# ctu-mrs/space_filling_forest_star

Measured on AMD Instinct MI355X. Metric: accepted node expansions/sec + collision checks/sec, dense_3D 6-DoF, higher is better.
Workload: dtype f64

## Files before the change

### space_filling_forest_star_amd/csrc/engine.cpp

```cpp
#include "engine.h"
#include <dlfcn.h>

#include <algorithm>
#include <chrono>
#include <cmath>
#include <cstdlib>
#include <cstring>
#include <limits>
#include <stdexcept>

#include "sff_geom.h"

namespace sff {

void hip_check(hipError_t e, const char* what) {
  if (e != hipSuccess) throw HipError{std::string(what) + ": " + hipGetErrorString(e)};
}
#define HIPCHK(x) hip_check((x), #x)

void DevBuf::ensure(size_t bytes) {
  if (bytes <= cap) return;
  size_t want = std::max(bytes, cap * 2);
  want = (want + 255) & ~(size_t)255;
  void* np = nullptr;
  HIPCHK(hipMalloc(&np, want));
  if (p) {
    HIPCHK(hipMemcpy(np, p, cap, hipMemcpyDeviceToDevice));
    (void)hipFree(p);
  }
  p = np;
  cap = want;
}
void DevBuf::release() {
  if (p) (void)hipFree(p);
  p = nullptr;
  cap = 0;
}
void PinBuf::ensure(size_t bytes) {
  if (bytes <= cap) return;
  size_t want = std::max(bytes, cap * 2);
  void* np = nullptr;
  HIPCHK(hipHostMalloc(&np, want, hipHostMallocDefault));
  if (p) {
    memcpy(np, p, cap);
    (void)hipHostFree(p);
  }
  p = np;
  cap = want;
}
void PinBuf::release() {
  if (p) (void)hipHostFree(p);
  p = nullptr;
  cap = 0;
}
void WordRing::init(uint64_t words) {
  HIPCHK(hipEventCreateWithFlags(&ev_ring, hipEventDisableTiming));
  ring_words = words;
  ring.ensure((size_t)words * 8);
  h_ring.ensure((size_t)words * 8);
}
void WordRing::release() {
  ring.release();
  h_ring.release();
  if (ev_ring) (void)hipEventDestroy(ev_ring);
  ev_ring = nullptr;
}
void WordRing::wait_on(hipStream_t s) {
  if (!ring_pending) return;
  HIPCHK(hipStreamWaitEvent(s, ev_ring, 0));
  ring_pending = false;
}

void Mt64::reseed(uint64_t seed) {
  mt[0] = seed;
  for (int i = 1; i < 312; ++i) mt[i] = 6364136223846793005ULL * (mt[i - 1] ^ (mt[i - 1] >> 62)) + (uint64_t)i;
  idx = 312;
  draws = 0;
  q = nullptr;
  qh = qn = 0;
}
static inline uint64_t mt_step(uint64_t a, uint64_t b, uint64_t far) {
  const uint64_t x = (a & 0xFFFFFFFF80000000ULL) | (b & 0x7FFFFFFFULL);
  return far ^ (x >> 1) ^ ((0ULL - (x & 1ULL)) & 0xB5026F5AA96619E9ULL);
}
static inline uint64_t mt_temper(uint64_t y) {
  y ^= (y >> 29) & 0x5555555555555555ULL;
  y ^= (y << 17) & 0x71D67FFFEDA60000ULL;
  y ^= (y << 37) & 0xFFF7EEE000000000ULL;
  y ^= (y >> 43);
  return y;
}
void Mt64::twist() {
  for (int i = 0; i < 156; ++i) mt[i] = mt_step(mt[i], mt[i + 1], mt[i + 156]);
  for (int i = 156; i < 311; ++i) mt[i] = mt_step(mt[i], mt[i + 1], mt[i - 156]);
  mt[311] = mt_step(mt[311], mt[0], mt[155]);
  idx = 0;
}
uint64_t Mt64::next() {
  ++draws;
  if (qh < qn) return q[qh++];
  if (idx >= 312) twist();
  return mt_temper(mt[idx++]);
}
void Mt64::fill(uint64_t* out, size_t n) {
  draws += n;
  size_t k = 0;
  if (qh < qn) {
    k = std::min(n, qn - qh);
    memcpy(out, q + qh, k * sizeof(uint64_t));
    qh += k;
  }
  while (k < n) {
    if (idx >= 312) twist();
    const size_t take = std::min<size_t>(312 - idx, n - k);
    for (size_t j = 0; j < take; ++j) out[k + j] = mt_temper(mt[idx + j]);
    idx += (int)take;
    k += take;
  }
}
void Mt64::prefetch(uint64_t* buf, size_t want) {
  if (q != buf || qh > 0) {
    const size_t left = qn - qh;
    if (left) memmove(buf, q + qh, left * sizeof(uint64_t));
    q = buf;
    qh = 0;
    qn = left;
  }
  while (qn < want) {
    if (idx >= 312) twist();
    size_t take = std::min<size_t>(312 - idx, want - qn);
    for (size_t k = 0; k < take; ++k) buf[qn + k] = mt_temper(mt[idx + k]);
    idx += (int)take;
    qn += take;
  }
}
int Mt64::uniform_int(int lo, int hi) {
  uint64_t range = (uint64_t)((int64_t)hi - (int64_t)lo) + 1ULL;
  unsigned __int128 prod = (unsigned __int128)next() * range;
  uint64_t low = (uint64_t)prod;
  if (low < range) {
    uint64_t thr = (0ULL - range) % range;
    while (low < thr) {
      prod = (unsigned __int128)next() * range;
      low = (uint64_t)prod;
    }
  }
  return lo + (int)(uint64_t)(prod >> 64);
}

Ctx::Ctx(int dev, const Ctx* owner) : device(dev) {
  kn = Knobs::from_env();
  int n = 0;
  HIPCHK(hipGetDeviceCount(&n));
  if (n <= 0) throw HipError{"no HIP device visible: libsffgpu has no CPU fallback"};
  if (dev < 0 || dev >= n) throw HipError{"device index out of range"};
  HIPCHK(hipSetDevice(dev));
  hipDeviceProp_t prop;
  HIPCHK(hipGetDeviceProperties(&prop, dev));
  if (std::string(prop.gcnArchName).find("gfx950") == std::string::npos)
    throw HipError{std::string("device is ") + prop.gcnArchName + ", kernels are built for gfx950 only"};
  if (owner) {
    env = owner->env;
    envv = owner->envv;
    robv = owner->robv;
    env_built_here = false;
    round_lazy = true;
    grid_compact = kn.compact_grid;
  } else {
    env = std::make_shared<EnvBlock>(dev);
  }
  {
    int khz = 0;
    if (hipDeviceGetAttribute(&khz, hipDeviceAttributeWallClockRate, dev) == hipSuccess && khz > 0) wall_clock_khz = khz;
  }
  HIPCHK(hipStreamCreateWithFlags(&stream, hipStreamNonBlocking));
  own_stream = stream;
  HIPCHK(hipStreamCreateWithFlags(&copy_stream, hipStreamNonBlocking));
  HIPCHK(hipEventCreateWithFlags(&ev_mid, hipEventDisableTiming));
  HIPCHK(hipEventCreateWithFlags(&ev_early, hipEventDisableTiming));
}

namespace {
struct RcclApi {
  struct Id128 { char b[128]; };
  int (*GetUniqueId)(void*) = nullptr;
  int (*CommInitRank)(void**, int, Id128, int) = nullptr;
  int (*AllGather)(const void*, void*, size_t, int, void*, hipStream_t) = nullptr;
  int (*CommDestroy)(void*) = nullptr;
  const char* (*GetErrorString)(int) = nullptr;
  bool ok = false;
};
RcclApi& rccl() {
  static RcclApi api;
  static bool tried = false;
  if (tried) return api;
  tried = true;
  void* h = nullptr;
  for (const char* name : {"librccl.so.1", "librccl.so"}) {
    h = dlopen(name, RTLD_NOW | RTLD_NOLOAD);
    if (h) break;
  }
  for (const char* name : {"librccl.so.1", "librccl.so", "/opt/rocm/lib/librccl.so.1"}) {
    if (h) break;
    h = dlopen(name, RTLD_NOW | RTLD_GLOBAL);
  }
  if (!h) return api;
  api.GetUniqueId = reinterpret_cast<decltype(api.GetUniqueId)>(dlsym(h, "ncclGetUniqueId"));
  api.CommInitRank = reinterpret_cast<decltype(api.CommInitRank)>(dlsym(h, "ncclCommInitRank"));
  api.AllGather = reinterpret_cast<decltype(api.AllGather)>(dlsym(h, "ncclAllGather"));
  api.CommDestroy = reinterpret_cast<decltype(api.CommDestroy)>(dlsym(h, "ncclCommDestroy"));
  api.GetErrorString = reinterpret_cast<decltype(api.GetErrorString)>(dlsym(h, "ncclGetErrorString"));
  api.ok = api.GetUniqueId && api.CommInitRank && api.AllGather && api.CommDestroy;
  return api;
}
void rccl_check(int rc, const char* what) {
  if (rc == 0) return;
  const char* msg = rccl().GetErrorString ? rccl().GetErrorString(rc) : "?";
  throw HipError{std::string("rccl: ") + what + " failed: " + msg};
}
}

void Ctx::rccl_unique_id(uint8_t* id128) {
  if (!rccl().ok) throw HipError{"rccl: librccl could not be bound"};
  rccl_check(rccl().GetUniqueId(id128), "ncclGetUniqueId");
}
void Ctx::rccl_init(const uint8_t* id128, int rank, int world) {
  if (!rccl().ok) throw HipError{"rccl: librccl could not be bound"};
  if (world < 1 || rank < 0 || rank >= world) throw HipError{"rccl: bad rank / world"};
  HIPCHK(hipSetDevice(device));
  if (rccl_comm) { (void)rccl().CommDestroy(rccl_comm); rccl_comm = nullptr; }
  RcclApi::Id128 id;
  memcpy(id.b, id128, 128);
  rccl_check(rccl().CommInitRank(&rccl_comm, world, id, rank), "ncclCommInitRank");
  rccl_rank = rank;
  rccl_world = world;
}
void Ctx::rccl_all_gather_i32(const void* send, void* recv, size_t words) {
  if (xchg_fn) {
    if (xchg_fn(xchg_user, send, recv, words, stream) != 0) throw HipError{"exchange: the caller's all-gather failed"};
    return;
  }
  rccl_check(rccl().AllGather(send, recv, words,  2, rccl_comm, stream), "ncclAllGather");
}

Ctx::~Ctx() {
  (void)hipSetDevice(device);
  if (stream) (void)hipStreamSynchronize(stream);
  if (own_stream && own_stream != stream) (void)hipStreamSynchronize(own_stream);
  if (copy_stream) (void)hipStreamSynchronize(copy_stream);
  if (rccl_comm && rccl().CommDestroy) { (void)rccl().CommDestroy(rccl_comm); rccl_comm = nullptr; }
  for (hipEvent_t e : rr_ev) if (e) (void)hipEventDestroy(e);
  for (SegJob& J : seg_job) if (J.ev) (void)hipEventDestroy(J.ev);
  if (ev_mid) (void)hipEventDestroy(ev_mid);
  if (ev_early) (void)hipEventDestroy(ev_early);
  for (auto& t : pending) { (void)hipEventDestroy(t.a); (void)hipEventDestroy(t.b); }
  for (auto e : pool) (void)hipEventDestroy(e);
  DevBuf* bufs[] = {&sx, &sy, &sz, &syaw, &spitch, &sroll, &stree, &spos,
                    &d_a, &d_b, &d_c, &d_d, &d_e, &d_f, &d_g, &d_h, &r_in, &r_out, &r_out2, &r_q, &r_cnt,
                    &r_sega, &r_segb, &r_items, &r_items2, &r_center, &r_qrec, &g_cnt, &g_items, &g_ovfcnt, &g_ovf, &g_bucket, &t_cnt, &t_items, &t_ovfcnt, &t_ovf, &t_occ, &g_lite, &g_ovf_lite, &t_lite, &t_ovf_lite, &r_sub, &rr_q1, &rr_q2, &rr_a, &rr_out, &rr_sq, &rr_np, &rr_alt, &rr_q2b, &rr_sqb, &seg_job[0].ids, &seg_job[0].a, &seg_job[0].b, &seg_job[0].c, &seg_job[1].ids, &seg_job[1].a,
                    &seg_job[1].b, &seg_job[1].c, &seg_job[2].ids, &seg_job[2].a, &seg_job[2].b, &seg_job[2].c, &seg_job[3].ids, &seg_job[3].a,
                    &seg_job[3].b, &seg_job[3].c, &sm_dev};
  for (DevBuf* b : bufs) b->release();
  env.reset();
  PinBuf* pins[] = {&h_a, &h_b, &h_c, &h_d, &h_e, &h_f, &h_g, &h_h, &p_in, &p_out, &rr_hq, &rr_hout, &seg_job[0].hids, &seg_job[0].hc, &seg_job[1].hids, &seg_job[1].hc, &seg_job[2].hids, &seg_job[2].hc,
                    &seg_job[3].hids, &seg_job[3].hc, &sm_pin};
  for (PinBuf* b : pins) b->release();
  if (copy_stream) (void)hipStreamDestroy(copy_stream);
  if (own_stream) (void)hipStreamDestroy(own_stream);
}

void Ctx::set_stream(hipStream_t s) {
  HIPCHK(hipSetDevice(device));
  sync();
  stream = s ? s : own_stream;
}

hipEvent_t Ctx::get_event() {
  if (!pool.empty()) {
    hipEvent_t e = pool.back();
    pool.pop_back();
    return e;
  }
  hipEvent_t e;
  HIPCHK(hipEventCreate(&e));
  return e;
}
void Ctx::time_begin(int kind) {
  kernel_calls[kind] += 1;
  if (round_scope) round_calls[kind] += 1;
  timed_now = timing_on;
  if (!timed_now) return;
  Timed t{get_event(), get_event(), kind, round_scope};
  HIPCHK(hipEventRecord(t.a, stream));
  pending.push_back(t);
}
void Ctx::time_end() { if (timed_now) HIPCHK(hipEventRecord(pending.back().b, stream)); }
double Ctx::kernel_ms_total(int kind) const {
  double ms = kernel_ms[kind];
  if (round_timed[kind]) ms += round_ms[kind] * ((double)round_calls[kind] / (double)round_timed[kind]);
  return ms;
}
void Ctx::sync() {
  HIPCHK(hipStreamSynchronize(stream));
  for (auto& t : pending) {
    float ms = 0;
    HIPCHK(hipEventElapsedTime(&ms, t.a, t.b));
    if (t.round) { round_ms[t.kind] += ms; round_timed[t.kind] += 1; }
    else kernel_ms[t.kind] += ms;
    kernel_launches[t.kind] += 1;
    pool.push_back(t.a);
    pool.push_back(t.b);
  }
  pending.clear();
}

static inline uint64_t spread21(uint64_t v) {
  v &= 0x1FFFFF;
  v = (v | v << 32) & 0x1F00000000FFFFULL;
  v = (v | v << 16) & 0x1F0000FF0000FFULL;
  v = (v | v << 8) & 0x100F00F00F00F00FULL;
  v = (v | v << 4) & 0x10C30C30C30C30C3ULL;
  v = (v | v << 2) & 0x1249249249249249ULL;
  return v;
}

void Ctx::upload_mesh(int role, const double* tri9, int n) {
  if (env.use_count() > 1)
    throw std::runtime_error("mesh_upload: the models of this context are shared with " + std::to_string(env.use_count() - 1) +
                             " other live context(s) (sffgpu_create_member); destroy them first");
  kn = Knobs::from_env();
  HIPCHK(hipSetDevice(device));
  struct Views {
    Ctx& c;
    ~Views() { c.envv = c.env->envv; c.robv = c.env->robv; }
  } views{*this};
  env->upload(kn, stream, role, tri9, n);
}

EnvBlock::~EnvBlock() {
  (void)hipSetDevice(device);
  DevBuf* bufs[] = {&env_tri, &env_box, &env_plane, &rob_tri, &env_clear, &env_clear_edge, &env_ext, &env_cand, &env_tg_start, &env_tg_list};
  for (DevBuf* b : bufs) b->release();
  for (auto& b : level_box) b.release();
}
size_t EnvBlock::device_bytes() const {
  size_t sum = env_tri.cap + env_box.cap + env_plane.cap + rob_tri.cap + env_clear.cap + env_clear_edge.cap + env_ext.cap + env_cand.cap +
               env_tg_start.cap + env_tg_list.cap;
  for (const DevBuf& b : level_box) sum += b.cap;
  return sum;
}

void EnvBlock::upload(const Knobs& kn, hipStream_t stream, int role, const double* tri9, int n) {
  if (role == SFFGPU_MESH_ROBOT) {
    if (n <= 0) throw HipError{"robot mesh must have at least one triangle"};
    rob_tri.ensure((size_t)n * 9 * sizeof(double));
    HIPCHK(hipMemcpy(rob_tri.p, tri9, (size_t)n * 9 * sizeof(double), hipMemcpyHostToDevice));
    robv.tri = rob_tri.as<double>();
    robv.n_tri = n;
    double lo[3] = {1e300, 1e300, 1e300}, hi[3] = {-1e300, -1e300, -1e300};
    for (int v = 0; v < n * 3; ++v)
      for (int i = 0; i < 3; ++i) {
        lo[i] = std::min(lo[i], tri9[3 * v + i]);
        hi[i] = std::max(hi[i], tri9[3 * v + i]);
      }
    double rad = 0;
    for (int i = 0; i < 3; ++i) { robv.lo[i] = lo[i]; robv.hi[i] = hi[i]; robv.center[i] = 0.5 * (lo[i] + hi[i]); }
    for (int v = 0; v < n * 3; ++v) {
      double d2 = 0;
      for (int i = 0; i < 3; ++i) d2 += (tri9[3 * v + i] - robv.center[i]) * (tri9[3 * v + i] - robv.center[i]);
      rad = std::max(rad, std::sqrt(d2));
    }
    robv.radius = rad;
    have_robot = true;
    h_rob.assign(tri9, tri9 + (size_t)n * 9);
    build_robot_extents(kn);
    build_clearance(kn, stream);
    build_tri_grid(kn, stream);
    return;
  }
  if (role != SFFGPU_MESH_ENV) throw HipError{"unknown mesh role"};
  envv = sffk::EnvView{};
  have_env = true;
  clear_cells = 0;
  if (n <= 0) return;
  std::vector<double> box((size_t)n * 6);
  double glo[3] = {1e300, 1e300, 1e300}, ghi[3] = {-1e300, -1e300, -1e300};
  for (int t = 0; t < n; ++t)
    for (int a = 0; a < 3; ++a) {
      const double* P = tri9 + 9 * (size_t)t;
      double lo = std::min(P[a], std::min(P[3 + a], P[6 + a])), hi = std::max(P[a], std::max(P[3 + a], P[6 + a]));
      box[6 * (size_t)t + a] = lo;
      box[6 * (size_t)t + 3 + a] = hi;
      glo[a] = std::min(glo[a], lo);
      ghi[a] = std::max(ghi[a], hi);
    }
  for (int a = 0; a < 3; ++a) { env_lo[a] = glo[a]; env_hi[a] = ghi[a]; }
  env_maxabs = 1.0;
  for (int a = 0; a < 3; ++a) env_maxabs = std::max(env_maxabs, std::max(std::fabs(glo[a]), std::fabs(ghi[a])));
  std::vector<std::pair<uint64_t, int>> order(n);
  for (int t = 0; t < n; ++t) {
    uint64_t code = 0;
    for (int a = 0; a < 3; ++a) {
      double ext = ghi[a] - glo[a];
      double c = 0.5 * (box[6 * (size_t)t + a] + box[6 * (size_t)t + 3 + a]);
      double u = ext > 0 ? (c - glo[a]) / ext : 0.0;
      uint64_t q = (uint64_t)std::min(2097151.0, std::max(0.0, u * 2097151.0));
      code |= spread21(q) << a;
    }
    order[t] = {code, t};
  }
  std::sort(order.begin(), order.end());
  std::vector<double> tri_s((size_t)n * 9), box_s((size_t)n * 6);
  for (int k = 0; k < n; ++k) {
    memcpy(&tri_s[9 * (size_t)k], tri9 + 9 * (size_t)order[k].second, 9 * sizeof(double));
    memcpy(&box_s[6 * (size_t)k], &box[6 * (size_t)order[k].second], 6 * sizeof(double));
// ... 232 lines not shown
  if (n <= 0) return;
  HIPCHK(hipSetDevice(device));
  store_reserve(store_n + n);
  const size_t pb = (size_t)n * 6 * sizeof(double), tb = (size_t)n * sizeof(int32_t);
  h_a.ensure(pb + tb);
  memcpy(h_a.p, pos6, pb);
  memcpy(h_a.as<char>() + pb, tree, tb);
  for (int i = 0; i < n * 6; ++i)
    if (i % 6 < 3) store_maxabs = std::max(store_maxabs, std::fabs(pos6[i]));
  d_a.ensure(pb + tb);
  HIPCHK(hipMemcpyAsync(d_a.p, h_a.p, pb + tb, hipMemcpyHostToDevice, stream));
  const bool fuse_grid = grid_on && grid_inserted == store_n;
  sffk::launch_store_write(stream, store_mut(*this), d_a.as<double>(), reinterpret_cast<const int32_t*>(d_a.as<char>() + pb),
                           nullptr, nullptr, n, store_n,
                           fuse_grid ? &gridv : nullptr);
  if (wait) sync();
  store_n += n;
  if (fuse_grid) grid_inserted = store_n;
}

void Ctx::store_set_tree(const int32_t* ids, int n, int32_t tree) {
  if (n <= 0) return;
  HIPCHK(hipSetDevice(device));
  h_a.ensure((size_t)n * 4);
  d_a.ensure((size_t)n * 4);
  memcpy(h_a.p, ids, (size_t)n * 4);
  HIPCHK(hipMemcpyAsync(d_a.p, h_a.p, (size_t)n * 4, hipMemcpyHostToDevice, stream));
  sffk::launch_set_tree(stream, stree.as<int32_t>(), d_a.as<int32_t>(), n, tree);
  sync();
  if (grid_on) {
    double lim[6];
    memcpy(lim, grid_limits, sizeof lim);
    grid_setup(lim, grid_cell);
    grid_insert_new();
    if (grid_compact) ++grid_rebuilds;
    grid_check(true);
  }
}

void Ctx::grid_setup(const double limits[6], double cell) {
  HIPCHK(hipSetDevice(device));
  memcpy(grid_limits, limits, sizeof grid_limits);
  double ext[3] = {limits[1] - limits[0], limits[3] - limits[2], limits[5] - limits[4]};
  for (int tries = 0; tries < 64; ++tries) {
    double cells = 1;
    for (int a = 0; a < 3; ++a) cells *= std::floor(ext[a] / cell) + 1;
    if (cells <= 16777216.0) break;
    cell *= 1.26;
  }
  gridv = sffk::GridView{};
  gridv.ox = (float)limits[0];
  gridv.oy = (float)limits[2];
  gridv.oz = (float)limits[4];
  grid_cell = cell;
  gridv.inv_cell = (float)(1.0 / cell);
  gridv.nx = (int)std::floor(ext[0] / cell) + 1;
  gridv.ny = (int)std::floor(ext[1] / cell) + 1;
  gridv.nz = (int)std::floor(ext[2] / cell) + 1;
  gridv.bk = grid_bk;
  const size_t ncells = (size_t)gridv.nx * gridv.ny * gridv.nz;
  if (gridv_ovf_cap_next < 65536) gridv_ovf_cap_next = 65536;
  gridv.ovf_cap = gridv_ovf_cap_next;
  if (kn.test_grid_ovf >= 0) gridv.ovf_cap = std::max(gridv.ovf_cap / 65536 * kn.test_grid_ovf, kn.test_grid_ovf);
  g_cnt.ensure(ncells * sizeof(int32_t));
  g_ovfcnt.ensure(16);
  g_ovf.ensure((size_t)gridv.ovf_cap * sizeof(sffk::GridItem));
  if (grid_compact) {
    int pool = grid_pool_next > 0 ? grid_pool_next : (kn.test_grid_pool > 0 ? kn.test_grid_pool : store_cap);
    if (kn.test_grid_pool <= 0) pool = std::max(pool, store_cap);
    grid_pool = grid_pool_next = std::max(pool, 1);
    g_bucket.ensure(ncells * sizeof(int32_t));
    g_items.ensure((size_t)grid_pool * gridv.bk * sizeof(sffk::GridItem));
    HIPCHK(hipMemsetAsync(g_bucket.p, 0xff, ncells * sizeof(int32_t), stream));
    gridv.bucket = g_bucket.as<int32_t>();
    gridv.pool_cnt = g_ovfcnt.as<int32_t>() + 1;
    gridv.pool_cap = grid_pool;
  } else {
    g_items.ensure(ncells * gridv.bk * sizeof(sffk::GridItem));
    g_lite.ensure(ncells * gridv.bk * sizeof(sffk::GridItem32));
    g_ovf_lite.ensure((size_t)gridv.ovf_cap * sizeof(sffk::GridItem32));
    gridv.lite = g_lite.as<sffk::GridItem32>();
    gridv.ovf_lite = g_ovf_lite.as<sffk::GridItem32>();
  }
  HIPCHK(hipMemsetAsync(g_cnt.p, 0, ncells * sizeof(int32_t), stream));
  HIPCHK(hipMemsetAsync(g_ovfcnt.p, 0, 16, stream));
  gridv.cnt = g_cnt.as<int32_t>();
  gridv.items = g_items.as<sffk::GridItem>();
  gridv.ovf_cnt = g_ovfcnt.as<int32_t>();
  gridv.ovf = g_ovf.as<sffk::GridItem>();
  tgridv = gridv;
  tgridv.bucket = nullptr;
  tgridv.pool_cnt = nullptr;
  tgridv.pool_cap = 0;
  tgridv.bk = 8;
  tgridv.ovf_cap = std::max(1 << 20, tgrid_ovf_min);
  tgridv.cnt = nullptr;
  tgridv.items = nullptr;
  tgridv.ovf = nullptr;
  tgridv.lite = nullptr;
  tgridv.ovf_lite = nullptr;
  tgridv.occ = nullptr;
  t_ovfcnt.ensure(16);
  HIPCHK(hipMemsetAsync(t_ovfcnt.p, 0, 16, stream));
  tgridv.ovf_cnt = t_ovfcnt.as<int32_t>();
  grid_on = true;
  grid_inserted = 0;
  const bool had_round = round_ready;
  round_ready = false;
  if (!round_lazy || had_round) round_grid();
}
void Ctx::grid_dense() {
  if (!grid_compact) return;
  grid_compact = false;
  if (!grid_on) return;
  sync();
  double lim[6];
  memcpy(lim, grid_limits, sizeof lim);
  grid_setup(lim, grid_cell);
  grid_insert_new();
  grid_check(true);
}
void Ctx::round_grid() {
  if (round_ready || !grid_on) return;
  if (grid_compact) throw HipError{"round grid asked for on a compact node grid (grid_dense() comes first)"};
  HIPCHK(hipSetDevice(device));
  const size_t ncells = (size_t)tgridv.nx * tgridv.ny * tgridv.nz;
  t_cnt.ensure(ncells * sizeof(int32_t));
  t_items.ensure(ncells * tgridv.bk * sizeof(sffk::GridItem));
  t_ovf.ensure((size_t)tgridv.ovf_cap * sizeof(sffk::GridItem));
  t_lite.ensure(ncells * tgridv.bk * sizeof(sffk::GridItem32));
  t_ovf_lite.ensure((size_t)tgridv.ovf_cap * sizeof(sffk::GridItem32));
  HIPCHK(hipMemsetAsync(t_cnt.p, 0, ncells * sizeof(int32_t), stream));
  tgridv.cnt = t_cnt.as<int32_t>();
  tgridv.items = t_items.as<sffk::GridItem>();
  tgridv.ovf = t_ovf.as<sffk::GridItem>();
  tgridv.lite = t_lite.as<sffk::GridItem32>();
  tgridv.ovf_lite = t_ovf_lite.as<sffk::GridItem32>();
  t_occ.ensure((ncells / 32 + 2) * 4);
  HIPCHK(hipMemsetAsync(t_occ.p, 0, (ncells / 32 + 2) * 4, stream));
  tgridv.occ = t_occ.as<uint32_t>();
  round_ready = true;
}
void Ctx::memory(sffgpu_ctx_memory* out) const {
  auto sum = [](std::initializer_list<const DevBuf*> l) { size_t s = 0; for (const DevBuf* b : l) s += b->cap; return (uint64_t)s; };
  *out = sffgpu_ctx_memory{};
  out->env_bytes = env_built_here ? (uint64_t)env->device_bytes() : 0;
  out->env_holders = (uint64_t)env.use_count();
  out->store_bytes = sum({&sx, &sy, &sz, &syaw, &spitch, &sroll, &stree, &spos});
  out->grid_bytes = sum({&g_cnt, &g_items, &g_ovfcnt, &g_ovf, &g_lite, &g_ovf_lite, &t_ovfcnt, &g_bucket});
  out->round_grid_bytes = sum({&t_cnt, &t_items, &t_ovf, &t_occ, &t_lite, &t_ovf_lite});
  out->other_bytes = sum({&d_a, &d_b, &d_c, &d_d, &d_e, &d_f, &d_g, &d_h, &sm_dev, &r_in, &r_out, &r_q, &r_cnt, &r_sega, &r_segb,
                          &r_items, &r_items2, &r_sub, &r_center, &r_qrec, &r_out2, &rr_q1, &rr_q2, &rr_a, &rr_out, &rr_sq, &rr_np, &rr_alt, &rr_q2b, &rr_sqb});
  for (const SegJob& J : seg_job) out->other_bytes += sum({&J.ids, &J.a, &J.b, &J.c});
  out->total_bytes = out->env_bytes + out->store_bytes + out->grid_bytes + out->round_grid_bytes + out->other_bytes;
}
void Ctx::grid_insert_new() {
  if (!grid_on || grid_inserted >= store_n) return;
  sffk::launch_grid_insert(stream, gridv, store_view(), grid_inserted, store_n - grid_inserted);
  grid_inserted = store_n;
}
void Ctx::grid_check(bool bulk) {
  if (!grid_on) return;
  int32_t v = 0;
  if (grid_compact) {
    int32_t w[2] = {0, 0};
    HIPCHK(hipMemcpyAsync(w, g_ovfcnt.p, 8, hipMemcpyDeviceToHost, stream));
    HIPCHK(hipStreamSynchronize(stream));
    for (int tries = 0; tries < 32 && w[1] > grid_pool; ++tries) {
      if (!bulk && w[0] > gridv.ovf_cap) throw HipError{"neighbour grid overflow list exhausted during a wave (nodes were dropped)"};
      grid_pool_next = std::max(2 * grid_pool, kn.test_grid_pool > 0 ? 0 : store_cap);
      double lim[6];
      memcpy(lim, grid_limits, sizeof lim);
      grid_setup(lim, grid_cell);
      grid_insert_new();
      ++grid_rebuilds;
      bulk = true;
      HIPCHK(hipMemcpyAsync(w, g_ovfcnt.p, 8, hipMemcpyDeviceToHost, stream));
      HIPCHK(hipStreamSynchronize(stream));
    }
  }
  HIPCHK(hipMemcpyAsync(&v, g_ovfcnt.p, 4, hipMemcpyDeviceToHost, stream));
  HIPCHK(hipStreamSynchronize(stream));
  if (bulk) {
    for (int tries = 0; tries < 40 && v > grid_rebuild_at(); ++tries) {
      const size_t cells_now = (size_t)gridv.nx * gridv.ny * gridv.nz;
      double cell = grid_cell;
      if (cells_now * 4 <= 16777216 && grid_cell * 0.63 >= 0.5 * grid_cell0) cell = grid_cell * 0.63;
      else if (grid_bk < kn.test_grid_bkmax && cells_now * (size_t)grid_bk * 2 * sizeof(sffk::GridItem) <= ((size_t)24 << 30)) grid_bk *= 2;
      else if (cells_now * 4 <= 16777216) cell = grid_cell * 0.63;
      else grid_grow_list();
      double lim[6];
      memcpy(lim, grid_limits, sizeof lim);
      grid_setup(lim, cell);
      grid_insert_new();
      ++grid_rebuilds;
      HIPCHK(hipMemcpyAsync(&v, g_ovfcnt.p, 4, hipMemcpyDeviceToHost, stream));
      HIPCHK(hipStreamSynchronize(stream));
    }
    if (v > gridv.ovf_cap) throw HipError{"grid overflow list exhausted"};
    return;
  }
  if (v > gridv.ovf_cap) throw HipError{"neighbour grid overflow list exhausted during a wave (nodes were dropped)"};
  if (v <= grid_rebuild_at()) return;
  const size_t cells_now = (size_t)gridv.nx * gridv.ny * gridv.nz;
  double cell = grid_cell;
  if (cells_now * 4 <= 16777216 && grid_cell * 0.63 >= 0.5 * grid_cell0) cell = grid_cell * 0.63;
  else if (grid_bk < kn.test_grid_bkmax && cells_now * (size_t)grid_bk * 2 * sizeof(sffk::GridItem) <= ((size_t)24 << 30))
    grid_bk *= 2;
  else grid_grow_list();
  double lim[6];
  memcpy(lim, grid_limits, sizeof lim);
  grid_setup(lim, cell);
  grid_insert_new();
  ++grid_rebuilds;
  HIPCHK(hipMemcpyAsync(&v, g_ovfcnt.p, 4, hipMemcpyDeviceToHost, stream));
  HIPCHK(hipStreamSynchronize(stream));
  if (v > gridv.ovf_cap) throw HipError{"grid overflow list exhausted"};
}

void Ctx::grid_grow_list() {
  grid_exhausted = true;
  if (gridv.ovf_cap > (1 << 24)) throw HipError{"neighbour grid: more than 2^24 nodes do not fit their cells' buckets (too many nodes per xyz cell)"};
  gridv_ovf_cap_next = gridv.ovf_cap * 4;
}

double Ctx::sweep_eps() const { return std::max(store_maxabs, env_maxabs()) * std::ldexp(1.0, -20); }

void Ctx::collide_poses(const double* pos6, int n, uint8_t* hit, bool explicit_rt) {
  if (n <= 0) return;
  if (!have_env() || !have_robot()) throw HipError{"collide_poses: upload ENV and ROBOT meshes first"};
  HIPCHK(hipSetDevice(device));
  const size_t per = (explicit_rt ? 12 : 6) * sizeof(double);
  h_a.ensure((size_t)n * per);
  h_b.ensure((size_t)n);
  memcpy(h_a.p, pos6, (size_t)n * per);
  d_a.ensure((size_t)n * per);
  d_b.ensure((size_t)n);
  HIPCHK(hipMemcpyAsync(d_a.p, h_a.p, (size_t)n * per, hipMemcpyHostToDevice, stream));
  time_begin(T_COLLIDE);
  sffk::launch_collide_poses(stream, envv, robv, d_a.as<double>(), n, nullptr, d_b.as<uint8_t>(), explicit_rt);
  time_end();
  HIPCHK(hipMemcpyAsync(h_b.p, d_b.p, (size_t)n, hipMemcpyDeviceToHost, stream));
  sync();
  memcpy(hit, h_b.p, (size_t)n);
}

void Ctx::collide_segments(const double* a6, const double* b6, int n, uint8_t* is_free, int32_t* first_hit,
                           int32_t* n_samples) {
  collide_segments_core(a6, b6, nullptr, nullptr, n, is_free, first_hit, n_samples);
}
void Ctx::collide_segments_ids(const int32_t* ida, const int32_t* idb, int n, uint8_t* is_free, int32_t* first_hit,
                               int32_t* n_samples) {
  collide_segments_core(nullptr, nullptr, ida, idb, n, is_free, first_hit, n_samples);
}
void Ctx::collide_segments_refs(const int32_t* ida, const int32_t* idb, int n, uint8_t* is_free, int32_t* first_hit, int32_t* n_samples) {
  if (!rr_np_dev) throw HipError{"collide_segments_refs: no rrt_chain has run"};
  collide_segments_core(nullptr, nullptr, ida, idb, n, is_free, first_hit, n_samples, rr_np_dev);
}
void Ctx::collide_segments_core(const double* a6, const double* b6, const int32_t* ida, const int32_t* idb, int n,
                                uint8_t* is_free, int32_t* first_hit, int32_t* n_samples, const double* extra_dev) {
  if (n <= 0) return;
  if (!have_env() || !have_robot()) throw HipError{"collide_segments: upload ENV and ROBOT meshes first"};
  HIPCHK(hipSetDevice(device));
  const size_t pb = (size_t)n * 6 * sizeof(double);
  h_a.ensure(pb); h_b.ensure(pb); h_c.ensure((size_t)n * 12 + 64);
  if (a6) {
    memcpy(h_a.p, a6, pb);
    memcpy(h_b.p, b6, pb);
  } else {
    memcpy(h_a.p, ida, (size_t)n * 4);
    memcpy(h_b.p, idb, (size_t)n * 4);
  }
  d_a.ensure(pb); d_b.ensure(pb); d_c.ensure((size_t)n * 12 + 64);
  int32_t* d_ns = d_c.as<int32_t>();
  int32_t* d_fh = d_ns + n;
  int32_t* d_ov = d_fh + n;
  int32_t* d_ctrl = d_ov + n;
  if (a6) {
    HIPCHK(hipMemcpyAsync(d_a.p, h_a.p, pb, hipMemcpyHostToDevice, stream));
    HIPCHK(hipMemcpyAsync(d_b.p, h_b.p, pb, hipMemcpyHostToDevice, stream));
  } else {
    d_d.ensure((size_t)n * 8);
    HIPCHK(hipMemcpyAsync(d_d.p, h_a.p, (size_t)n * 4, hipMemcpyHostToDevice, stream));
    HIPCHK(hipMemcpyAsync(d_d.as<int32_t>() + n, h_b.p, (size_t)n * 4, hipMemcpyHostToDevice, stream));
    sffk::launch_seg_gather(stream, spos.as<double>(), d_d.as<int32_t>(), d_d.as<int32_t>() + n, n, d_a.as<double>(),
                            d_b.as<double>(), extra_dev);
  }
  HIPCHK(hipMemsetAsync(d_ctrl, 0, 64, stream));
  const int list_cap = 8 * n + 65536;
  r_items.ensure((size_t)list_cap * SFFK_ITEM_BYTES);
  r_items2.ensure(((size_t)list_cap + (1u << 20)) * 8);
  time_begin(T_COLLIDE);
  sffk::launch_seg_prepare(stream, d_a.as<double>(), d_b.as<double>(), n, d_ns, d_fh, d_ov);
  sffk::launch_collide_segments_dyn(stream, kn, envv, robv, d_a.as<double>(), d_b.as<double>(), d_ns, n, d_ctrl,
                                    r_items.p, list_cap, r_items2.p, d_fh, d_ov);
  time_end();
  HIPCHK(hipMemcpyAsync(h_c.p, d_c.p, (size_t)n * 12, hipMemcpyDeviceToHost, stream));
  sync();
  seg_finish(h_c.as<int32_t>(), n, a6, b6, d_a.p, d_b.p, is_free, first_hit, n_samples);
}

void Ctx::seg_finish(const int32_t* hn_in, int n, const double* a6, const double* b6, const void* dev_a, const void* dev_b, uint8_t* is_free,
                     int32_t* first_hit, int32_t* n_samples) {
  const size_t pb = (size_t)n * 6 * sizeof(double);
  bool any_ovf = false;
  {
// ... 535 lines not shown
```

### space_filling_forest_star_amd/csrc/engine.h

```cpp
#pragma once
#include <hip/hip_runtime.h>
#include <stdint.h>
#include <string.h>

#include <algorithm>
#include <functional>
#include <map>
#include <memory>
#include <unordered_set>
#include <string>
#include <utility>
#include <vector>

#include "../../include/sffgpu.h"
#include "kernels.h"
#include "knobs.h"

namespace sff {

struct HipError {
  std::string msg;
};
void hip_check(hipError_t e, const char* what);

struct DevBuf {
  void* p = nullptr;
  size_t cap = 0;
  void ensure(size_t bytes);
  void release();
  template <class T> T* as() const { return reinterpret_cast<T*>(p); }
};
struct PinBuf {
  void* p = nullptr;
  size_t cap = 0;
  void ensure(size_t bytes);
  void release();
  template <class T> T* as() const { return reinterpret_cast<T*>(p); }
};

struct Mt64 {
  uint64_t mt[312];
  int idx;
  uint64_t draws = 0;
  uint64_t* q = nullptr;
  size_t qh = 0, qn = 0;
  explicit Mt64(uint64_t seed = 5489ULL) { reseed(seed); }
  void reseed(uint64_t seed);
  void twist();
  void prefetch(uint64_t* buf, size_t want);
  uint64_t next();
  void fill(uint64_t* out, size_t n);
  int uniform_int(int lo, int hi);
};

struct WordRing {
  DevBuf ring;
  PinBuf h_ring;
  hipEvent_t ev_ring = nullptr;
  uint64_t ring_words = 0;
  uint64_t produced = 0;
  bool ring_pending = false;
  void init(uint64_t words);
  void release();
  template <class PerRun = void (*)(uint64_t, size_t)>
  void append(hipStream_t copy_stream, const uint64_t* words, Mt64* gen, size_t n, PerRun per_run = [](uint64_t, size_t) {}) {
    uint64_t* hr = h_ring.as<uint64_t>();
    for (size_t done = 0; done < n;) {
      const uint64_t at = (produced + done) & (ring_words - 1);
      const size_t run = std::min<size_t>(n - done, (size_t)(ring_words - at));
      if (words) memcpy(hr + at, words + done, run * 8);
      else gen->fill(hr + at, run);
      hip_check(hipMemcpyAsync(ring.as<uint64_t>() + at, hr + at, run * 8, hipMemcpyHostToDevice, copy_stream), "ring copy");
      per_run(at, run);
      done += run;
    }
    produced += n;
    hip_check(hipEventRecord(ev_ring, copy_stream), "ring event");
    ring_pending = true;
  }
  void wait_on(hipStream_t s);
};

struct HitRec {
  double d;
  int id;
  bool operator<(const HitRec& o) const { return d < o.d || (d == o.d && id < o.id); }
};

enum TimerKind { T_SWEEP = 0, T_COLLIDE = 1, T_SAMPLE = 2, T_COMMIT = 3, T_EXCHANGE = 4, T_KINDS = 5 };

struct EnvBlock {
  int device = 0;
  DevBuf env_tri, env_box, env_plane, level_box[SFFK_MAX_LEVELS], rob_tri, env_clear, env_clear_edge, env_ext, env_cand;
  DevBuf env_tg_start, env_tg_list;
  std::vector<double> h_plane, h_rob;
  sffk::EnvView envv{};
  sffk::RobotView robv{};
  bool have_env = false, have_robot = false;
  double env_maxabs = 1.0;
  double env_lo[3] = {0, 0, 0}, env_hi[3] = {0, 0, 0};
  long long clear_cells = 0;
  void upload(const Knobs& kn, hipStream_t stream, int role, const double* tri9, int n);
  void build_robot_extents(const Knobs& kn);
  void build_clearance(const Knobs& kn, hipStream_t stream);
  void build_tri_grid(const Knobs& kn, hipStream_t stream);
  size_t device_bytes() const;
  explicit EnvBlock(int dev) : device(dev) {}
  EnvBlock(const EnvBlock&) = delete;
  EnvBlock& operator=(const EnvBlock&) = delete;
  ~EnvBlock();
};

struct Ctx {
  int device = 0;
  Knobs kn;
  int wall_clock_khz = 100000;
  hipStream_t stream = nullptr;
  hipStream_t own_stream = nullptr;
  void set_stream(hipStream_t s);
  hipStream_t copy_stream = nullptr;
  hipEvent_t ev_mid = nullptr, ev_early = nullptr;
  std::string err;

  std::shared_ptr<EnvBlock> env;
  bool env_built_here = true;
  sffk::EnvView envv{};
  sffk::RobotView robv{};
  bool have_env() const { return env->have_env; }
  bool have_robot() const { return env->have_robot; }
  double env_maxabs() const { return env->env_maxabs; }
  void* rccl_comm = nullptr;
  int rccl_rank = 0, rccl_world = 1;
  void rccl_init(const uint8_t* id128, int rank, int world);
  void rccl_all_gather_i32(const void* send, void* recv, size_t words);
  int (*xchg_fn)(void* user, const void* send_dev, void* recv_dev, size_t words_i32, void* hip_stream) = nullptr;
  void* xchg_user = nullptr;
  int xchg_rank = 0, xchg_world = 1;
  bool can_exchange(int rank, int world) const {
    return (xchg_fn && xchg_world == world && xchg_rank == rank) || (rccl_comm && rccl_world == world && rccl_rank == rank);
  }
  static void rccl_unique_id(uint8_t* id128);

  int store_cap = 0, store_n = 0;
  DevBuf sx, sy, sz, syaw, spitch, sroll, stree, spos;
  double store_maxabs = 1.0;

  bool grid_on = false;
  sffk::GridView gridv{};
  DevBuf g_cnt, g_items, g_ovfcnt, g_ovf, g_lite, g_ovf_lite;
  DevBuf g_bucket;
  DevBuf t_cnt, t_items, t_ovfcnt, t_ovf, t_occ, t_lite, t_ovf_lite;
  sffk::GridView tgridv{};
  bool round_lazy = false;
  bool grid_compact = false;
  int grid_pool = 0;
  int grid_pool_next = 0;
  void grid_dense();
  bool round_ready = false;
  void round_grid();
  int grid_inserted = 0;
  void grid_setup(const double limits[6], double cell);
  void grid_insert_new();
  void grid_check(bool bulk = false);
  double grid_cell = 0, grid_limits[6] = {0, 0, 0, 0, 0, 0};
  int grid_rebuilds = 0;
  int gridv_ovf_cap_next = 65536;
  int grid_bk = 8;
  bool grid_exhausted = false;
  int grid_rebuild_at() const { return grid_exhausted ? std::max(128, gridv.ovf_cap / 4) : std::min(gridv.ovf_cap / 4, 128); }
  void grid_grow_list();
  double grid_cell0 = 0;
  int tgrid_ovf_min = 0;

  DevBuf d_a, d_b, d_c, d_d, d_e, d_f, d_g, d_h;
  PinBuf h_a, h_b, h_c, h_d, h_e, h_f, h_g, h_h;
  DevBuf sm_dev;
  PinBuf sm_pin;
  DevBuf r_in, r_out, r_q, r_cnt, r_sega, r_segb, r_items, r_items2, r_sub, r_center;
  DevBuf r_qrec;
  DevBuf r_out2;
  PinBuf p_in, p_out;

  struct Timed { hipEvent_t a, b; int kind; bool round; };
  std::vector<Timed> pending;
  std::vector<hipEvent_t> pool;
  double kernel_ms[T_KINDS] = {0, 0, 0, 0, 0};
  uint64_t kernel_launches[T_KINDS] = {0, 0, 0, 0, 0};
  uint64_t kernel_calls[T_KINDS] = {0, 0, 0, 0, 0};
  double round_ms[T_KINDS] = {0, 0, 0, 0, 0};
  uint64_t round_calls[T_KINDS] = {0, 0, 0, 0, 0}, round_timed[T_KINDS] = {0, 0, 0, 0, 0};
  bool round_scope = false;
  bool timing_on = true, timed_now = true;
  double kernel_ms_total(int kind) const;

  explicit Ctx(int dev, const Ctx* owner = nullptr);
  ~Ctx();
  void memory(sffgpu_ctx_memory* out) const;
  void sync();
  hipEvent_t get_event();
  void time_begin(int kind);
  void time_end();

  void upload_mesh(int role, const double* tri9, int n);
  sffk::NodeStoreView store_view() const;
  void store_reset(int capacity);
  void store_reserve(int capacity);
  void store_append(const double* pos6, const int32_t* tree, int n, bool wait = true);
  void store_set_tree(const int32_t* ids, int n, int32_t tree);

  void collide_poses(const double* pos6, int n, uint8_t* hit, bool explicit_rt = false);
  void collide_segments(const double* a6, const double* b6, int n, uint8_t* is_free, int32_t* first_hit,
                        int32_t* n_samples);
  void collide_segments_ids(const int32_t* ida, const int32_t* idb, int n, uint8_t* is_free, int32_t* first_hit,
                            int32_t* n_samples);
  void collide_segments_refs(const int32_t* ida, const int32_t* idb, int n, uint8_t* is_free, int32_t* first_hit, int32_t* n_samples);
  const double* rr_np_dev = nullptr;
  void collide_segments_core(const double* a6, const double* b6, const int32_t* ida, const int32_t* idb, int n,
                             uint8_t* is_free, int32_t* first_hit, int32_t* n_samples, const double* extra_dev = nullptr);
  void sample_steer(const uint64_t* words, const double* center6, int n, double dist, int dim, const double* limits,
                    double* out6, uint8_t* in_limits);
  void radius(const double* q6, int nq, const double* r, const int32_t* tree, const int32_t* max_id, int32_t* idx,
              double* dist, int32_t* cnt, int cap);
  void knn(const double* q6, int nq, int k, const int32_t* tree, const int32_t* max_id, int32_t* idx, double* dist,
           int32_t* cnt, bool tree_by_grid = false);
  struct RrtRows {
    double* np6; uint8_t* hit; int32_t* seg; int32_t* mem_idx; double* mem_d; int32_t* mem_cnt;
    int32_t* conn_idx; double* conn_d; int32_t* conn_cnt;
  };
  void rrt_chain(const double* rnd6, const int32_t* tree, int n, double dist, bool by_grid1, int kmax, bool by_gridk,
                 int32_t* near_idx, double* near_d, int32_t* near_cnt, int32_t* mate, RrtRows& R, double conn_r = 0, int conn_cap = 0,
                 int alt_cap = 0, int32_t* alt_slot = nullptr, int32_t* alt_mate = nullptr, int32_t* n_alt = nullptr, RrtRows* R2 = nullptr);
  void rrt_chain_alt(const int32_t* slot, const int32_t* mate, int n_alt, double dist, int kmax, bool by_gridk, RrtRows& R,
                     double conn_r = 0, int conn_cap = 0);
  int rr_rows0 = 0;
  DevBuf rr_q1, rr_q2, rr_a, rr_out, rr_sq, rr_np, rr_alt, rr_q2b, rr_sqb;
  struct SegJob { DevBuf ids, a, b, c; PinBuf hids, hc; hipEvent_t ev = nullptr; int n = 0; };
  SegJob seg_job[4];
  void seg_refs_begin(int which, const int32_t* ida, const int32_t* idb, int n, int n_hint);
  void seg_refs_end(int which, uint8_t* is_free, int32_t* first_hit, int32_t* n_samples);
  void seg_finish(const int32_t* hn_in, int n, const double* a6, const double* b6, const void* dev_a, const void* dev_b, uint8_t* is_free,
                  int32_t* first_hit, int32_t* n_samples);
  hipEvent_t rr_ev[3] = {nullptr, nullptr, nullptr};
  PinBuf rr_hq, rr_hout;
  double sweep_eps() const;
  void sweep_lists(const double* q6, int nq, const std::vector<double>& r, const int32_t* tree, const int32_t* max_id,
                   const std::vector<uint8_t>& active, int cap, int n_store, std::vector<int32_t>& cnt,
                   std::vector<std::vector<HitRec>>& out, bool sort_lists = true);
};

struct FNode {
  double pos[6];
  int tree, parent, idx_in_tree;
  double d_closest, d_root;
  unsigned iter;
};
struct Border {
  int n1, n2;
  double dist;
};

struct PHeap {
  std::vector<int> v;
  const std::vector<FNode>* nodes = nullptr;
  double ref[6];
  double cost(int i) const;
  void bubble_down(int index);
  void bubble_up(int index);
  void push(int n);
  int pop();
  int pop_at(int id);
};

struct FlatSet64 {
  std::vector<uint64_t> tab;
  size_t used = 0;
  bool insert(uint64_t key) {
    if (tab.empty()) tab.assign(1024, 0);
    if ((used + 1) * 10 > tab.size() * 7) grow();
    size_t m = tab.size() - 1, h = (size_t)((key * 0x9E3779B97F4A7C15ULL) >> 20) & m;
    while (tab[h] != 0) {
      if (tab[h] == key) return false;
      h = (h + 1) & m;
    }
    tab[h] = key;
    ++used;
    return true;
  }
  void grow() {
    std::vector<uint64_t> old;
    old.swap(tab);
    tab.assign(old.size() * 2, 0);
    used = 0;
    for (uint64_t k : old) if (k) insert(k);
  }
};

struct DevEngine {
  bool on = false;
  bool inited = false;
  bool active = false;
  bool host_stale = false;
  bool table_dirty = false;
  DevBuf frontier2, rm_words, rm_pref, slot_pos, act_slot2, w_acc, acc_pref, ustate32, wg_pub, commit_seq, kc_trace;
  DevBuf ord_hist, ord_start, ord_key, ord_rank, ord_pos, ord_lst, ord_cnt;
  DevBuf w_ev, ev_h, ev_nb, ev_raw;
  DevBuf ctrl, parent, d_root, d_closest, iter, nflag, frontier, closed, claim, slot_node, slot_fail, act_slot, b_n1,
      b_n2, b_ta, b_tb, b_dist, bt_key, bt_val, pair, ulist, d_parent, d_parent2, d_force, fault_pending;
  DevBuf hp_base, hp_size, hp_v, hp_key, hp_pos, hp_ref, hp_gen, hp_cnt, slot_tree, slot_heap, slot_idx, slot_word, hp_plan;
  int prio_heaps = 0, prio_cap = 0;
  DevBuf s_ktab, s_tree_cnt, s_head, s_mcnt, s_mid, s_md, s_next, s_prop, s_best, s_psel, s_dcl, s_cnt, s_accs, s_hdr, s_changed,
      s_ew, s_ida, s_idb, s_sub, s_segns, s_fh, s_sovf, s_evs, s_evn, s_eve, s_evd, s_acc, s_backup, s_items, s_dbg, s_hist;
  int hist_cap = 0;
  int s_items_cap = 0;
  bool star_inited = false;
  hipGraphExec_t wave_graph = nullptr;
  uint64_t wave_graph_sig = 0;
  bool graph_enabled = true;
  int round_parity = 0;
  int force_timing = -1;
  bool round_timing = false;
  uint64_t graph_calls[T_KINDS] = {0, 0, 0, 0, 0};
  uint64_t waves_enqueued = 0, graph_launches = 0, graph_captures = 0;
  PinBuf h_ctrl, h_trig;
  WordRing wr;
  DevBuf trig;
  bool dev_trig = false;
  hipEvent_t ev_wave = nullptr, ev_wave2 = nullptr;
  int node_cap = 0, border_cap = 0, temp_base = 0;
  uint64_t bt_size = 0, max_wave_words = 0;
  uint64_t rounds_enqueued = 0;
  int host_nodes = 0, host_borders = 0;
  sffk::DevCtrl last{};
  uint32_t status_next = 0;
  uint32_t status_of[2] = {0, 0};
  bool status_copied[2] = {true, true};
  DevBuf spec_tab, spec_area;
  DevBuf qclk_sh;
  int spec_n_sc = 0, spec_sets = 0, spec_tm = 0;
  bool spec_off = false;
  PinBuf h_seq;
  DevBuf seq_args;
  uint64_t seq_pick_slack = 0;
};

struct Forest {
  Ctx* ctx;
  sffgpu_forest_cfg cfg;
  Knobs kn;
  DevEngine dev;
  bool device_eligible() const;
  sffk::DevForestView dev_view() const;
  sffk::StarView star_view() const;
  void dev_star_setup();
  void dev_size_node_arrays();
  void dev_size_border_arrays(int want_cap);
  void dev_ring_append(const uint64_t* words, size_t n);
  void dev_ring_top_up(uint64_t cursor, uint64_t ahead);
  void dev_upload_state();
  void dev_to_host();
  void dev_enqueue_begin();
  void dev_enqueue_round_eval(void* send_dev, bool sample = true);
  void dev_enqueue_round_commit(const void* recv_dev, bool sample_next = false);
  void dev_enqueue_end(int slot = 0);
  int dev_finish_wave(double* wait_ms, int slot = 0, bool stream_idle = true);
  void dev_enqueue_wave(int slot);
  void dev_enqueue_wave_kernels(bool sharded, size_t words);
  uint64_t dev_launch_signature();
  DevBuf x_send, x_recv;
  bool need_host_exchange = false;
  bool exchange_open = false;
  Ctx::Timed exchange_t{};
  void exchange_timer_drop();
  bool dev_wave_begin();
  size_t dev_exchange_bytes() const;
  void run_device(int max_waves);
  bool batch_eligible() const;
  bool seq_eligible() const;
  void run_device_seq(int max_waves);
  int seq_kind() const { return (cfg.optimize ? 1 : 0) | (use_priority() ? 2 : 0) | (cfg.has_goal ? 4 : 0); }
  int seq_launch_waves(int waves_left) const;
  uint64_t seq_words_end(int batch) const;
  uint64_t seq_words_per_wave() const;
  void seq_note_launch(uint64_t waves_before);
  sffk::SeqArgs seq_prepare(int batch);
  void grid_dense();
  void seq_lists_fault();
  bool spec_setup();
  bool seq_suspended = false;
  void sync_host();
  void fill_stats(sffgpu_forest_stats* out);
  ~Forest();
  Mt64 rng;
  std::vector<uint64_t> rng_ahead;
  struct HistRec { int32_t node, parent; uint32_t iter; };
  std::vector<HistRec> hist;
  size_t hist_sorted = 0;
  bool hist_overflow = false;
  std::vector<FNode> nodes;
  std::vector<uint8_t> nflag;
  std::vector<std::vector<int>> trees;
  std::vector<int> frontier, closed;
  std::map<std::pair<int, int>, std::vector<Border>> borders;
  FlatSet64 border_keys;
  std::vector<int> connected;
  int num_roots = 0;
  int goal_node = -1;
  int iter = 0;
  bool solved = false, empty_frontier = false;
  sffgpu_forest_stats st{};

  struct Slot { int node; bool from_closed; bool failing; int tree = -1, heap = -1; };
  std::vector<Slot> slots;
  std::vector<std::vector<PHeap>> heaps;
  bool use_priority() const { return cfg.priority_bias != 0; }
  void dev_prio_upload(int gen = -2);
  void dev_prio_download();
  void dev_prio_regrow();
  bool tree_frontiers_empty(int t) const;
  bool all_frontiers_empty() const;
  int round = 0;
  bool in_wave = false;

  struct Nb {
    int tree;
    double d;
    int order;
    int id;
    bool same_tree;
    int seg;
    bool free = false;
    int fh = -1, ns = 0;
  };
  struct Member {
    int id;
    bool fwd_free = false, bwd_free = false;
    int fwd_fh = -1, fwd_ns = 0, bwd_fh = -1, bwd_ns = 0;
    int seg_f = -1, seg_b = -1;
  };
  struct Cand {
    int slot, expanded;
    int accepted_id = -1;
    bool in_lim = false;
    bool answered = false, pose_hit = false, par_free = false;
    bool has_members = false;
    int par_fh = -1, par_ns = 0;
    double pdist = 0;
    double pos[6];
    int pose_task = -1, seg_parent = -1;
    std::vector<Nb> nbs;
    std::vector<Member> members;
    void reset(int s, int e) {
      slot = s; expanded = e; accepted_id = -1; in_lim = false;
      answered = pose_hit = par_free = false; par_fh = -1; par_ns = 0; pdist = 0;
      if (has_members) { members.clear(); has_members = false; }
    }
  };
  std::vector<Cand> cands;
  std::vector<int> round_todo;
  const double* round_hpos = nullptr;
  const double* round_hpd = nullptr;
  const uint8_t* round_hlim = nullptr;
  std::vector<uint8_t> round_skip;
  int n_cands = 0;
  std::vector<int32_t> records;
  uint64_t bulk_counts[4] = {0, 0, 0, 0};
  bool pending_round = false;
  int iter0 = 0, N0 = 0, Tb = 0;
  double knn_r = 0;
  std::vector<std::vector<HitRec>> knn_out;
  std::vector<int32_t> edge_ia, edge_ib;
  bool query_wide = false;
  void on_list_fault();

  struct Holder {
    int n1 = -1, n2 = -1;
    double dist = 1.7976931348623157e308;
    std::vector<int> plan;
    bool exists() const { return n1 >= 0; }
  };
  std::vector<Holder> nm;
  Holder& NM(int i, int j) { return nm[(size_t)(i < j ? i : j) * num_roots + (i < j ? j : i)]; }
  void get_paths();
  void get_all_paths();
  void smooth_paths();
  sffgpu_smooth_stats sm{};

  Forest(Ctx* c, const sffgpu_forest_cfg& cf, const double* roots6, int n_roots);
  int add_node(const double* pos, int tree, int parent, double dclosest, double droot, unsigned it);
  std::vector<Border>& border(int i, int j);
  int max_connected();
  template <class HasBorder> int max_connected_over(HasBorder has_border, std::vector<int>& out_connected) const;
  bool budget_hit() const { return cfg.node_budget > 0 && (int)nodes.size() >= cfg.node_budget; }
  bool terminated() const { return solved || iter >= cfg.max_iterations || budget_hit(); }
  void begin_wave();
  void end_wave();
  void round_begin();
  void round_commit(const int32_t* all, int total_words, const int32_t* counts, int world);
  void run(int max_waves);
  uint64_t fingerprint() const;
};

void run_forest_batch(Forest* const* members, int n, int max_waves, int* failed);

struct RNode {
  double pos[6];
  int root_tree;
  int tree;
  int parent, idx_in_tree;
  double d_closest, d_root;
  unsigned iter;
};
// ... 84 lines not shown
```

### space_filling_forest_star_amd/csrc/forest.cpp

```cpp
#include <algorithm>
#include <chrono>
#include <cmath>
#include <cstdio>
#include <cstdlib>
#include <cstring>
#include <limits>

#include "engine.h"
#include "sff_geom.h"

namespace sff {

#define HIPCHK(x) hip_check((x), #x)
using Clock = std::chrono::steady_clock;
static double g_sec[8] = {0, 0, 0, 0, 0, 0, 0, 0};
extern double g_sweep_dbg[4];
static double g_star[4] = {0, 0, 0, 0};
static double g_wait[3] = {0, 0, 0};
static uint64_t g_items[4] = {0, 0, 0, 0};
static uint64_t g_cnt[4] = {0, 0, 0, 0};
struct Sec {
  int k;
  Clock::time_point t0;
  explicit Sec(int kk) : k(kk), t0(Clock::now()) {}
// ... 103 lines not shown
  if (cfg.has_goal) {
    goal_node = add_node(cfg.goal, n_roots, -1, 0, 0, 0);
    if (cfg.record_parents) hist.push_back({goal_node, -1, 0u});
    int32_t gt = n_roots;
    ctx->store_append(cfg.goal, &gt, 1);
  }
  ctx->grid_insert_new();
  if (use_priority()) {
    heaps.resize(num_roots);
    auto add_heap = [&](int tree, int ref_node) {
      PHeap hp;
      hp.nodes = &nodes;
      memcpy(hp.ref, nodes[ref_node].pos, sizeof hp.ref);
      for (int id : trees[tree]) hp.v.push_back(id);
      for (int k = (int)hp.v.size() - 1; k >= 0; --k) hp.bubble_down(k);
      heaps[tree].push_back(hp);
    };
    if (!cfg.has_goal) {
      for (int i = 0; i < n_roots; ++i)
        for (int j = 0; j < n_roots; ++j)
          if (i != j) add_heap(i, trees[j][0]);
    } else {
      for (int i = 0; i < n_roots; ++i) add_heap(i, goal_node);
    }
  }
  memset(&st, 0, sizeof st);
  knn_r = 2.5 * cfg.sampling_dist;
  if (kn.test_hitcap < 24) query_wide = true;
  dev.spec_off = !kn.spec;
  if (kn.no_graph >= 0) dev.graph_enabled = kn.no_graph == 0;
  else if (cfg.optimize && kn.profiler_preloaded) {
    dev.graph_enabled = false;
    fprintf(stderr, "[sffgpu] profiler library in LD_PRELOAD: SFF* waves are launched kernel by kernel (SFFGPU_NO_GRAPH=0 / 1 overrides)\n");
  }
}

int Forest::add_node(const double* pos, int tree, int parent, double dclosest, double droot, unsigned it) {
  FNode n;
  memcpy(n.pos, pos, sizeof n.pos);
  n.tree = tree;
  n.parent = parent;
  n.d_closest = dclosest;
  n.d_root = droot;
  n.iter = it;
  n.idx_in_tree = (int)trees[tree].size();
  int id = (int)nodes.size();
  nodes.push_back(n);
  nflag.push_back(0);
  trees[tree].push_back(id);
  return id;
}

std::vector<Border>& Forest::border(int i, int j) {
  if (i > j) std::swap(i, j);
  return borders[{i, j}];
}

template <class HasBorder>
int Forest::max_connected_over(HasBorder has_border, std::vector<int>& out_connected) const {
  int max_conn = 0, remaining = num_roots;
  std::vector<char> conn(num_roots, 0);
  int unconnected = 0;
  while (max_conn < remaining) {
    out_connected.clear();
    std::vector<int> stack{unconnected};
    conn[unconnected] = 1;
    while (!stack.empty()) {
      int root = stack.front();
      stack.erase(stack.begin());
      out_connected.push_back(root);
      for (int i = 0; i < num_roots; ++i) {
        if (root == i) continue;
        if (!conn[i] && has_border(std::min(root, i), std::max(root, i))) {
          conn[i] = 1;
          stack.insert(stack.begin(), i);
        }
      }
    }
    max_conn = (int)out_connected.size();
    for (int i = 0; i < num_roots; ++i)
      if (!conn[i]) { unconnected = i; break; }
    remaining -= max_conn;
  }
  return max_conn;
}
int Forest::max_connected() {
  return max_connected_over([&](int a, int b) {
    auto it = borders.find({a, b});
    return it != borders.end() && !it->second.empty();
  }, connected);
}

void Forest::fill_stats(sffgpu_forest_stats* out) {
  sffgpu_forest_stats s = st;
  if (dev.active && dev.host_stale) {
    const sffk::DevCtrl& k = dev.last;
    std::vector<uint8_t> pair((size_t)num_roots * num_roots);
    HIPCHK(hipMemcpy(pair.data(), dev.pair.p, pair.size(), hipMemcpyDeviceToHost));
    std::vector<int> conn;
    const int mc = max_connected_over([&](int a, int b) { return pair[(size_t)a * num_roots + b] != 0; }, conn);
    s.iterations = k.iter;
    s.solved = (k.solved || (!cfg.has_goal && mc == num_roots)) ? 1 : 0;
    s.n_nodes = k.n_nodes;
    s.frontier_size = k.frontier_n;
    s.closed_size = k.closed_n;
    s.n_connected = (int)conn.size();
    s.n_borders = k.n_borders;
    s.collide_calls = k.collide_calls;
    s.path_free_calls = k.path_free_calls;
    s.nn_queries = k.nn_queries;
    s.poses_executed = k.poses_executed;
    s.segments_executed = k.segments_executed;
    s.samples_executed = k.samples_executed;
    if (use_priority() && kn.prio_seq) s.prio_seq_waves += k.waves - st.waves;
    s.waves = k.waves;
    s.sweeps = k.rounds;
    s.sweep_nodes = k.round_nodes;
    s.sweep_queries = k.round_queries;
    s.star_rounds = k.star_rounds;
    s.star_passes = k.star_passes;
    s.star_members = k.star_members;
    s.star_rewires = k.star_rewires;
    s.spec_steps = k.spec_steps;
    s.spec_evaluated = k.spec_evaluated;
    s.spec_committed = k.spec_committed;
  } else {
    s.iterations = iter;
    bool sv = solved;
    if (!sv && !cfg.has_goal) sv = max_connected() == num_roots;
    s.solved = sv;
    s.n_nodes = (int)nodes.size();
    s.frontier_size = (int)frontier.size();
    s.closed_size = (int)closed.size();
    s.n_connected = (int)connected.size();
    int nb = 0;
    for (auto& kv : borders) nb += (int)kv.second.size();
    s.n_borders = nb;
  }
  s.n_trees = (int)trees.size();
  if (dev.active || dev.inited) {
    s.query_clock_ms = (double)dev.last.q_ticks / (double)ctx->wall_clock_khz;
    s.query_clock_launches = dev.last.q_launches;
  }
  s.grid_rebuilds = (uint64_t)ctx->grid_rebuilds;
  s.sweep_ms = ctx->kernel_ms_total(T_SWEEP);
  s.collide_ms = ctx->kernel_ms_total(T_COLLIDE);
  s.sample_ms = ctx->kernel_ms_total(T_SAMPLE);
  s.commit_ms = ctx->kernel_ms_total(T_COMMIT);
  s.exchange_ms = ctx->kernel_ms_total(T_EXCHANGE);
  s.graph_launches = dev.graph_launches;
  *out = s;
}

Forest::~Forest() {
  DevBuf* bufs[] = {&dev.ctrl, &dev.parent, &dev.d_root, &dev.d_closest, &dev.iter, &dev.nflag, &dev.frontier, &dev.closed,
                    &dev.claim, &dev.slot_node, &dev.slot_fail, &dev.act_slot, &dev.b_n1, &dev.b_n2, &dev.b_ta, &dev.b_tb,
                    &dev.b_dist, &dev.bt_key, &dev.bt_val, &dev.pair, &dev.ulist,
                    &dev.d_parent, &dev.d_parent2, &dev.d_force, &dev.fault_pending, &dev.frontier2, &dev.rm_words, &dev.rm_pref,
                    &dev.slot_pos, &dev.act_slot2, &dev.trig, &dev.s_ktab, &dev.s_tree_cnt, &dev.s_head, &dev.s_mcnt, &dev.s_mid, &dev.s_md,
                    &dev.s_next, &dev.s_prop, &dev.s_best, &dev.s_psel, &dev.s_dcl, &dev.s_cnt, &dev.s_accs, &dev.s_hdr, &dev.s_changed,
                    &dev.s_ew, &dev.s_ida, &dev.s_idb, &dev.s_sub, &dev.s_segns, &dev.s_fh, &dev.s_sovf, &dev.s_evs, &dev.s_evn, &dev.s_eve,
                    &dev.s_evd, &dev.s_acc, &dev.s_backup, &dev.s_items, &dev.s_dbg, &dev.s_hist, &dev.w_acc, &dev.acc_pref, &dev.ustate32, &dev.wg_pub, &dev.commit_seq, &dev.kc_trace, &x_send, &x_recv,
                    &dev.hp_base, &dev.hp_size, &dev.hp_v, &dev.hp_key, &dev.hp_pos, &dev.hp_ref, &dev.hp_gen, &dev.hp_cnt, &dev.slot_tree, &dev.slot_heap, &dev.slot_idx, &dev.slot_word, &dev.hp_plan,
                    &dev.ord_hist, &dev.ord_start, &dev.ord_key, &dev.ord_rank, &dev.ord_pos, &dev.ord_lst, &dev.ord_cnt,
                    &dev.w_ev, &dev.ev_h, &dev.ev_nb, &dev.ev_raw, &dev.spec_tab, &dev.spec_area, &dev.qclk_sh, &dev.seq_args};
  if (dev.inited) {
    (void)hipSetDevice(ctx->device);
    (void)hipStreamSynchronize(ctx->stream);
    (void)hipStreamSynchronize(ctx->copy_stream);
  }
  for (DevBuf* b : bufs) b->release();
  dev.h_ctrl.release();
  dev.h_seq.release();
  dev.wr.release();
  dev.h_trig.release();
  if (dev.wave_graph) (void)hipGraphExecDestroy(dev.wave_graph);
  if (dev.ev_wave) (void)hipEventDestroy(dev.ev_wave);
  if (dev.ev_wave2) (void)hipEventDestroy(dev.ev_wave2);
}

void Forest::begin_wave() {
  slots.clear();
  if (use_priority() && !empty_frontier) {
    int pool = 0;
    for (auto& hs : heaps) if (!hs.empty()) pool += (int)hs[0].v.size();
    const int n_slots = std::max(1, std::min(cfg.wave, pool));
    for (int s = 0; s < n_slots; ++s) {
      if (all_frontiers_empty()) break;
      int t = -1;
      while (t < 0 || tree_frontiers_empty(t)) t = rng.uniform_int(0, (int)trees.size() - 1);
      int hp = -1;
      while (hp < 0 || heaps[t][hp].v.empty()) hp = rng.uniform_int(0, (int)heaps[t].size() - 1);
      PHeap& prior = heaps[t][hp];
      Slot sl;
      if (sffg::uniform_real(rng.next(), 0.0, 1.0) <= cfg.priority_bias) sl.node = prior.pop();
      else sl.node = prior.pop_at(rng.uniform_int(0, (int)prior.v.size() - 1));
      sl.from_closed = false;
      sl.failing = true;
      sl.tree = t;
      sl.heap = hp;
      slots.push_back(sl);
    }
  } else {
    const bool use_closed = !closed.empty() && empty_frontier;
    const int pool = use_closed ? (int)closed.size() : (int)frontier.size();
    const int n_slots = std::max(1, std::min(cfg.wave, pool));
    for (int s = 0; s < n_slots; ++s) {
      Slot sl;
      if (use_closed) {
        sl.node = closed[rng.uniform_int(0, (int)closed.size() - 1)];
        sl.from_closed = true;
      } else {
        sl.node = frontier[rng.uniform_int(0, (int)frontier.size() - 1)];
        sl.from_closed = false;
      }
      sl.failing = true;
      slots.push_back(sl);
    }
  }
  round = 0;
  in_wave = true;
  ++st.waves;
}

void Forest::end_wave() {
  bool removed = false;
  for (Slot& sl : slots) {
    if (use_priority() && sl.tree >= 0) {
      if (sl.failing) {
        for (int i = (int)heaps[sl.tree].size() - 1; i > -1; --i) {
          if (i == sl.heap) continue;
          PHeap& p = heaps[sl.tree][i];
          for (int j = (int)p.v.size() - 1; j > -1; --j)
            if (j < (int)p.v.size() && p.v[j] == sl.node) p.pop_at(j);
        }
        if (!(nflag[sl.node] & 1)) {
          nflag[sl.node] |= 1;
          closed.push_back(sl.node);
        }
      } else {
        heaps[sl.tree][sl.heap].push(sl.node);
      }
      continue;
    }
    if (sl.failing && !sl.from_closed && (nflag[sl.node] & 2)) {
      nflag[sl.node] = (uint8_t)((nflag[sl.node] & ~2) | 1);
      closed.push_back(sl.node);
      removed = true;
    }
  }
  if (removed) {
    size_t w = 0;
    for (size_t r = 0; r < frontier.size(); ++r)
      if (nflag[frontier[r]] & 2) frontier[w++] = frontier[r];
    frontier.resize(w);
  }
  ctx->grid_check();
  if (!solved && use_priority()) empty_frontier = all_frontiers_empty();
  else empty_frontier = frontier.empty();
  if (!solved) {
    bool conn = max_connected() == num_roots;
    solved = (!cfg.has_goal && empty_frontier && conn);
  } else {
    max_connected();
  }
  in_wave = false;
}

static const int32_t REC_MAGIC = 0x53464652;

static void sample_point_libm(const uint64_t* w, const double* center, double dist, int dim, double* out) {
  sffg::SampleTrig t{};
  const double phi = sffg::sample_angle(w[0]);
  t.c_phi = std::cos(phi);
  t.s_phi = std::sin(phi);
  if (dim != 2) {
    const double theta = sffg::sample_angle(w[1]);
    t.c_theta = std::cos(theta);
    t.s_theta = std::sin(theta);
    t.acos_u = std::acos(sffg::sample_acos_arg(w[3]));
  }
  const double nolim[6] = {-1e300, 1e300, -1e300, 1e300, -1e300, 1e300};
  sffg::sample_point_with(w, center, dist, dim, nolim, out, t);
}

void Forest::round_begin() {
  Ctx& c = *ctx;
  HIPCHK(hipSetDevice(c.device));
  if (pending_round) throw HipError{"forest: round_begin called twice without round_commit"};
  if (dev.active) dev_to_host();
  grid_dense();
  c.round_grid();
  if (!in_wave) {
    if (terminated()) return;
    begin_wave();
  }
  auto t_host = Clock::now();
  double wait_ms = 0;
  auto timed_sync = [&]() {
    auto t0 = Clock::now();
    c.sync();
    wait_ms += ms_since(t0);
  };
  auto _t0 = Clock::now();
  if (cands.size() < slots.size()) cands.resize(slots.size());
  n_cands = 0;
  for (int s = 0; s < (int)slots.size(); ++s) {
    if (!slots[s].failing) continue;
    if (iter + n_cands >= cfg.max_iterations) break;
    cands[n_cands++].reset(s, slots[s].node);
  }
  const int n = n_cands;
  ++round;
  pending_round = true;
  records.clear();
  records.push_back(REC_MAGIC);
  records.push_back(n);
  for (int k = 0; k < 8; ++k) records.push_back(0);
  bulk_counts[0] = bulk_counts[1] = bulk_counts[2] = bulk_counts[3] = 0;
  if (n == 0) return;
  iter0 = iter;
  iter += n;
  N0 = (int)nodes.size();
  Tb = (N0 + 3) & ~3;
  c.store_reserve(Tb + n + 4);

  g_sec[0] += ms_since(_t0);
  auto _t1 = Clock::now();
  const int words_per = cfg.dim == 2 ? 1 : 6;
  const int CAP = kn.test_hitcap, NBCAP = kn.test_nbcap, STRIDE = 1 + NBCAP;
  const size_t in_words = 0, in_parent = (size_t)n * 48, in_force = in_parent + (size_t)n * 4;
// ... 842 lines not shown
```

### space_filling_forest_star_amd/csrc/forest_batch.cpp

```cpp
#include "batch_lockstep.h"

namespace sff {

namespace {
struct ForestFamily {
  using Args = sffk::SeqArgs;
  static constexpr int n_kinds = 8;
  Forest* const* m;
  int n, max_waves;
  std::vector<uint64_t> w0, w_launch;
  std::vector<double> alone_ms;

  int device() { return m[0]->ctx->device; }
  void begin(int i) {
    Forest& f = *m[i];
    if (!f.dev.active) f.dev_upload_state();
    f.ctx->sync();
    w0[i] = f.dev.last.waves;
  }
  int plan(int i) {
    Forest& f = *m[i];
    const sffk::DevCtrl& k = f.dev.last;
    while (k.in_wave) {
      const double before = f.st.total_ms;
      f.seq_suspended = true;
      f.run_device(1);
      f.seq_suspended = false;
      alone_ms[i] += f.st.total_ms - before;
      f.ctx->sync();
    }
    if (k.terminated) return 0;
    if (max_waves > 0 && (int)(k.waves - w0[i]) >= max_waves) return 0;
    return f.seq_launch_waves(max_waves > 0 ? max_waves - (int)(k.waves - w0[i]) : 0);
  }
  uint64_t words_needed(int i, int waves) {
    const uint64_t end = m[i]->seq_words_end(waves);
    return end > m[i]->dev.wr.produced ? end - m[i]->dev.wr.produced : 0;
  }
  Mt64& gen(int i) { return m[i]->rng; }
  void ring_append(int i, const uint64_t* w, size_t nw) { m[i]->dev_ring_append(w, nw); }
  WordRing& ring(int i) { return m[i]->dev.wr; }
  Args prepare(int i, int waves) {
    w_launch[i] = m[i]->dev.last.waves;
    return m[i]->seq_prepare(waves);
  }
  int kind(int i) { return m[i]->seq_kind(); }
  hipStream_t stream(int i) { return m[i]->ctx->stream; }
  StatusBlock status(int i) { return {m[i]->dev.h_ctrl.p, m[i]->dev.ctrl.p, sizeof(sffk::DevCtrl)}; }
  hipError_t launch(hipStream_t s, const Args* a, int count, int kind, size_t lds) {
    return sffk::launch_seq_waves_batch(s, a, count, (kind & 1) != 0, (kind & 2) != 0, (kind & 4) != 0, lds);
  }
  void take_in(int i, double* wait_ms) {
    Forest& f = *m[i];
    f.dev.status_copied[0] = true;
    f.dev.host_stale = true;
    ++f.st.batch_launches;
    const int fault = f.dev_finish_wave(wait_ms, 0, true);
    f.seq_note_launch(w_launch[i]);
    if (fault == SFFK_FAULT_LISTS) f.seq_lists_fault();
    f.ctx->sync();
  }
  void finish(double wall, double wait_ms) {
    for (int i = 0; i < n; ++i) {
      m[i]->seq_suspended = false;
      m[i]->st.total_ms += std::max(0.0, wall - alone_ms[i]);
      m[i]->st.host_ms += std::max(0.0, wall - alone_ms[i] - wait_ms);
    }
  }
};
}

void run_forest_batch(Forest* const* members, int n, int max_waves, int* failed) {
  ForestFamily fam{members, n, max_waves, std::vector<uint64_t>((size_t)n), std::vector<uint64_t>((size_t)n, 0), std::vector<double>((size_t)n, 0.0)};
  run_lockstep(fam, n, failed);
}

}
```

### space_filling_forest_star_amd/csrc/forest_dev.cpp

```cpp
#include <algorithm>
#include <chrono>
#include <cmath>
#include <cstdio>
#include <cstdlib>
#include <cstring>
#include <thread>
#include <vector>

#include "engine.h"
#include "sff_geom.h"

namespace sff {

#define HIPCHK(x) hip_check((x), #x)
using Clock = std::chrono::steady_clock;
static double ms_since(Clock::time_point t0) { return std::chrono::duration<double, std::milli>(Clock::now() - t0).count(); }

static uint64_t next_pow2(uint64_t v) {
  uint64_t p = 1;
  while (p < v) p <<= 1;
  return p;
}

bool Forest::device_eligible() const {
  if (!use_priority()) return true;
  if (cfg.has_goal) {
    if (!kn.prio_goal_loop || !kn.prio_device || kn.no_seq || num_roots > 64 || cfg.wave != 1 || cfg.world > 1) return false;
    const long long heaps_n = num_roots - 1;
    const long long cap = (long long)std::max(cfg.node_budget, 4096) + 2LL * cfg.wave + 128;
    return heaps_n >= 1 && heaps_n <= SFFK_PRIO_MAX_HEAPS && heaps_n * cap * 16 <= (32LL << 30);
  }
  const int min_wave = !kn.prio_device ? 0x7fffffff : (kn.prio_loop && !kn.no_seq && num_roots <= 64) ? 1 : 2;
  if (cfg.wave < min_wave || cfg.world > 1) return false;
  const long long heaps_n = (long long)num_roots * (num_roots - 1);
  const long long cap = (long long)std::max(cfg.node_budget, 4096) + 2LL * cfg.wave + 128;
  return heaps_n >= 1 && heaps_n <= SFFK_PRIO_MAX_HEAPS && heaps_n * cap * 16 <= (32LL << 30);
}

void Forest::dev_prio_upload(int gen) {
  DevEngine& d = dev;
  Ctx& c = *ctx;
  int H = 0;
  std::vector<int32_t> base(heaps.size() + 1, 0);
  for (size_t t = 0; t < heaps.size(); ++t) { base[t] = H; H += (int)heaps[t].size(); }
  base[heaps.size()] = H;
  const int cap = cfg.node_budget > 0 ? std::min(d.node_cap, cfg.node_budget + 2 * cfg.wave + 256) : d.node_cap;
  d.prio_heaps = H;
  d.prio_cap = cap;
  d.hp_base.ensure(base.size() * 4);
  d.hp_size.ensure((size_t)H * 4);
  d.hp_gen.ensure((size_t)H * 4);
  d.hp_cnt.ensure(16);
  d.hp_ref.ensure((size_t)H * 48);
  d.hp_v.ensure((size_t)H * cap * 4);
  d.hp_key.ensure((size_t)H * cap * 8);
  d.hp_pos.ensure((size_t)H * cap * 4);
  d.slot_tree.ensure((size_t)cfg.wave * 4);
  d.slot_heap.ensure((size_t)cfg.wave * 4);
  d.slot_idx.ensure((size_t)cfg.wave * 4);
  d.slot_word.ensure((size_t)cfg.wave * 8);
  d.hp_plan.ensure(64);
  std::vector<int32_t> sizes(H);
  std::vector<double> refs((size_t)H * 6);
  HIPCHK(hipMemsetAsync(d.hp_pos.p, 0xFF, (size_t)H * cap * 4, c.stream));
  HIPCHK(hipMemsetD32Async(reinterpret_cast<hipDeviceptr_t>(d.hp_gen.p), gen, (size_t)H, c.stream));
  HIPCHK(hipMemsetAsync(d.hp_cnt.p, 0, 16, c.stream));
  std::vector<double> keys;
  int h = 0;
  for (size_t t = 0; t < heaps.size(); ++t)
    for (PHeap& hp : heaps[t]) {
      sizes[h] = (int32_t)hp.v.size();
      memcpy(&refs[6 * (size_t)h], hp.ref, 48);
      if (!hp.v.empty()) {
        keys.resize(hp.v.size());
        for (size_t i = 0; i < hp.v.size(); ++i) keys[i] = hp.cost((int)i);
        HIPCHK(hipMemcpy(d.hp_v.as<int32_t>() + (size_t)h * cap, hp.v.data(), hp.v.size() * 4, hipMemcpyHostToDevice));
        HIPCHK(hipMemcpy(d.hp_key.as<double>() + (size_t)h * cap, keys.data(), keys.size() * 8, hipMemcpyHostToDevice));
      }
      ++h;
    }
  HIPCHK(hipMemcpy(d.hp_base.p, base.data(), base.size() * 4, hipMemcpyHostToDevice));
  HIPCHK(hipMemcpy(d.hp_size.p, sizes.data(), (size_t)H * 4, hipMemcpyHostToDevice));
  HIPCHK(hipMemcpy(d.hp_ref.p, refs.data(), refs.size() * 8, hipMemcpyHostToDevice));
  sffk::launch_prio_index(c.stream, dev_view().prio);
  HIPCHK(hipStreamSynchronize(c.stream));
}
void Forest::dev_prio_regrow() {
  DevEngine& d = dev;
  Ctx& c = *ctx;
  const int H = d.prio_heaps, old_cap = d.prio_cap;
  const int cap = cfg.node_budget > 0 ? std::min(d.node_cap, cfg.node_budget + 2 * cfg.wave + 256) : d.node_cap;
  if (!H || cap <= old_cap) return;
  DevBuf nv, nk;
  nv.ensure((size_t)H * cap * 4);
  nk.ensure((size_t)H * cap * 8);
  HIPCHK(hipMemcpy2DAsync(nv.p, (size_t)cap * 4, d.hp_v.p, (size_t)old_cap * 4, (size_t)old_cap * 4, H, hipMemcpyDeviceToDevice, c.stream));
  HIPCHK(hipMemcpy2DAsync(nk.p, (size_t)cap * 8, d.hp_key.p, (size_t)old_cap * 8, (size_t)old_cap * 8, H, hipMemcpyDeviceToDevice, c.stream));
  HIPCHK(hipStreamSynchronize(c.stream));
  d.hp_v.release(); d.hp_key.release(); d.hp_pos.release();
  d.hp_v = nv; d.hp_key = nk;
  nv.p = nullptr; nv.cap = 0; nk.p = nullptr; nk.cap = 0;
  d.hp_pos.ensure((size_t)H * cap * 4);
  d.prio_cap = cap;
  HIPCHK(hipMemsetAsync(d.hp_pos.p, 0xFF, (size_t)H * cap * 4, c.stream));
  sffk::launch_prio_index(c.stream, dev_view().prio);
  HIPCHK(hipStreamSynchronize(c.stream));
}
void Forest::dev_prio_download() {
  DevEngine& d = dev;
  if (!d.prio_heaps) return;
  const int H = d.prio_heaps, cap = d.prio_cap;
  std::vector<int32_t> sizes(H);
  HIPCHK(hipMemcpy(sizes.data(), d.hp_size.p, (size_t)H * 4, hipMemcpyDeviceToHost));
  int h = 0;
  for (size_t t = 0; t < heaps.size(); ++t)
    for (PHeap& hp : heaps[t]) {
      hp.v.resize((size_t)sizes[h]);
      if (sizes[h]) HIPCHK(hipMemcpy(hp.v.data(), d.hp_v.as<int32_t>() + (size_t)h * cap, (size_t)sizes[h] * 4, hipMemcpyDeviceToHost));
      ++h;
    }
}

sffk::StarView Forest::star_view() const {
  const DevEngine& d = dev;
  sffk::StarView v{};
  v.ktab = d.s_ktab.as<int32_t>();
  v.tree_cnt = d.s_tree_cnt.as<int32_t>();
  v.head = d.s_head.as<unsigned long long>();
  v.m_cnt = d.s_mcnt.as<int32_t>();
  v.m_id = d.s_mid.as<int32_t>();
  v.m_d = d.s_md.as<double>();
  v.next = d.s_next.as<int32_t>();
  v.prop = d.s_prop.as<double>();
  v.best = d.s_best.as<double>();
  v.psel = d.s_psel.as<int32_t>();
  v.dcl = d.s_dcl.as<double>();
  v.cnt = d.s_cnt.as<unsigned long long>();
  v.acc_sample = d.s_accs.as<int32_t>();
  v.hdr = d.s_hdr.as<int32_t>();
  v.changed = d.s_changed.as<int32_t>();
  v.ew = d.s_ew.as<int32_t>();
  v.ens = d.s_segns.as<int32_t>();
  v.first_hit = d.s_fh.as<int32_t>();
  v.seg_ovf = d.s_sovf.as<int32_t>();
  v.ida = d.s_ida.as<int32_t>();
  v.idb = d.s_idb.as<int32_t>();
  v.sub = d.s_sub.as<int32_t>();
  v.items = d.s_items.p;
  v.items_cap = d.s_items_cap;
  v.ev_sample = d.s_evs.as<int32_t>();
  v.ev_nb = d.s_evn.as<int32_t>();
  v.ev_ex = d.s_eve.as<int32_t>();
  v.ev_dist = d.s_evd.as<double>();
  v.acc = d.s_acc.as<unsigned long long>();
  v.backup = d.s_backup.as<sffk::DevCtrl>();
  v.dbg = d.s_dbg.as<unsigned long long>();
  if (cfg.record_parents) {
    v.hist = d.s_hist.as<int32_t>() + 4;
    v.hist_ctl = d.s_hist.as<int32_t>();
    v.hist_cap = d.hist_cap;
  }
  return v;
}
// ... 8 lines not shown
    for (int m = 1; m < 64; ++m) {
      long long lo = 1, hi = 0x7fffffffLL;
      if (k_of(hi) < m) { ktab[m] = 0x7fffffff; continue; }
      while (lo < hi) {
        const long long mid = (lo + hi) / 2;
        if (k_of(mid) >= m) hi = mid; else lo = mid + 1;
      }
      ktab[m] = (int32_t)lo;
    }
    d.s_ktab.ensure(64 * 4);
    HIPCHK(hipMemcpy(d.s_ktab.p, ktab.data(), 64 * 4, hipMemcpyHostToDevice));
    d.s_tree_cnt.ensure((size_t)num_roots * 16 * 4);
    d.s_mcnt.ensure(W * 4);
    d.s_mid.ensure(W * KC * 4);
    d.s_md.ensure(W * KC * 8);
    d.s_next.ensure(W * KC * 4);
    d.s_prop.ensure(W * KC * 8);
    d.s_best.ensure(W * 8);
    d.s_psel.ensure(W * 4);
    d.s_dcl.ensure(W * 8);
    d.s_cnt.ensure(W * 16);
    d.s_accs.ensure(W * 4);
    d.s_hdr.ensure(64);
    d.s_changed.ensure(256);
    d.s_ew.ensure(W * KC * 2 * 4);
    d.s_ida.ensure(W * KC * 2 * 4);
    d.s_idb.ensure(W * KC * 2 * 4);
    d.s_sub.ensure((size_t)SFFK_STAR_PASSES * SFFK_SUBLISTS * SFFK_STAR_SUB * 4);
    d.s_segns.ensure(W * KC * 2 * 4);
    d.s_fh.ensure(W * KC * 2 * 4);
    d.s_sovf.ensure(W * KC * 2 * 4);
    d.s_evs.ensure(W * 4);
    d.s_evn.ensure(W * 4);
    d.s_eve.ensure(W * 4);
    d.s_evd.ensure(W * 8);
    d.s_acc.ensure(64 * SFFK_STAR_ACC * 8);
    d.s_backup.ensure(sizeof(sffk::DevCtrl));
    d.s_items_cap = (int)std::min<size_t>(16 * W + 65536, (size_t)1 << 26) / SFFK_SUBLISTS * SFFK_SUBLISTS;
    if (kn.test_star_items >= 0) d.s_items_cap = std::max(SFFK_SUBLISTS, kn.test_star_items) / SFFK_SUBLISTS * SFFK_SUBLISTS;
    d.s_items.ensure((size_t)d.s_items_cap * sizeof(sffk::SurvivorItem));
    HIPCHK(hipMemset(d.s_sub.p, 0, d.s_sub.cap));
    if (kn.profile) {
      d.s_dbg.ensure(32 * 8);
      HIPCHK(hipMemset(d.s_dbg.p, 0, 32 * 8));
    }
    HIPCHK(hipMemset(d.s_hdr.p, 0, 64));
    HIPCHK(hipMemset(d.s_changed.p, 0, 256));
    HIPCHK(hipMemset(d.s_acc.p, 0, 64 * SFFK_STAR_ACC * 8));
    d.star_inited = true;
  }
  if (cfg.record_parents) {
    d.hist_cap = std::max(d.hist_cap, 4 * ctx->store_cap + 4 * cfg.wave);
    d.s_hist.ensure(((size_t)3 * d.hist_cap + 4) * 4);
    HIPCHK(hipMemset(d.s_hist.p, 0, 16));
  }
  if (d.s_head.p) HIPCHK(hipMemset(d.s_head.p, 0, d.s_head.cap));
  std::vector<int32_t> tc((size_t)num_roots * 16, 0);
  for (int t = 0; t < num_roots; ++t) tc[(size_t)t * 16] = (int32_t)trees[t].size();
  HIPCHK(hipMemcpy(d.s_tree_cnt.p, tc.data(), tc.size() * 4, hipMemcpyHostToDevice));
}

sffk::DevForestView Forest::dev_view() const {
  const DevEngine& d = dev;
  sffk::DevForestView v{};
  v.ctrl = d.ctrl.as<sffk::DevCtrl>();
  v.parent = d.parent.as<int32_t>();
  v.d_root = d.d_root.as<double>();
  v.d_closest = d.d_closest.as<double>();
  v.iter = d.iter.as<uint32_t>();
  v.nflag = d.nflag.as<uint8_t>();
  v.frontier = d.frontier.as<int32_t>();
  v.frontier2 = d.frontier2.as<int32_t>();
  v.rm_words = d.rm_words.as<unsigned long long>();
  v.rm_pref = d.rm_pref.as<int32_t>();
  v.slot_pos = d.slot_pos.as<int32_t>();
  v.closed = d.closed.as<int32_t>();
  v.claim = d.claim.as<int32_t>();
  v.slot_node = d.slot_node.as<int32_t>();
  v.act_slot = d.act_slot.as<int32_t>();
  v.act_slot2 = d.act_slot2.as<int32_t>();
  v.w_acc = d.w_acc.as<unsigned long long>();
  v.acc_pref = d.acc_pref.as<int32_t>();
  v.w_ev = d.w_ev.as<unsigned long long>();
  v.ev_h = d.ev_h.as<unsigned long long>();
  v.ev_nb = d.ev_nb.as<int32_t>();
  v.ev_raw = d.ev_raw.as<int32_t>();
  v.ustate32 = d.ustate32.as<int32_t>();
  v.wg_pub = d.wg_pub.as<unsigned long long>();
  v.commit_seq = d.commit_seq.as<int32_t>();
  v.goal_id = cfg.has_goal ? goal_node : -1;
  {
    const sffk::GridView& g = ctx->gridv;
    if (!kn.no_order && !use_priority() && d.ord_hist.p && g.cnt && g.nx > 0 && cfg.wave >= kn.order_min_wave) {
      sffk::OrderView& o = v.ord;
      o.hist = d.ord_hist.as<int32_t>(); o.start = d.ord_start.as<int32_t>();
      o.slot_key = d.ord_key.as<int32_t>(); o.slot_rank = d.ord_rank.as<int32_t>();
      o.slot_pos = d.ord_pos.as<int32_t>();
      o.n_sub = (cfg.wave + 63) / 64;
      o.lst[0] = d.ord_lst.as<int32_t>(); o.lst[1] = o.lst[0] + (size_t)o.n_sub * 64;
      o.cnt[0] = d.ord_cnt.as<int32_t>(); o.cnt[1] = o.cnt[0] + (size_t)o.n_sub * SFFK_ORD_CNT_STRIDE;
      o.pos = ctx->spos.as<double>();
      o.ox = g.ox; o.oy = g.oy; o.oz = g.oz; o.inv_cell = g.inv_cell;
      o.nx = g.nx; o.ny = g.ny; o.nz = g.nz;
      int sh = 0;
      auto coarse = [&](int n) { return ((n - 1) >> sh) + 1; };
      while ((long long)coarse(g.nx) * coarse(g.ny) * coarse(g.nz) > SFFK_ORD_BUCKETS) ++sh;
      o.shift = sh; o.cnx = coarse(g.nx); o.cny = coarse(g.ny);
      o.n_buckets = coarse(g.nx) * coarse(g.ny) * coarse(g.nz);
    }
  }
  if (use_priority() && d.prio_heaps) {
    v.prio.n_heaps = d.prio_heaps; v.prio.cap = d.prio_cap;
    v.prio.base = d.hp_base.as<int32_t>(); v.prio.size = d.hp_size.as<int32_t>(); v.prio.v = d.hp_v.as<int32_t>();
    v.prio.key = d.hp_key.as<double>(); v.prio.pos = d.hp_pos.as<int32_t>(); v.prio.ref = d.hp_ref.as<double>();
    v.prio.slot_tree = d.slot_tree.as<int32_t>(); v.prio.slot_heap = d.slot_heap.as<int32_t>(); v.prio.slot_idx = d.slot_idx.as<int32_t>();
    v.prio.counters = d.hp_cnt.as<int32_t>(); v.prio.gen = d.hp_gen.as<int32_t>();
    v.prio.slot_word = d.slot_word.as<unsigned long long>();
    v.prio.plan = kn.prio_seq ? nullptr : d.hp_plan.as<int32_t>();
    v.prio.bias = cfg.priority_bias;
  }
  v.profile = kn.profile ? 1 : 0;
  v.qclk_sh = d.qclk_sh.as<unsigned long long>();
  v.host_status = (!kn.no_zc_status && d.h_ctrl.p) ? d.h_ctrl.as<sffk::DevCtrl>() : nullptr;
  v.kc_trace = d.kc_trace.as<unsigned long long>();
  v.kc_trace_round = kn.kc_trace;
  v.b_n1 = d.b_n1.as<int32_t>();
  v.b_n2 = d.b_n2.as<int32_t>();
  v.b_ta = d.b_ta.as<int32_t>();
  v.b_tb = d.b_tb.as<int32_t>();
  v.b_dist = d.b_dist.as<double>();
  v.bt_key = d.bt_key.as<unsigned long long>();
  v.bt_val = d.bt_val.as<unsigned long long>();
  v.bt_mask = d.bt_size - 1;
  v.pair = d.pair.as<uint8_t>();
  v.ring = d.wr.ring.as<uint64_t>();
  v.ring_mask = d.wr.ring_words - 1;
  v.node_cap = d.node_cap;
  v.border_cap = d.border_cap;
  v.wave = cfg.wave;
  v.n_trees = num_roots;
  v.words_per = cfg.dim == 2 ? 1 : 6;
  v.threshold_misses = cfg.threshold_misses;
  v.max_iterations = cfg.max_iterations;
  v.node_budget = cfg.node_budget;
  v.temp_base = d.temp_base;
  v.ulist = d.ulist.as<int32_t>();
  return v;
}

void Forest::dev_size_node_arrays() {
  Ctx& c = *ctx;
  DevEngine& d = dev;
  const int cap = c.store_cap;
  d.node_cap = cap - cfg.wave - 16;
  d.temp_base = (cap - cfg.wave - 8) & ~3;
  if (d.node_cap < 64) throw HipError{"forest: node store too small for the device engine"};
  d.parent.ensure((size_t)cap * 4);
  d.d_root.ensure((size_t)cap * 8);
  d.d_closest.ensure((size_t)cap * 8);
  d.iter.ensure((size_t)cap * 4);
  d.nflag.ensure((size_t)cap);
  d.frontier.ensure((size_t)cap * 4);
  d.frontier2.ensure((size_t)cap * 4);
  const size_t old_rm = d.rm_words.cap;
  d.rm_words.ensure(((size_t)cap / 64 + 2) * 8);
  if (d.rm_words.cap != old_rm)
    HIPCHK(hipMemsetAsync(d.rm_words.p, 0, d.rm_words.cap, c.stream));
  d.rm_pref.ensure(((size_t)cap / 64 + 2) * 4);
  d.closed.ensure((size_t)cap * 4);
  if (cfg.optimize) {
    const size_t old_head = d.s_head.cap;
    d.s_head.ensure((size_t)cap * 8);
    if (d.s_head.cap != old_head) HIPCHK(hipMemsetAsync(d.s_head.p, 0, d.s_head.cap, c.stream));
  }
  if (cfg.record_parents && d.s_hist.p && 4 * cap + 4 * cfg.wave > d.hist_cap) {
    d.hist_cap = 4 * cap + 4 * cfg.wave;
    d.s_hist.ensure(((size_t)3 * d.hist_cap + 4) * 4);
  }
  const size_t old_claim = d.claim.cap;
  d.claim.ensure((size_t)cap * 4);
  if (d.claim.cap != old_claim)
    HIPCHK(hipMemsetD32Async(reinterpret_cast<hipDeviceptr_t>(d.claim.p), 0x7fffffff, d.claim.cap / 4, c.stream));
}

void Forest::dev_size_border_arrays(int want_cap) {
  Ctx& c = *ctx;
  DevEngine& d = dev;
  if (want_cap > d.border_cap) {
    d.border_cap = want_cap;
    d.b_n1.ensure((size_t)want_cap * 4);
    d.b_n2.ensure((size_t)want_cap * 4);
    d.b_ta.ensure((size_t)want_cap * 4);
    d.b_tb.ensure((size_t)want_cap * 4);
    d.b_dist.ensure((size_t)want_cap * 8);
  }
  const uint64_t want_tab = next_pow2((uint64_t)std::max(kn.test_border_cap >= 0 ? 64 : 1 << 16, 4 * d.border_cap));
  if (want_tab > d.bt_size) {
    d.bt_size = want_tab;
    d.bt_key.release();
    d.bt_val.release();
    d.bt_key.ensure((size_t)want_tab * 8);
    d.bt_val.ensure((size_t)want_tab * 8);
    HIPCHK(hipMemsetAsync(d.bt_key.p, 0, (size_t)want_tab * 8, c.stream));
    HIPCHK(hipMemsetAsync(d.bt_val.p, 0xFF, (size_t)want_tab * 8, c.stream));
    d.table_dirty = true;
  }
}

void Forest::dev_ring_append(const uint64_t* words, size_t n) {
  DevEngine& d = dev;
  Ctx& c = *ctx;
  d.wr.append(c.copy_stream, words, &rng, n, [&](uint64_t at, size_t run) {
    if (cfg.libm_sampling) {
      double* ht = d.h_trig.as<double>() + 3 * at;
      const uint64_t* hw = d.wr.h_ring.as<uint64_t>() + at;
      const unsigned hw_threads = std::max(1u, std::min(16u, std::thread::hardware_concurrency()));
      const size_t per = (run + hw_threads - 1) / hw_threads;
      auto work = [&](size_t b, size_t e) {
        for (size_t j = b; j < e; ++j) {
          const double ang = sffg::sample_angle(hw[j]);
          ht[3 * j] = std::cos(ang);
          ht[3 * j + 1] = std::sin(ang);
          ht[3 * j + 2] = std::acos(sffg::sample_acos_arg(hw[j]));
        }
      };
      if (run < 4096 || hw_threads == 1) work(0, run);
      else {
        std::vector<std::thread> th;
        for (unsigned t = 0; t < hw_threads; ++t) {
          const size_t b = std::min(run, t * per), e = std::min(run, b + per);
          if (b < e) th.emplace_back(work, b, e);
        }
        for (auto& x : th) x.join();
      }
      HIPCHK(hipMemcpyAsync(d.trig.as<double>() + 3 * at, ht, run * 24, hipMemcpyHostToDevice, c.copy_stream));
    } else if (d.dev_trig) {
      sffk::launch_ring_trig(c.copy_stream, d.wr.ring.as<uint64_t>() + at, d.trig.as<double>() + 3 * at, (int)run);
    }
  });
}

void Forest::dev_ring_top_up(uint64_t cursor, uint64_t ahead) {
  DevEngine& d = dev;
  if (d.wr.produced >= cursor + ahead) return;
  const uint64_t need = cursor + ahead - d.wr.produced;
  if (d.wr.produced + need - cursor > d.wr.ring_words) throw HipError{"forest: engine-word ring too small (internal error)"};
  dev_ring_append(nullptr, (size_t)need);
}

void Forest::dev_upload_state() {
  Ctx& c = *ctx;
  DevEngine& d = dev;
  HIPCHK(hipSetDevice(c.device));
  const int wave = cfg.wave;
  const int words_per = cfg.dim == 2 ? 1 : 6;
  if (!d.inited) {
    HIPCHK(hipEventCreateWithFlags(&d.ev_wave, hipEventDisableTiming));
    HIPCHK(hipEventCreateWithFlags(&d.ev_wave2, hipEventDisableTiming));
    d.max_wave_words = (uint64_t)wave * ((use_priority() ? 5 : 1) + (uint64_t)std::max(1, cfg.threshold_misses) * words_per) + 64;
    uint64_t ring_words = next_pow2(std::max<uint64_t>(4 * d.max_wave_words, (uint64_t)rng_ahead.size() + 2 * d.max_wave_words + 64));
    if (cfg.wave == 1) ring_words = std::max<uint64_t>(ring_words, 1 << 18);
    d.wr.init(ring_words);
    if (cfg.libm_sampling) {
      d.trig.ensure((size_t)d.wr.ring_words * 24);
      d.h_trig.ensure((size_t)d.wr.ring_words * 24);
    } else if (cfg.wave == 1 && !kn.no_dev_trig) {
      d.trig.ensure((size_t)d.wr.ring_words * 24);
      d.dev_trig = true;
    }
    d.ctrl.ensure(sizeof(sffk::DevCtrl));
    d.h_ctrl.ensure((size_t)SFFK_STATUS_RING * sizeof(sffk::DevCtrl));
    d.slot_node.ensure((size_t)wave * 4);
    d.slot_pos.ensure((size_t)wave * 4);
    d.act_slot.ensure((size_t)wave * 4);
    d.act_slot2.ensure((size_t)wave * 4);
    d.w_acc.ensure(((size_t)wave / 64 + 2) * 8);
    d.acc_pref.ensure(((size_t)wave / 64 + 2) * 4);
    d.w_ev.ensure(((size_t)wave / 64 + 2) * 8);
    d.ev_h.ensure(((size_t)wave + 64) * 8);
    d.ev_nb.ensure(((size_t)wave + 64) * 4);
    d.ev_raw.ensure(((size_t)wave + 64) * 4);
    d.ustate32.ensure(((size_t)wave + 64) * 4);
    d.wg_pub.ensure(((size_t)wave / 64 + 2) * SFFK_PUB_WORDS * 8);
    d.commit_seq.ensure(64);
    d.qclk_sh.ensure(64 * 16 * 8);
    HIPCHK(hipMemsetAsync(d.qclk_sh.p, 0, 64 * 16 * 8, c.stream));
    d.ord_hist.ensure((size_t)SFFK_ORD_BUCKETS * 4);
    d.ord_start.ensure((size_t)SFFK_ORD_BUCKETS * 4);
    d.ord_key.ensure((size_t)wave * 4);
    d.ord_rank.ensure((size_t)wave * 4);
    d.ord_pos.ensure((size_t)wave * 4);
    {
      const size_t n_sub = ((size_t)wave + 63) / 64;
      d.ord_lst.ensure(2 * n_sub * 64 * 4);
      d.ord_cnt.ensure(2 * n_sub * SFFK_ORD_CNT_STRIDE * 4);
      HIPCHK(hipMemsetAsync(d.ord_cnt.p, 0, 2 * n_sub * SFFK_ORD_CNT_STRIDE * 4, c.stream));
    }
    HIPCHK(hipMemsetAsync(d.ord_hist.p, 0, (size_t)SFFK_ORD_BUCKETS * 4, c.stream));
    if (kn.kc_trace >= 0) {
      d.kc_trace.ensure(((size_t)wave / 64 + 2) * 64);
      HIPCHK(hipMemsetAsync(d.kc_trace.p, 0, ((size_t)wave / 64 + 2) * 64, c.stream));
    }
    HIPCHK(hipMemsetAsync(d.ustate32.p, 0, ((size_t)wave + 64) * 4, c.stream));
    HIPCHK(hipMemsetAsync(d.wg_pub.p, 0, ((size_t)wave / 64 + 2) * SFFK_PUB_WORDS * 8, c.stream));
    HIPCHK(hipMemsetAsync(d.commit_seq.p, 0, 64, c.stream));
    d.ulist.ensure((size_t)wave * 4);
    d.d_parent.ensure((size_t)wave * 4);
    d.d_parent2.ensure((size_t)wave * 4);
    d.d_force.ensure((size_t)wave);
    d.fault_pending.ensure(16);
    HIPCHK(hipMemsetAsync(d.fault_pending.p, 0, 16, c.stream));
    d.pair.ensure((size_t)num_roots * num_roots);
    d.inited = true;
  }
  c.store_reserve((int)nodes.size() + 2 * wave + 64);
  dev_size_node_arrays();
  int nb = 0;
  for (auto& kv : borders) nb += (int)kv.second.size();
  {
    int first_cap = std::max(std::max(1 << 16, 2 * (nb + wave)), cfg.node_budget > 0 ? cfg.node_budget / 10 + 2 * wave : 0);
    if (kn.test_border_cap >= 0) first_cap = std::max(nb + 1, kn.test_border_cap);
    dev_size_border_arrays(first_cap);
  }
  if (cfg.optimize) dev_star_setup();
  if (use_priority()) dev_prio_upload();
  for (int a = 0; a < 6; ++a) c.store_maxabs = std::max(c.store_maxabs, std::fabs(cfg.limits[a]));

  const int n = (int)nodes.size();
  {
    std::vector<int32_t> par(n);
    std::vector<double> dr(n), dc(n);
    std::vector<uint32_t> it(n);
    for (int i = 0; i < n; ++i) { par[i] = nodes[i].parent; dr[i] = nodes[i].d_root; dc[i] = nodes[i].d_closest; it[i] = nodes[i].iter; }
    HIPCHK(hipMemcpyAsync(d.parent.p, par.data(), (size_t)n * 4, hipMemcpyHostToDevice, c.stream));
    HIPCHK(hipMemcpyAsync(d.d_root.p, dr.data(), (size_t)n * 8, hipMemcpyHostToDevice, c.stream));
    HIPCHK(hipMemcpyAsync(d.d_closest.p, dc.data(), (size_t)n * 8, hipMemcpyHostToDevice, c.stream));
    HIPCHK(hipMemcpyAsync(d.iter.p, it.data(), (size_t)n * 4, hipMemcpyHostToDevice, c.stream));
    HIPCHK(hipMemcpyAsync(d.nflag.p, nflag.data(), (size_t)n, hipMemcpyHostToDevice, c.stream));
    if (!frontier.empty()) HIPCHK(hipMemcpyAsync(d.frontier.p, frontier.data(), frontier.size() * 4, hipMemcpyHostToDevice, c.stream));
    if (!closed.empty()) HIPCHK(hipMemcpyAsync(d.closed.p, closed.data(), closed.size() * 4, hipMemcpyHostToDevice, c.stream));
    HIPCHK(hipStreamSynchronize(c.stream));
  }
  {
    std::vector<int32_t> n1, n2, ta, tb;
    std::vector<double> ds;
    std::vector<uint8_t> pair((size_t)num_roots * num_roots, 0);
    for (auto& kv : borders)
      for (const Border& b : kv.second) {
        n1.push_back(b.n1); n2.push_back(b.n2); ta.push_back(kv.first.first); tb.push_back(kv.first.second); ds.push_back(b.dist);
        pair[(size_t)kv.first.first * num_roots + kv.first.second] = 1;
        pair[(size_t)kv.first.second * num_roots + kv.first.first] = 1;
      }
    const size_t m = n1.size();
    if (m) {
      HIPCHK(hipMemcpyAsync(d.b_n1.p, n1.data(), m * 4, hipMemcpyHostToDevice, c.stream));
      HIPCHK(hipMemcpyAsync(d.b_n2.p, n2.data(), m * 4, hipMemcpyHostToDevice, c.stream));
      HIPCHK(hipMemcpyAsync(d.b_ta.p, ta.data(), m * 4, hipMemcpyHostToDevice, c.stream));
      HIPCHK(hipMemcpyAsync(d.b_tb.p, tb.data(), m * 4, hipMemcpyHostToDevice, c.stream));
      HIPCHK(hipMemcpyAsync(d.b_dist.p, ds.data(), m * 8, hipMemcpyHostToDevice, c.stream));
    }
    HIPCHK(hipMemcpyAsync(d.pair.p, pair.data(), pair.size(), hipMemcpyHostToDevice, c.stream));
    HIPCHK(hipMemsetAsync(d.bt_key.p, 0, (size_t)d.bt_size * 8, c.stream));
    HIPCHK(hipMemsetAsync(d.bt_val.p, 0xFF, (size_t)d.bt_size * 8, c.stream));
    d.table_dirty = false;
    sffk::launch_border_rehash(c.stream, dev_view(), (int)m);
    HIPCHK(hipStreamSynchronize(c.stream));
    d.host_borders = (int)m;
  }
  {
    const uint64_t cursor = rng.draws;
    d.wr.produced = cursor;
    const size_t left = rng.qn - rng.qh;
    std::vector<uint64_t> ahead(rng.q ? rng.q + rng.qh : nullptr, rng.q ? rng.q + rng.qn : nullptr);
    rng.q = nullptr;
    rng.qh = rng.qn = 0;
    if (left) dev_ring_append(ahead.data(), std::min<size_t>(left, (size_t)d.wr.ring_words));
    if (left > d.wr.ring_words) throw HipError{"forest: look-ahead queue larger than the engine-word ring"};
    rng.draws = d.wr.produced;
    sffk::DevCtrl k{};
    k.status_seq = (int32_t)d.status_next;
    k.n_nodes = n;
    k.iter = iter;
    k.round = round;
    k.in_wave = in_wave ? 1 : 0;
    k.frontier_n = (int)frontier.size();
    k.closed_n = (int)closed.size();
    k.solved = solved ? 1 : 0;
    k.empty_frontier = empty_frontier ? 1 : 0;
    k.terminated = (!in_wave && terminated()) ? 1 : 0;
    k.halt = k.terminated;
    k.n_borders = d.host_borders;
    k.cursor = cursor;
    k.collide_calls = st.collide_calls;
    k.path_free_calls = st.path_free_calls;
    k.nn_queries = st.nn_queries;
    k.poses_executed = st.poses_executed;
    k.segments_executed = st.segments_executed;
    k.samples_executed = st.samples_executed;
    k.waves = st.waves;
    k.rounds = st.sweeps;
    k.round_nodes = st.sweep_nodes;
    k.round_queries = st.sweep_queries;
    k.star_rounds = st.star_rounds;
    k.star_passes = st.star_passes;
    k.star_members = st.star_members;
    k.star_rewires = st.star_rewires;
    k.spec_steps = st.spec_steps;
    k.spec_evaluated = st.spec_evaluated;
    k.spec_committed = st.spec_committed;
    k.epoch = 1;
    k.prio_n0 = n;
    k.prio_all_empty = (use_priority() && all_frontiers_empty()) ? 1 : 0;
    k.prio_gen = -2;
    if (in_wave && use_priority() && !slots.empty() && slots[0].tree >= 0) {
      k.prio_wave = 1;
      std::vector<int32_t> stt(slots.size()), sh(slots.size());
      for (size_t s = 0; s < slots.size(); ++s) { stt[s] = slots[s].tree; sh[s] = slots[s].heap; }
      HIPCHK(hipMemcpy(d.slot_tree.p, stt.data(), stt.size() * 4, hipMemcpyHostToDevice));
      HIPCHK(hipMemcpy(d.slot_heap.p, sh.data(), sh.size() * 4, hipMemcpyHostToDevice));
    }
    if (in_wave) {
      k.n_slots = (int)slots.size();
      k.use_closed = (!slots.empty() && slots[0].from_closed) ? 1 : 0;
      std::vector<int32_t> sn(slots.size()), sp(slots.size(), 0), act;
      std::vector<int32_t> where(nodes.size(), 0);
      for (size_t r = 0; r < frontier.size(); ++r) where[frontier[r]] = (int32_t)r;
      for (size_t s = 0; s < slots.size(); ++s) {
        sn[s] = slots[s].node;
        sp[s] = where[slots[s].node];
        if (slots[s].failing) act.push_back((int32_t)s);
      }
      k.act_cnt = (int)act.size();
      k.act_sel = 0;
      HIPCHK(hipMemcpy(d.slot_pos.p, sp.data(), sp.size() * 4, hipMemcpyHostToDevice));
      HIPCHK(hipMemcpy(d.slot_node.p, sn.data(), sn.size() * 4, hipMemcpyHostToDevice));
      if (!act.empty()) HIPCHK(hipMemcpy(d.act_slot.p, act.data(), act.size() * 4, hipMemcpyHostToDevice));
    }
    HIPCHK(hipMemcpy(d.ctrl.p, &k, sizeof k, hipMemcpyHostToDevice));
    d.last = k;
  }
  d.host_nodes = n;
  d.host_stale = false;
  d.active = true;
}

void Forest::sync_host() {
  DevEngine& d = dev;
  if (!d.active || !d.host_stale) return;
  Ctx& c = *ctx;
  HIPCHK(hipSetDevice(c.device));
  HIPCHK(hipStreamSynchronize(c.stream));
  sffk::DevCtrl k;
  HIPCHK(hipMemcpy(&k, d.ctrl.p, sizeof k, hipMemcpyDeviceToHost));
  if (cfg.optimize && d.star_inited) {
    unsigned long long acc[64 * SFFK_STAR_ACC], sum[SFFK_STAR_ACC] = {0, 0, 0, 0, 0, 0, 0, 0};
    HIPCHK(hipMemcpy(acc, d.s_acc.p, sizeof acc, hipMemcpyDeviceToHost));
    bool any = false;
    for (int j = 0; j < 64 * SFFK_STAR_ACC; ++j) { sum[j % SFFK_STAR_ACC] += acc[j]; any |= acc[j] != 0; }
    if (any) {
      k.collide_calls += sum[0]; k.path_free_calls += sum[1];
      k.star_rounds += sum[2]; k.star_passes += sum[3]; k.star_members += sum[4]; k.star_rewires += sum[5];
      HIPCHK(hipMemset(d.s_acc.p, 0, sizeof acc));
      HIPCHK(hipMemcpy(d.ctrl.p, &k, sizeof k, hipMemcpyHostToDevice));
    }
  }
  d.last = k;
  const int n = k.n_nodes, n0 = d.host_nodes;
  if (n > n0) {
    const int m = n - n0;
    std::vector<double> pos((size_t)m * 6), dr(m), dc(m);
    std::vector<int32_t> par(m), tr(m);
    std::vector<uint32_t> it(m);
    HIPCHK(hipMemcpy(pos.data(), c.spos.as<double>() + 6 * (size_t)n0, (size_t)m * 48, hipMemcpyDeviceToHost));
    HIPCHK(hipMemcpy(tr.data(), c.stree.as<int32_t>() + n0, (size_t)m * 4, hipMemcpyDeviceToHost));
    HIPCHK(hipMemcpy(par.data(), d.parent.as<int32_t>() + n0, (size_t)m * 4, hipMemcpyDeviceToHost));
    HIPCHK(hipMemcpy(dr.data(), d.d_root.as<double>() + n0, (size_t)m * 8, hipMemcpyDeviceToHost));
    HIPCHK(hipMemcpy(dc.data(), d.d_closest.as<double>() + n0, (size_t)m * 8, hipMemcpyDeviceToHost));
    HIPCHK(hipMemcpy(it.data(), d.iter.as<uint32_t>() + n0, (size_t)m * 4, hipMemcpyDeviceToHost));
    for (int j = 0; j < m; ++j) add_node(&pos[6 * (size_t)j], tr[j], par[j], dc[j], dr[j], it[j]);
  }
  if (cfg.optimize && cfg.record_parents && d.s_hist.p) {
    int32_t ctl[4];
    HIPCHK(hipMemcpy(ctl, d.s_hist.p, 16, hipMemcpyDeviceToHost));
    if (ctl[1]) hist_overflow = true;
    const int m = std::min(ctl[0], d.hist_cap);
    if (m > 0) {
      std::vector<int32_t> raw((size_t)3 * m);
      HIPCHK(hipMemcpy(raw.data(), d.s_hist.as<int32_t>() + 4, raw.size() * 4, hipMemcpyDeviceToHost));
      for (int j = 0; j < m; ++j) hist.push_back({raw[3 * (size_t)j], raw[3 * (size_t)j + 1], (uint32_t)raw[3 * (size_t)j + 2]});
      HIPCHK(hipMemset(d.s_hist.p, 0, 16));
    }
  }
  if (cfg.optimize && n0 > 0) {
    std::vector<double> dr(n0), dc(n0);
    std::vector<int32_t> par(n0);
    HIPCHK(hipMemcpy(par.data(), d.parent.p, (size_t)n0 * 4, hipMemcpyDeviceToHost));
    HIPCHK(hipMemcpy(dr.data(), d.d_root.p, (size_t)n0 * 8, hipMemcpyDeviceToHost));
    HIPCHK(hipMemcpy(dc.data(), d.d_closest.p, (size_t)n0 * 8, hipMemcpyDeviceToHost));
    for (int j = 0; j < n0; ++j) { nodes[j].parent = par[j]; nodes[j].d_root = dr[j]; nodes[j].d_closest = dc[j]; }
  }
  if (n > 0) HIPCHK(hipMemcpy(nflag.data(), d.nflag.p, (size_t)n, hipMemcpyDeviceToHost));
  frontier.resize((size_t)k.frontier_n);
  closed.resize((size_t)k.closed_n);
  if (k.frontier_n) HIPCHK(hipMemcpy(frontier.data(), k.front_sel ? d.frontier2.p : d.frontier.p, (size_t)k.frontier_n * 4, hipMemcpyDeviceToHost));
  if (k.closed_n) HIPCHK(hipMemcpy(closed.data(), d.closed.p, (size_t)k.closed_n * 4, hipMemcpyDeviceToHost));
  if (k.n_borders > d.host_borders) {
    const int b0 = d.host_borders, m = k.n_borders - b0;
    std::vector<int32_t> n1(m), n2(m), ta(m), tb(m);
    std::vector<double> ds(m);
    HIPCHK(hipMemcpy(n1.data(), d.b_n1.as<int32_t>() + b0, (size_t)m * 4, hipMemcpyDeviceToHost));
    HIPCHK(hipMemcpy(n2.data(), d.b_n2.as<int32_t>() + b0, (size_t)m * 4, hipMemcpyDeviceToHost));
    HIPCHK(hipMemcpy(ta.data(), d.b_ta.as<int32_t>() + b0, (size_t)m * 4, hipMemcpyDeviceToHost));
    HIPCHK(hipMemcpy(tb.data(), d.b_tb.as<int32_t>() + b0, (size_t)m * 4, hipMemcpyDeviceToHost));
    HIPCHK(hipMemcpy(ds.data(), d.b_dist.as<double>() + b0, (size_t)m * 8, hipMemcpyDeviceToHost));
    for (int j = 0; j < m; ++j) {
      border(ta[j], tb[j]).push_back({n1[j], n2[j], ds[j]});
      border_keys.insert(((uint64_t)(uint32_t)n1[j] << 32) | ((uint64_t)(uint32_t)n2[j] + 1));
    }
    d.host_borders = k.n_borders;
  }
  iter = k.iter;
  solved = k.solved != 0;
  empty_frontier = k.empty_frontier != 0;
  in_wave = k.in_wave != 0;
  round = k.round;
  st.collide_calls = k.collide_calls;
  st.path_free_calls = k.path_free_calls;
  st.nn_queries = k.nn_queries;
  st.poses_executed = k.poses_executed;
  st.segments_executed = k.segments_executed;
  st.samples_executed = k.samples_executed;
  if (use_priority() && kn.prio_seq) st.prio_seq_waves += k.waves - st.waves;
  st.waves = k.waves;
  st.sweeps = k.rounds;
  st.sweep_nodes = k.round_nodes;
  st.sweep_queries = k.round_queries;
  st.star_rounds = k.star_rounds;
  st.star_passes = k.star_passes;
  st.star_members = k.star_members;
  st.star_rewires = k.star_rewires;
  st.spec_steps = k.spec_steps;
  st.spec_evaluated = k.spec_evaluated;
  st.spec_committed = k.spec_committed;
  if (use_priority()) {
    dev_prio_download();
    if (in_wave)
      for (int id = std::max(k.prio_n0, 0); id < n; ++id)
        for (PHeap& hp : heaps[nodes[id].tree]) hp.push(id);
  }
  if (in_wave) {
    std::vector<int32_t> sn(k.n_slots), act((size_t)k.act_cnt);
    std::vector<uint8_t> sf(k.n_slots, 0);
    HIPCHK(hipMemcpy(sn.data(), d.slot_node.p, (size_t)k.n_slots * 4, hipMemcpyDeviceToHost));
    if (k.act_cnt) HIPCHK(hipMemcpy(act.data(), k.act_sel ? d.act_slot2.p : d.act_slot.p, (size_t)k.act_cnt * 4, hipMemcpyDeviceToHost));
    for (int32_t s : act) sf[s] = 1;
    slots.resize((size_t)k.n_slots);
    for (int s = 0; s < k.n_slots; ++s) { slots[s].node = sn[s]; slots[s].failing = sf[s] != 0; slots[s].from_closed = k.use_closed != 0; slots[s].tree = -1; slots[s].heap = -1; }
    if (use_priority() && k.prio_wave) {
      std::vector<int32_t> stt(k.n_slots), sh(k.n_slots);
      HIPCHK(hipMemcpy(stt.data(), d.slot_tree.p, (size_t)k.n_slots * 4, hipMemcpyDeviceToHost));
      HIPCHK(hipMemcpy(sh.data(), d.slot_heap.p, (size_t)k.n_slots * 4, hipMemcpyDeviceToHost));
      for (int s = 0; s < k.n_slots; ++s) { slots[s].tree = stt[s]; slots[s].heap = sh[s]; slots[s].from_closed = false; }
    }
  }
  if (cfg.has_goal && batch_eligible() && !in_wave) max_connected();
  c.store_n = n;
  c.grid_inserted = n;
  d.host_nodes = n;
  d.host_stale = false;
}

void Forest::dev_to_host() {
  DevEngine& d = dev;
  exchange_timer_drop();
  if (!d.active) return;
  d.host_stale = true;
  sync_host();
  Ctx& c = *ctx;
  HIPCHK(hipStreamSynchronize(c.copy_stream));
  const uint64_t cursor = d.last.cursor;
  const size_t left = (size_t)(d.wr.produced - cursor);
  const size_t keep = std::max(rng_ahead.size(), left + 16);
  std::vector<uint64_t> buf(keep, 0);
  const uint64_t* hr = d.wr.h_ring.as<uint64_t>();
  for (size_t j = 0; j < left; ++j) buf[j] = hr[(cursor + j) & (d.wr.ring_words - 1)];
  rng_ahead.swap(buf);
  rng.q = rng_ahead.data();
  rng.qh = 0;
  rng.qn = left;
  rng.draws = cursor;
  d.active = false;
}

struct DevRoundBufs {
  int n, CAP, NBCAP, STRIDE, list_cap;
  double *d_pos, *d_pd;
// ... 120 lines not shown
  P.dv.force_out = d.d_force.as<uint8_t>();
  P.dv.qclk = reinterpret_cast<unsigned long long*>(reinterpret_cast<char*>(d.ctrl.p) + offsetof(sffk::DevCtrl, q_t0));
  P.dv.qclk_sh = d.qclk_sh.as<unsigned long long>();
  P.dv.ord = V.ord;
  P.node_pos = c.spos.as<double>();
  P.n = B.n;
  P.dist = F.cfg.sampling_dist;
  P.dim = F.cfg.dim;
  P.out6 = B.d_pos;
  P.in_lim = B.d_lim;
  P.parent_dist = B.d_pd;
  P.queries = c.r_q.as<sffk::SweepQuery>();
  P.q_max_base = d.temp_base;
  return P;
}

void Forest::dev_enqueue_round_eval(void* send_dev, bool sample) {
  Ctx& c = *ctx;
  DevEngine& d = dev;
  const sffk::DevForestView V = dev_view();
  const DevRoundBufs B = dev_round_bufs(*this);
  const int n = B.n;
  const int32_t* dev_n = reinterpret_cast<const int32_t*>(d.ctrl.p);
  c.timing_on = d.force_timing >= 0 ? d.force_timing != 0
                                   : (kn.timer_stride <= 1 || d.rounds_enqueued % (uint64_t)kn.timer_stride == 0);
  d.round_timing = c.timing_on;
  c.round_scope = true;
  ++d.rounds_enqueued;
  if (sample) {
    const sffk::SampleLaunch P = dev_sample_launch(*this, B);
    c.time_begin(T_SAMPLE);
    sffk::launch_sample_steer(c.stream, P);
    c.time_end();
  }
  int32_t* const round_parent = (d.round_parity ? d.d_parent2 : d.d_parent).as<int32_t>();
  unsigned long long* const qclk = reinterpret_cast<unsigned long long*>(reinterpret_cast<char*>(d.ctrl.p) + offsetof(sffk::DevCtrl, q_t0));
  sffk::ClassifyArgs ca{};
  ca.n = n; ca.N0 = d.temp_base; ca.cap = B.CAP; ca.nbcap = B.NBCAP; ca.rank = cfg.rank; ca.world = cfg.world;
  ca.goal_id = cfg.has_goal ? goal_node : -1;
  ca.wide = query_wide ? 1 : 0;
  ca.lazy_nb = (cfg.world <= 1 && !cfg.optimize) ? 1 : 0;
  ca.qrec = c.r_qrec.as<sffk::QRec>();
  ca.dist_tree = cfg.dist_tree;
  ca.newpos = B.d_pos;
  ca.in_lim = B.d_lim;
  ca.pdist = B.d_pd;
  ca.parent = round_parent;
  ca.center = c.r_center.as<double>();
  ca.force = d.d_force.as<uint8_t>();
  ca.cnt = c.r_cnt.as<int32_t>();
  ca.hit_idx = nullptr;
  ca.hit_dist = nullptr;
  ca.tree = c.stree.as<int32_t>();
  ca.pos = c.spos.as<double>();
  ca.rec_flags = B.d_rec;
  ca.rec_nnb = ca.rec_flags + n;
  ca.rec_nb = ca.rec_nnb + n;
  ca.rec_meta = ca.rec_nb + (size_t)n * B.NBCAP;
  ca.seg_a = c.r_sega.as<double>();
  ca.seg_b = c.r_segb.as<double>();
  ca.seg_ns = B.seg_ns;
  ca.first_hit = B.first_hit;
  ca.seg_ovf = B.seg_ovf;
  ca.ctrl = B.d_rctrl;
  ca.dev_n = dev_n;
  ca.qclk = qclk;
  ca.qclk_sh = d.qclk_sh.as<unsigned long long>();
  if (V.ord.hist) {
    ca.ord_valid = reinterpret_cast<const int32_t*>(reinterpret_cast<char*>(d.ctrl.p) + offsetof(sffk::DevCtrl, ord_valid));
    ca.ord_nslots = reinterpret_cast<const int32_t*>(reinterpret_cast<char*>(d.ctrl.p) + offsetof(sffk::DevCtrl, n_slots));
    ca.ord_sel = reinterpret_cast<const int32_t*>(reinterpret_cast<char*>(d.ctrl.p) + offsetof(sffk::DevCtrl, act_sel));
    for (int q = 0; q < 2; ++q) { ca.ord_lst[q] = V.ord.lst[q]; ca.ord_cnt[q] = V.ord.cnt[q]; }
  }
  c.time_begin(T_SWEEP);
  ca.items = c.r_items.p;
  ca.items_cap = B.list_cap;
  ca.sub = c.r_sub.as<int32_t>();
  ca.pose_hit = B.d_pose;
  const bool blocked = sffk::launch_query_classify(c.stream, kn, c.gridv, &c.tgridv, c.store_view(), c.r_q.as<sffk::SweepQuery>(), ca, &c.envv);
  c.time_end();
  c.time_begin(T_COLLIDE);
  sffk::TempGridRef tref{c.tgridv, c.sx.as<float>() + d.temp_base, c.sy.as<float>() + d.temp_base,
                         c.sz.as<float>() + d.temp_base, n};
  sffk::TempGridRef tref_keep = tref;
  tref_keep.tg = sffk::GridView{};
  tref_keep.n = 0;
  sffk::launch_collide_items(c.stream, kn, c.envv, c.robv, B.d_pos, n, ca.rec_flags, B.d_pose, ca.seg_a, ca.seg_b, ca.seg_ns,
                             B.STRIDE, ca.ctrl, c.r_items.p, ca.items_cap, ca.sub, ca.first_hit, ca.seg_ovf,
                             cfg.optimize ? &tref_keep : &tref, dev_n, blocked ? &ca : nullptr);
  c.time_end();
  if (send_dev) {
    c.time_begin(T_EXCHANGE);
    sffk::launch_pack_records(c.stream, dev_resolve_args(*this, B), cfg.rank, cfg.world, n, static_cast<int32_t*>(send_dev));
    exchange_timer_drop();
    exchange_open = c.timed_now;
    if (exchange_open) { exchange_t = c.pending.back(); c.pending.pop_back(); }
  }
  c.timing_on = true;
  c.round_scope = false;
}

void Forest::dev_enqueue_round_commit(const void* recv_dev, bool sample_next) {
  Ctx& c = *ctx;
  const DevRoundBufs B = dev_round_bufs(*this);
  const sffk::ResolveArgs ra = dev_resolve_args(*this, B);
  if (recv_dev) {
    sffk::launch_unpack_records(c.stream, ra, cfg.rank, cfg.world, B.n, static_cast<const int32_t*>(recv_dev));
    if (exchange_open) {
      HIPCHK(hipEventRecord(exchange_t.b, c.stream));
      c.pending.push_back(exchange_t);
      exchange_open = false;
    }
  }
  sffk::SampleLaunch next{};
  if (sample_next) {
    dev.round_parity ^= 1;
    next = dev_sample_launch(*this, dev_round_bufs(*this));
    dev.round_parity ^= 1;
  }
  c.round_scope = true;
  c.timing_on = dev.round_timing;
  c.time_begin(T_COMMIT);
  if (cfg.optimize) {
    sffk::StarLaunch sl{};
    sl.g = c.gridv;
    sl.tg = c.tgridv;
    sl.st = c.store_view();
    sl.env = c.envv;
    sl.rob = c.robv;
    sl.cell_edge = c.grid_cell;
    sl.slack = 8 * c.sweep_eps();
    sl.cube_reach = 2.0 * cfg.sampling_dist;
    sl.passes = kn.test_star_passes;
    sl.tail = kn.star_tail ? 1 : 0;
    sl.tail_wgs = kn.star_tail_wgs;
    sl.tail_stall = kn.test_star_stall;
    sl.knn_lone = kn.star_knn == Knobs::STAR_KNN_LONE;
    sl.seg_blocks = kn.seg_blocks;
    sffk::launch_commit(c.stream, ra, B.n, &sl, sample_next ? &next : nullptr);
  } else {
    sffk::launch_commit(c.stream, ra, B.n, nullptr, sample_next ? &next : nullptr);
  }
  c.time_end();
  c.timing_on = true;
  c.round_scope = false;
}

void Forest::dev_enqueue_end(int slot) {
  Ctx& c = *ctx;
  DevEngine& d = dev;
  if (use_priority()) sffk::launch_prio_end(c.stream, dev_view(), c.store_view());
  sffk::launch_wave_end(c.stream, dev_view(), c.gridv.ovf_cnt, c.tgridv.ovf_cnt,
                        cfg.optimize ? d.s_acc.as<unsigned long long>() : nullptr);
  d.status_copied[slot] = kn.no_zc_status;
  if (!kn.no_zc_status) d.status_of[slot] = d.status_next++;
  else HIPCHK(hipMemcpyAsync(d.h_ctrl.as<sffk::DevCtrl>() + slot, d.ctrl.p, sizeof(sffk::DevCtrl), hipMemcpyDeviceToHost, c.stream));
  HIPCHK(hipEventRecord(slot ? d.ev_wave2 : d.ev_wave, c.stream));
}

uint64_t Forest::dev_launch_signature() {
  Ctx& c = *ctx;
  uint64_t x = 1469598103934665603ULL;
  auto mix = [&](const void* p, size_t n) {
    const unsigned char* q = static_cast<const unsigned char*>(p);
    for (size_t i = 0; i < n; ++i) { x ^= q[i]; x *= 1099511628211ULL; }
  };
  for (int parity = 0; parity < 2; ++parity) {
    dev.round_parity = parity;
    const DevRoundBufs B = dev_round_bufs(*this);
    const sffk::ResolveArgs ra = dev_resolve_args(*this, B);
    mix(&B, sizeof B);
    mix(&ra, sizeof ra);
  }
  dev.round_parity = 0;
  mix(&c.gridv, sizeof c.gridv);
  mix(&c.tgridv, sizeof c.tgridv);
  mix(&c.envv, sizeof c.envv);
  mix(&c.robv, sizeof c.robv);
  const void* ptrs[] = {c.r_q.p, c.r_cnt.p, c.r_sega.p, c.r_segb.p, c.r_items.p, c.r_sub.p, c.r_out.p, c.r_center.p, c.r_qrec.p, dev.d_parent.p, dev.d_force.p,
                        dev.ctrl.p, dev.wr.ring.p, dev.trig.p, c.sx.p, c.spos.p, c.stree.p};
  mix(ptrs, sizeof ptrs);
  const double scal[] = {c.sweep_eps(), c.grid_cell, cfg.sampling_dist, cfg.dist_tree};
  mix(scal, sizeof scal);
  const int ints[] = {cfg.threshold_misses, kn.test_star_passes, cfg.wave, c.store_cap, dev.temp_base, kn.test_hitcap, kn.test_nbcap, query_wide ? 1 : 0};
  mix(ints, sizeof ints);
  return x ? x : 1;
}

void Forest::dev_enqueue_wave_kernels(bool sharded, size_t words) {
  sffk::launch_wave_begin(ctx->stream, dev_view());
  const int R = std::max(1, cfg.threshold_misses);
  const bool fuse = !kn.no_fused_sample;
  for (int r = 0; r < R; ++r) {
    dev.round_parity = fuse ? (r & 1) : 0;
    dev_enqueue_round_eval(sharded ? x_send.p : nullptr, !fuse || r == 0);
    if (sharded) ctx->rccl_all_gather_i32(x_send.p, x_recv.p, words);
    dev_enqueue_round_commit(sharded ? x_recv.p : nullptr, fuse && r + 1 < R);
  }
  dev.round_parity = 0;
  if (use_priority()) sffk::launch_prio_end(ctx->stream, dev_view(), ctx->store_view());
  sffk::launch_wave_end(ctx->stream, dev_view(), ctx->gridv.ovf_cnt, ctx->tgridv.ovf_cnt,
                        cfg.optimize ? dev.s_acc.as<unsigned long long>() : nullptr);
}

void Forest::dev_enqueue_wave(int slot) {
  Ctx& c = *ctx;
  DevEngine& d = dev;
  grid_dense();
  c.round_grid();
  d.wr.wait_on(c.stream);
  const bool self_exchange = kn.test_exchange_self;
  const bool sharded = cfg.world > 1 || (self_exchange && (ctx->rccl_comm != nullptr || ctx->xchg_fn != nullptr));
  size_t words = 0;
  if (sharded) {
    words = dev_exchange_bytes() / 4;
    x_send.ensure(words * 4);
    x_recv.ensure(words * 4 * (size_t)cfg.world);
  }
  const bool timed_wave = kn.timer_stride <= 1 || d.waves_enqueued % (uint64_t)kn.timer_stride == 0;
  ++d.waves_enqueued;
  const bool use_graph = d.graph_enabled && !sharded && !timed_wave;
  if (use_graph) {
    const uint64_t sig = dev_launch_signature();
    if (!d.wave_graph || sig != d.wave_graph_sig) {
      if (d.wave_graph) { (void)hipGraphExecDestroy(d.wave_graph); d.wave_graph = nullptr; }
      uint64_t before[T_KINDS];
      for (int k = 0; k < T_KINDS; ++k) before[k] = c.round_calls[k];
      d.force_timing = 0;
      HIPCHK(hipStreamBeginCapture(c.stream, hipStreamCaptureModeRelaxed));
      hipGraph_t g = nullptr;
      try {
        dev_enqueue_wave_kernels(false, 0);
      } catch (...) {
        (void)hipStreamEndCapture(c.stream, &g);
        if (g) (void)hipGraphDestroy(g);
        d.force_timing = -1;
        throw;
      }
      d.force_timing = -1;
      HIPCHK(hipStreamEndCapture(c.stream, &g));
      HIPCHK(hipGraphInstantiate(&d.wave_graph, g, nullptr, nullptr, 0));
      (void)hipGraphDestroy(g);
      for (int k = 0; k < T_KINDS; ++k) {
        d.graph_calls[k] = c.round_calls[k] - before[k];
        c.round_calls[k] = before[k];
        c.kernel_calls[k] -= d.graph_calls[k];
      }
      d.rounds_enqueued -= (uint64_t)std::max(1, cfg.threshold_misses);
      d.wave_graph_sig = sig;
      ++d.graph_captures;
    }
    HIPCHK(hipGraphLaunch(d.wave_graph, c.stream));
    for (int k = 0; k < T_KINDS; ++k) { c.round_calls[k] += d.graph_calls[k]; c.kernel_calls[k] += d.graph_calls[k]; }
    d.rounds_enqueued += (uint64_t)std::max(1, cfg.threshold_misses);
    ++d.graph_launches;
  } else {
    d.force_timing = d.graph_enabled && !sharded ? 1 : -1;
    dev_enqueue_wave_kernels(sharded, words);
    d.force_timing = -1;
  }
  d.status_copied[slot] = kn.no_zc_status;
  if (!kn.no_zc_status) d.status_of[slot] = d.status_next++;
  else HIPCHK(hipMemcpyAsync(d.h_ctrl.as<sffk::DevCtrl>() + slot, d.ctrl.p, sizeof(sffk::DevCtrl), hipMemcpyDeviceToHost, c.stream));
  HIPCHK(hipEventRecord(slot ? d.ev_wave2 : d.ev_wave, c.stream));
  dev.host_stale = true;
}

int Forest::dev_finish_wave(double* wait_ms, int slot, bool stream_idle) {
  Ctx& c = *ctx;
  DevEngine& d = dev;
  {
    auto tw = Clock::now();
    HIPCHK(hipEventSynchronize(slot ? d.ev_wave2 : d.ev_wave));
    if (stream_idle) c.sync();
    if (wait_ms) *wait_ms += ms_since(tw);
  }
  if (!d.status_copied[slot]) {
    d.last = d.h_ctrl.as<sffk::DevCtrl>()[d.status_of[slot] & (SFFK_STATUS_RING - 1)];
    if ((uint32_t)d.last.status_seq != d.status_of[slot])
      throw HipError{"device engine: the wave's status block is not the one expected (sequence " + std::to_string(d.last.status_seq) +
                     ", expected " + std::to_string(d.status_of[slot]) + ")"};
  } else {
    d.last = d.h_ctrl.as<sffk::DevCtrl>()[slot];
  }
  if (!stream_idle) return d.last.fault;
  d.host_stale = true;
  const sffk::DevCtrl& s = d.last;
  const bool prof = kn.profile;
  const auto t_ev = Clock::now();
  if (s.fault) {
    const int fault = s.fault;
    if (fault == SFFK_FAULT_INTERNAL) throw HipError{"device engine: a workgroup of the commit waited in vain for a lower one's word"};
    if (fault == SFFK_FAULT_LISTS) return fault;
    if (fault == SFFK_FAULT_CAPACITY) {
      if (s.n_nodes + cfg.wave > d.node_cap - 8) {
        c.store_reserve(std::max(c.store_cap * 2, s.n_nodes + 4 * cfg.wave + 64));
        dev_size_node_arrays();
        if (use_priority()) dev_prio_regrow();
      }
      if (s.n_borders + cfg.wave > d.border_cap) dev_size_border_arrays(2 * (s.n_borders + cfg.wave));
    } else if (fault == SFFK_FAULT_BORDER_TABLE) {
      dev_size_border_arrays(std::max(4 * d.border_cap, 2 * (s.n_borders + cfg.wave)));
    } else if (fault == SFFK_FAULT_PRIO_REDRAW) {
      throw HipError{"forest: a priority-frontier draw fell into the rejection zone of the uniform-int algorithm (probability ~ heap size / 2^64); run this forest with SFFGPU_PRIO_SEQ=1"};
    } else {
      throw HipError{"forest: unknown device fault"};
    }
    if (d.table_dirty) {
      sffk::launch_border_rehash(c.stream, dev_view(), s.n_borders);
      d.table_dirty = false;
    }
    int32_t clear[2] = {0, 0};
    HIPCHK(hipMemcpyAsync(reinterpret_cast<char*>(d.ctrl.p) + offsetof(sffk::DevCtrl, fault), &clear[0], 4, hipMemcpyHostToDevice, c.stream));
    HIPCHK(hipMemcpyAsync(reinterpret_cast<char*>(d.ctrl.p) + offsetof(sffk::DevCtrl, halt), &clear[1], 4, hipMemcpyHostToDevice, c.stream));
    HIPCHK(hipStreamSynchronize(c.stream));
    d.last.fault = 0;
    d.last.halt = 0;
    if (prof) fprintf(stderr, "[sffgpu host event] wave %llu: growth fault %d handled in %.2f ms (%d nodes, %d borders)\n",
                      (unsigned long long)s.waves, fault, ms_since(t_ev), s.n_nodes, s.n_borders);
    return 0;
  }
  if (s.grid_ovf > c.gridv.ovf_cap || s.tgrid_ovf > c.tgridv.ovf_cap)
    throw HipError{"neighbour grid overflow list exhausted during a wave (nodes were dropped)"};
  if (s.grid_ovf > c.grid_rebuild_at()) {
    c.store_n = s.n_nodes;
    c.grid_inserted = s.n_nodes;
    c.grid_check();
    if (prof) fprintf(stderr, "[sffgpu host event] wave %llu: node grid re-celled in %.2f ms (%d nodes, overflow list %d, cell %.3f)\n",
                      (unsigned long long)s.waves, ms_since(t_ev), s.n_nodes, s.grid_ovf, c.grid_cell);
  }
  return 0;
}

void Forest::exchange_timer_drop() {
  if (!exchange_open) return;
  ctx->pool.push_back(exchange_t.a);
  ctx->pool.push_back(exchange_t.b);
  exchange_open = false;
}

void Forest::on_list_fault() { query_wide = true; }

bool Forest::dev_wave_begin() {
  if (!dev.on) throw HipError{"forest: the device engine does not drive this forest"};
  HIPCHK(hipSetDevice(ctx->device));
  exchange_timer_drop();
  grid_dense();
  ctx->round_grid();
  if (!dev.active) dev_upload_state();
  const sffk::DevCtrl& k = dev.last;
  if (!k.in_wave && k.terminated) return false;
  dev_ring_top_up(k.cursor, 2 * dev.max_wave_words);
  dev_enqueue_begin();
  dev.host_stale = true;
  return true;
}

bool Forest::batch_eligible() const {
  if (cfg.has_goal && use_priority()) return dev.on && kn.prio_goal_loop && cfg.wave == 1 && cfg.world == 1 && num_roots <= 64;
  if (cfg.has_goal && !kn.goal_loop) return false;
  return dev.on && cfg.wave == 1 && cfg.world == 1 && num_roots <= 64 && (!use_priority() || kn.prio_loop);
}
bool Forest::seq_eligible() const { return batch_eligible() && !kn.no_seq && !seq_suspended; }

static const size_t SPEC_HEAD = 4096;
bool Forest::spec_setup() {
  DevEngine& d = dev;
  if (d.spec_off || use_priority() || cfg.has_goal) return false;
  const int TM = std::max(1, cfg.threshold_misses);
  if (d.spec_n_sc > 0 && d.spec_tm == TM) return true;
  if (TM > 8) { d.spec_off = true; return false; }
  const int depth = std::max(1, std::min(kn.spec_depth > 0 ? kn.spec_depth : (cfg.optimize ? 4 : 3), SFFK_SPEC_DEPTH));
  const int sets = std::max(1, std::min(kn.spec_sets, 4));
  struct Sc { int level; int out[SFFK_SPEC_DEPTH]; int anc[SFFK_SPEC_DEPTH]; int child[9]; };
  std::vector<Sc> tab;
  Sc root{};
  for (int& v : root.child) v = -1;
  tab.push_back(root);
  for (size_t i = 0; i < tab.size(); ++i) {
    if (tab[i].level + 1 >= depth) continue;
    for (int o = cfg.optimize ? TM : 0; o <= TM; ++o) {
      if ((tab.size() + 1) * (size_t)TM * (size_t)sets * (cfg.optimize ? 3 : 2) + 3 > 960) break;
      Sc ch = tab[i];
      ch.level = tab[i].level + 1;
      ch.out[tab[i].level] = o;
      ch.anc[tab[i].level] = (int)i;
      for (int& v : ch.child) v = -1;
      tab[i].child[o] = (int)tab.size();
      tab.push_back(ch);
    }
  }
  std::vector<int32_t> flat(tab.size() * SFFK_SPEC_TAB, 0);
  for (size_t i = 0; i < tab.size(); ++i) {
    int32_t* t = flat.data() + i * SFFK_SPEC_TAB;
    t[0] = tab[i].level;
    for (int l = 0; l < SFFK_SPEC_DEPTH; ++l) { t[1 + l] = tab[i].out[l]; t[1 + SFFK_SPEC_DEPTH + l] = tab[i].anc[l]; }
    for (int o = 0; o < 9; ++o) t[1 + 2 * SFFK_SPEC_DEPTH + o] = tab[i].child[o];
  }
  d.spec_tab.ensure(flat.size() * 4);
  HIPCHK(hipMemcpy(d.spec_tab.p, flat.data(), flat.size() * 4, hipMemcpyHostToDevice));
  d.spec_n_sc = (int)tab.size();
  d.spec_sets = sets;
  d.spec_tm = TM;
  d.spec_area.ensure(SPEC_HEAD + (size_t)sets * d.spec_n_sc * TM * (SFFK_SPEC_REC * 8 + 8) + 2048);
  return true;
}

uint64_t Forest::seq_words_per_wave() const {
  return (uint64_t)(8 + (use_priority() ? 2 * num_roots : 0) + std::max(1, cfg.threshold_misses) * (cfg.dim == 2 ? 1 : 6));
}
void Forest::seq_note_launch(uint64_t waves_before) {
  DevEngine& d = dev;
  if (!use_priority()) return;
  const sffk::DevCtrl& k = d.last;
  if (k.waves == waves_before && !k.fault && !k.terminated) d.seq_pick_slack = std::min<uint64_t>(std::max<uint64_t>(64, 2 * d.seq_pick_slack), d.wr.ring_words / 4);
  else d.seq_pick_slack = 0;
}

int Forest::seq_launch_waves(int waves_left) const {
  const uint64_t per_wave = seq_words_per_wave();
  int batch = (int)std::min<uint64_t>(4096, dev.wr.ring_words / (2 * per_wave));
  if (waves_left > 0) batch = std::min(batch, waves_left);
  return batch;
}

uint64_t Forest::seq_words_end(int batch) const {
  return dev.last.cursor + (uint64_t)batch * seq_words_per_wave() + 16 + dev.seq_pick_slack;
}

sffk::SeqArgs Forest::seq_prepare(int batch) {
  Ctx& c = *ctx;
  DevEngine& d = dev;
  dev_ring_top_up(d.last.cursor, seq_words_end(batch) - d.last.cursor);
  sffk::SeqArgs a{};
  a.f = dev_view();
  a.st = sffk::NodeStoreMut{c.sx.as<float>(), c.sy.as<float>(), c.sz.as<float>(), c.syaw.as<float>(),
                            c.spitch.as<float>(), c.sroll.as<float>(), c.stree.as<int32_t>(), c.spos.as<double>()};
  a.g = c.gridv;
  a.env = c.envv;
  a.rob = c.robv;
  memcpy(a.limits, cfg.limits, sizeof a.limits);
  a.dist_tree = cfg.dist_tree;
  a.sampling_dist = cfg.sampling_dist;
  a.sweep_abs_eps = c.sweep_eps();
  a.trig = (cfg.libm_sampling || d.dev_trig) ? d.trig.as<double>() : nullptr;
  a.words_end = d.wr.produced;
  a.grid_ovf_src = c.gridv.ovf_cnt;
  a.dim = cfg.dim;
  a.max_waves = batch;
  a.hit_cap = kn.test_hitcap;
  a.grid_ovf_limit = c.grid_rebuild_at();
  a.optimize = cfg.optimize ? 1 : 0;
  if (cfg.optimize) {
    const sffk::StarView sv = star_view();
    a.ktab = sv.ktab;
    a.tree_cnt = sv.tree_cnt;
    a.hist = sv.hist;
    a.hist_ctl = sv.hist_ctl;
    a.hist_cap = sv.hist_cap;
    a.cell_edge = c.grid_cell;
    a.knn_slack = 8 * c.sweep_eps();
  }
  return a;
}

void Forest::grid_dense() {
  Ctx& c = *ctx;
  if (!c.grid_compact) return;
  if (dev.active) {
    c.store_n = dev.last.n_nodes;
    c.grid_inserted = dev.last.n_nodes;
  }
  c.grid_dense();
}

void Forest::seq_lists_fault() {
  ++st.host_fallback_waves;
  dev_to_host();
  while (in_wave) {
    round_begin();
    int32_t cnt = (int32_t)records.size();
    round_commit(records.data(), cnt, &cnt, 1);
  }
  on_list_fault();
  dev_upload_state();
}

void Forest::run_device_seq(int max_waves) {
  Ctx& c = *ctx;
  DevEngine& d = dev;
  HIPCHK(hipSetDevice(c.device));
  auto t0 = Clock::now();
  double wait_ms = 0;
  if (!d.active) dev_upload_state();
  const uint64_t w0 = d.last.waves;
  while (true) {
    const sffk::DevCtrl& k = d.last;
    if (!k.in_wave && k.terminated) break;
    if (max_waves > 0 && !k.in_wave && (int)(k.waves - w0) >= max_waves) break;
    if (k.in_wave) {
      seq_suspended = true;
      st.total_ms += ms_since(t0);
      st.host_ms += ms_since(t0) - wait_ms;
      run_device(1);
      seq_suspended = false;
      t0 = Clock::now();
      wait_ms = 0;
      continue;
    }
    const int batch = seq_launch_waves(max_waves > 0 ? max_waves - (int)(k.waves - w0) : 0);
    const bool spec = spec_setup();
    if (spec) grid_dense();
    sffk::SeqArgs a = seq_prepare(batch);
    d.wr.wait_on(c.stream);
    const char* trace_path = kn.seq_trace.empty() ? nullptr : kn.seq_trace.c_str();
    DevBuf trace_buf;
    if (trace_path) {
      trace_buf.ensure((size_t)batch * 32);
      HIPCHK(hipMemsetAsync(trace_buf.p, 0xff, (size_t)batch * 32, c.stream));
      a.trace = trace_buf.as<int32_t>();
      a.trace_cap = batch;
    }
    const uint64_t waves_before = k.waves;
    if (spec) {
      sffk::SpecArgs sa{};
      sa.q = a;
      sa.sc_tab = d.spec_tab.as<int32_t>();
      sa.n_sc = d.spec_n_sc;
      sa.tm = d.spec_tm;
      sa.n_slots = d.spec_n_sc * d.spec_tm;
      sa.n_sets = d.spec_sets;
      sa.base = d.spec_area.as<unsigned long long>();
      sa.cur_step = reinterpret_cast<int32_t*>(d.spec_area.as<uint8_t>() + SPEC_HEAD - 256);
      sa.rec = reinterpret_cast<unsigned long long*>(d.spec_area.as<uint8_t>() + SPEC_HEAD);
      sa.timeout_ticks = 20000000ULL;
      sa.pipeline = kn.spec_pipe ? 1 : 0;
      if (kn.test_spec_stall && st.spec_steps == 0 && d.last.spec_steps == 0) sa.test_stall = kn.test_spec_stall;
      const size_t rec_bytes = (size_t)sa.n_sets * sa.n_slots * SFFK_SPEC_REC * 8;
      if (kn.profile) sa.hb = reinterpret_cast<unsigned long long*>(d.spec_area.as<uint8_t>() + SPEC_HEAD + rec_bytes);
      HIPCHK(hipMemsetAsync(d.spec_area.p, 0, d.spec_area.cap, c.stream));
      sffk::launch_spec_waves(c.stream, sa);
    } else {
      d.h_seq.ensure(sizeof a);
      d.seq_args.ensure(sizeof a);
      *d.h_seq.as<sffk::SeqArgs>() = a;
      HIPCHK(hipMemcpyAsync(d.seq_args.p, d.h_seq.p, sizeof a, hipMemcpyHostToDevice, c.stream));
      const int kind = seq_kind();
      HIPCHK(sffk::launch_seq_waves_batch(c.stream, d.seq_args.as<sffk::SeqArgs>(), 1, (kind & 1) != 0, (kind & 2) != 0, (kind & 4) != 0,
                                          sffk::collide_lds_bytes(a.rob.n_tri, 1)));
    }
    HIPCHK(hipMemcpyAsync(d.h_ctrl.as<sffk::DevCtrl>(), d.ctrl.p, sizeof(sffk::DevCtrl), hipMemcpyDeviceToHost, c.stream));
    d.status_copied[0] = true;
    HIPCHK(hipEventRecord(d.ev_wave, c.stream));
    d.host_stale = true;
    const int fault = dev_finish_wave(&wait_ms, 0, true);
    seq_note_launch(waves_before);
    if (trace_path) {
      const size_t nw = (size_t)(d.last.waves - waves_before);
      std::vector<int32_t> tr(nw * 8);
      if (nw) HIPCHK(hipMemcpy(tr.data(), trace_buf.p, nw * 32, hipMemcpyDeviceToHost));
      if (FILE* fp = fopen(trace_path, "ab")) { fwrite(tr.data(), 4, tr.size(), fp); fclose(fp); }
      trace_buf.release();
    }
    if (spec && kn.profile) {
      const int nw = d.spec_sets * d.spec_n_sc * d.spec_tm;
      unsigned long long wq[22];
      HIPCHK(hipMemcpy(wq, d.spec_area.as<uint8_t>() + SPEC_HEAD + (size_t)nw * SFFK_SPEC_REC * 8 + ((size_t)nw + 64) * 8, sizeof wq, hipMemcpyDeviceToHost));
      const unsigned long long* wp = wq + 1;
      const double n = (double)std::max<unsigned long long>(1, wq[0]) * 100.0;
      fprintf(stderr, "[sffgpu k_spec_waves worker us per ACCEPTED attempt, this launch] control block -> scenario + node %.2f | node data + words %.2f sample %.2f "
              "pose %.2f parent edge %.2f neighbour query %.2f neighbour loop %.2f | SFF*: k %.2f k nearest %.2f choose parent %.2f rewire + record %.2f (%llu attempts)\n",
              wp[0] / n, wp[5] / n, wp[6] / n, wp[1] / n, wp[2] / n, wp[3] / n, wp[4] / n, wp[8] / n, wp[9] / n, wp[10] / n, wp[7] / n, wq[0]);
      if (wq[20]) fprintf(stderr, "   k nearest searches: %llu, per search: shells %.2f count groups %.2f item batches %.2f insertions %.2f overflow-list entries %.1f\n", wq[20],
                          (double)wq[16] / wq[20], (double)wq[17] / wq[20], (double)wq[18] / wq[20], (double)wq[19] / wq[20], (double)wq[21] / wq[20]);
    }
    if (spec && d.last.spec_stalled) {
      d.spec_off = true;
      if (kn.profile) {
        fprintf(stderr, "[sffgpu k_spec_waves] a record did not arrive: back to the single wavefront (k_seq_waves_batch)\n");
        const int nw = d.spec_sets * d.spec_n_sc * d.spec_tm;
        std::vector<unsigned long long> hb((size_t)nw + 8 + 34);
        HIPCHK(hipMemcpy(hb.data(), d.spec_area.as<uint8_t>() + SPEC_HEAD + (size_t)nw * SFFK_SPEC_REC * 8, hb.size() * 8, hipMemcpyDeviceToHost));
        fprintf(stderr, "  leader waited at step %llu scenario %llu attempt %llu set %llu; granules seen:", hb[nw], hb[nw + 1], hb[nw + 2], hb[nw + 3]);
        for (int q = 0; q < 34; ++q) fprintf(stderr, " %llx", hb[nw + 8 + q]);
        fprintf(stderr, "\n  workers (step:phase):");
        for (int w = 0; w < nw; ++w) fprintf(stderr, " %llu:%llu", hb[w] >> 8, hb[w] & 255);
        fprintf(stderr, "\n");
      }
    }
    if (fault == SFFK_FAULT_LISTS) seq_lists_fault();
  }
  st.total_ms += ms_since(t0);
  st.host_ms += ms_since(t0) - wait_ms;
  if (kn.profile && d.last.spec_steps > 0) {
    const sffk::DevCtrl& k = d.last;
    const double sp = (double)k.spec_steps;
    fprintf(stderr, "[sffgpu k_spec_waves leader us/step] publish %.2f first record of the first wave %.2f of the later waves %.2f other records %.2f accepted node %.2f "
            "closed list + termination %.2f erases %.2f other %.2f | %llu steps, %.2f iterations/step, %.2f evaluated/committed\n",
            k.wprof[0] / sp / 100.0, k.wprof[1] / sp / 100.0, k.wprof[7] / sp / 100.0, k.wprof[2] / sp / 100.0, k.wprof[3] / sp / 100.0, k.wprof[4] / sp / 100.0,
            k.wprof[5] / sp / 100.0, k.wprof[6] / sp / 100.0, (unsigned long long)k.spec_steps, (double)k.spec_committed / sp,
            (double)k.spec_evaluated / (double)std::max<uint64_t>(1, k.spec_committed));
  } else if (kn.profile) {
    const sffk::DevCtrl& k = d.last;
    const double it = (double)std::max(1, k.iter);
    fprintf(stderr, "[sffgpu k_seq_waves us/iteration] pick + node %.2f sample %.2f pose %.2f parent edge %.2f neighbour query %.2f "
            "neighbour loop %.2f append %.2f wave end %.2f | %d iterations\n", k.wprof[0] / it / 100.0, k.wprof[1] / it / 100.0,
            k.wprof[2] / it / 100.0, k.wprof[3] / it / 100.0, k.wprof[4] / it / 100.0, k.wprof[5] / it / 100.0, k.wprof[6] / it / 100.0,
            k.wprof[7] / it / 100.0, k.iter);
  }
}

void Forest::run_device(int max_waves) {
  if (seq_eligible()) { run_device_seq(max_waves); return; }
  if (use_priority() && cfg.has_goal) {
    dev_to_host();
    while (in_wave) {
      round_begin();
      int32_t cnt = (int32_t)records.size();
      round_commit(records.data(), cnt, &cnt, 1);
    }
    dev_upload_state();
    return;
  }
  Ctx& c = *ctx;
  DevEngine& d = dev;
  HIPCHK(hipSetDevice(c.device));
  auto t0 = Clock::now();
  double wait_ms = 0;
  if (!d.active) dev_upload_state();
  const uint64_t w0 = d.last.waves;
  need_host_exchange = false;
  const bool ahead_ok = !kn.no_wave_ahead;
  int slot = 0;
  bool have_next = false;
  uint64_t started = 0;
  while (true) {
    const sffk::DevCtrl& k = d.last;
    if (!have_next) {
      if (!k.in_wave) {
        if (k.terminated) break;
        if (max_waves > 0 && (int)(k.waves - w0) >= max_waves) break;
      }
      dev_ring_top_up(k.cursor, d.max_wave_words);
      dev_enqueue_wave(slot);
      started = 1;
    } else {
      have_next = false;
    }
    const bool room = max_waves <= 0 || (int)(k.waves - w0) + (int)started + 1 <= max_waves;
    if (ahead_ok && room && !k.fault) {
      dev_ring_top_up(k.cursor, 2 * d.max_wave_words);
      dev_enqueue_wave(1 - slot);
      have_next = true;
    } else {
      dev_ring_top_up(k.cursor, 2 * d.max_wave_words);
    }
    int fault = dev_finish_wave(&wait_ms, slot, !have_next);
    const sffk::DevCtrl& s1 = d.last;
    const bool needs_host = fault != 0 || s1.terminated || s1.grid_ovf > c.grid_rebuild_at() || s1.tgrid_ovf > c.tgridv.ovf_cap;
    if (have_next && needs_host) {
      fault = dev_finish_wave(&wait_ms, 1 - slot, true);
      have_next = false;
      started = 0;
    } else if (have_next) {
      slot = 1 - slot;
      started = 1;
      continue;
    } else {
      started = 0;
    }
    if (fault == SFFK_FAULT_LISTS && cfg.world > 1) {
      ++st.host_fallback_waves;
      dev_to_host();
      on_list_fault();
      need_host_exchange = true;
      break;
    }
    if (fault == SFFK_FAULT_LISTS) {
      ++st.host_fallback_waves;
      dev_to_host();
      const bool whole_wave = kn.fallback_whole_wave;
      do {
        round_begin();
        int32_t cnt = (int32_t)records.size();
        round_commit(records.data(), cnt, &cnt, 1);
      } while (in_wave && whole_wave);
      on_list_fault();
      dev_upload_state();
    }
  }
  st.total_ms += ms_since(t0);
  st.host_ms += ms_since(t0) - wait_ms;
  if (kn.profile) {
    int32_t why[4] = {0, 0, 0, 0};
    HIPCHK(hipMemcpy(why, dev.fault_pending.p, 16, hipMemcpyDeviceToHost));
    {
      unsigned long long pd[16];
      sffk::debug_counters_prio(pd);
      if (pd[0]) fprintf(stderr, "[sffgpu prio heap 0] pops %llu, us per pop %.2f (first loads %.2f), windows per pop %.2f, us per window load %.2f, walk %.2f\n",
                         pd[0], pd[1] * 0.01 / pd[0], pd[2] * 0.01 / pd[0], (double)pd[3] / pd[0], pd[4] * 0.01 / (pd[3] ? pd[3] : 1), pd[5] * 0.01 / (pd[3] ? pd[3] : 1));
      if (pd[0]) fprintf(stderr, "[sffgpu prio heap 0, wave ends] new nodes pushed %llu (gather %.1f ms, pushes %.1f ms) | slot operations %llu, %llu of them removals (gather %.1f ms, apply %.1f ms)\n",
                         pd[6], pd[7] * 1e-5, pd[8] * 1e-5, pd[9], pd[12], pd[10] * 1e-5, pd[11] * 1e-5);
    }
    fprintf(stderr, "[sffgpu samples that sent their round to the host path] hit / neighbour list overflow %d, triangle candidate list %d, walk past a cut neighbour record %d | host fallback waves %llu\n",
            why[1], why[2], why[3], (unsigned long long)st.host_fallback_waves);
  }
  if (kn.profile) {
    const sffk::DevCtrl& k = d.last;
    {
      const double w = (double)std::max<unsigned long long>(1ULL, k.wprof[7]);
      fprintf(stderr, "[sffgpu us/wave, last workgroup] k_wave_begin %.1f\n", k.wprof[6] / w / 100.0);
    }
    if (d.s_dbg.p) {
      unsigned long long g[32];
      HIPCHK(hipMemcpy(g, d.s_dbg.p, sizeof g, hipMemcpyDeviceToHost));
      const double w = (double)std::max<unsigned long long>(1ULL, g[0]);
      if (g[0] && !g[9])
        fprintf(stderr, "[sffgpu k_star_knn_wg per accepted sample] us: store search %.1f earlier samples of the round %.1f lists %.1f | longest sample %.1f | samples %llu\n",
                g[1] / w / 100.0, g[3] / w / 100.0, g[4] / w / 100.0, g[7] / 100.0, g[0]);
      if (g[0] && g[9]) {
        fprintf(stderr, "[sffgpu k_star_knn per accepted sample] us: cube %.1f shells %.1f mates %.1f lists %.1f | longest %.1f | shells walked %.2f "
                "(samples beyond the cube %.3f) cube candidates %.0f | samples %llu\n", g[1] / w / 100.0, g[2] / w / 100.0, g[3] / w / 100.0,
                g[4] / w / 100.0, g[7] / 100.0, g[5] / w, g[8] / w, g[6] / w, g[0]);
        fprintf(stderr, "[sffgpu k_star_knn cube phase] us: counts %.1f items+distances %.1f bisection %.1f sort+rest %.1f\n", g[9] / w / 100.0,
                g[10] / w / 100.0, g[11] / w / 100.0, g[12] / w / 100.0);
      }
      if (g[16]) {
        const double n = (double)g[16], ps = (double)std::max<unsigned long long>(1ULL, g[17]);
        fprintf(stderr, "[sffgpu k_star_tail, workgroup 0] launches that ran passes %llu, passes each %.2f | us per pass: pass phase %.1f exact phase %.1f "
                "barriers: counting in %.1f waiting for the others %.1f\n", g[16], g[17] / n, g[18] / ps / 100.0, g[19] / ps / 100.0, g[20] / ps / 100.0,
                g[21] / ps / 100.0);
        if (g[24]) fprintf(stderr, "[sffgpu k_star_tail, sections of a sample's pass (STAR_PASS_TRACE build)] us: first loads %.1f views %.1f evaluate %.1f (of it requests %.1f) "
                           "loops %.1f writes %.1f\n", g[24] / ps / 100.0, g[25] / ps / 100.0, (g[26] + g[27]) / ps / 100.0, g[27] / ps / 100.0, g[28] / ps / 100.0, g[29] / ps / 100.0);
      }
    }
    const double r = (double)std::max<unsigned long long>(1ULL, k.prof[6]);
    if (d.kc_trace.p) {
      const size_t nw = (size_t)cfg.wave / 64 + 2;
      std::vector<unsigned long long> tr(nw * 8);
      HIPCHK(hipMemcpy(tr.data(), d.kc_trace.p, nw * 64, hipMemcpyDeviceToHost));
      unsigned long long t0 = ~0ULL;
      size_t used = 0;
      for (size_t w = 0; w < nw; ++w) if (tr[8 * w]) { t0 = std::min(t0, tr[8 * w]); used = w + 1; }
      static const char* names[8] = {"start", "walk done", "count published", "stamps posted", "lower counts in (ids)", "lower stamps in", "lower owned counts in", "end"};
      for (int k = 0; k < 8 && used; ++k) {
        std::vector<double> v;
        for (size_t w = 0; w < used; ++w) if (tr[8 * w + k]) v.push_back((double)(tr[8 * w + k] - t0) / 100.0);
        if (v.empty()) continue;
        std::vector<double> sv = v;
        std::sort(sv.begin(), sv.end());
        fprintf(stderr, "[sffgpu k_commit trace, %zu workgroups] %-24s us after the first start: min %.1f median %.1f max %.1f | first wg %.1f last wg %.1f\n",
                used, names[k], sv.front(), sv[sv.size() / 2], sv.back(), v.front(), v.back());
      }
    }
    fprintf(stderr, "[sffgpu k_commit us/commit, last workgroup] walks + waits for earlier samples %.1f (%.2f polls, max %llu) "
            "lower workgroups' counts %.1f borders %.1f | control block (%s) %.1f | dependent/round %.0f | "
            "border events with a neighbour accepted in the same round %llu, in a lower workgroup %llu\n", k.prof[0] / r / 100.0, k.prof[5] / r,
            (unsigned long long)k.prof[7], k.prof[1] / r / 100.0, k.prof[2] / r / 100.0,
            cfg.optimize ? "in k_commit" : "finalize block of the append launch", k.prof[3] / r / 100.0,
            (double)k.n_unsettled / r, (unsigned long long)(k.prof[4] & 0xffffffffULL), (unsigned long long)(k.prof[4] >> 32));
#ifdef SFFK_CI_TRACE
    {
      std::vector<unsigned long long> tr(4096 * 8);
      sffk::debug_ci_trace(tr.data());
      unsigned long long t0 = ~0ULL, tend = 0;
      for (int w = 0; w < 4096; ++w) if (tr[8 * w]) { t0 = std::min(t0, tr[8 * w]); tend = std::max(tend, tr[8 * w + 7]); }
      struct It { double start, broad, end; int nc, smp, items, wave; double entry, pre; };
      std::vector<It> its;
      int waves = 0, n_pose_items = 0;
      double pose_us = 0, pose_max = 0;
      for (int w = 0; w < 4096; ++w) {
        if (!tr[8 * w]) continue;
        ++waves;
        { const unsigned long long pp = tr[8 * w + 6] >> 8; n_pose_items += (int)(pp & 0xff); pose_us += (double)(pp >> 8) / 100.0; if ((pp & 0xff) && (double)(pp >> 8) / 100.0 > pose_max) pose_max = (double)(pp >> 8) / 100.0; tr[8 * w + 6] &= 0xff; }
        if (!tr[8 * w + 6]) continue;
        its.push_back({(tr[8 * w + 1] - t0) / 100.0, tr[8 * w + 2] >= tr[8 * w + 1] ? (tr[8 * w + 2] - t0) / 100.0 : -1.0, (tr[8 * w + 3] - t0) / 100.0,
                       (int)tr[8 * w + 4], (int)(tr[8 * w + 5] & 0xff), (int)tr[8 * w + 6], w, (tr[8 * w] - t0) / 100.0, ((tr[8 * w + 5] >> 8) - t0) / 100.0});
      }
      std::sort(its.begin(), its.end(), [](const It& a, const It& b) { return a.end > b.end; });
      fprintf(stderr, "[sffgpu k_collide_items trace] %d waves, %zu with items, kernel %.1f us (first start -> last end)\n", waves, its.size(), (tend - t0) / 100.0);
      for (size_t k = 0; k < its.size() && k < 12; ++k)
        fprintf(stderr, "  wave %4d: entry %.1f preamble done %.1f | items %d | first item: start %.1f broad done %.1f end %.1f us | candidates %d masked samples %d\n",
                its[k].wave, its[k].entry, its[k].pre, its[k].items, its[k].start, its[k].broad, its[k].end, its[k].nc, its[k].smp);
      {
        std::vector<double> e, p, st, en;
        for (const It& i : its) { e.push_back(i.entry); p.push_back(i.pre); st.push_back(i.start); en.push_back(i.end); }
        auto q = [](std::vector<double> v, double f) { std::sort(v.begin(), v.end()); return v.empty() ? 0.0 : v[(size_t)(f * (v.size() - 1))]; };
        fprintf(stderr, "  entry min/med/max %.1f %.1f %.1f | preamble done %.1f %.1f %.1f | first item start %.1f %.1f %.1f | end %.1f %.1f %.1f\n",
                q(e, 0), q(e, .5), q(e, 1), q(p, 0), q(p, .5), q(p, 1), q(st, 0), q(st, .5), q(st, 1), q(en, 0), q(en, .5), q(en, 1));
      }
      double sum_b = 0, sum_n = 0; int nb = 0;
      for (const It& i : its) if (i.broad >= 0) { sum_b += i.broad - i.start; sum_n += i.end - i.broad; ++nb; }
      if (nb) fprintf(stderr, "  first items with a broad phase: %d, avg broad %.1f us, avg after-broad %.1f us\n", nb, sum_b / nb, sum_n / nb);
      fprintf(stderr, "  pose items: %d, avg %.1f us, longest per wave %.1f us\n", n_pose_items, n_pose_items ? pose_us / n_pose_items : 0.0, pose_max);
    }
#endif
#ifdef SFFK_DEBUG_COUNTERS
    unsigned long long g[16];
    sffk::debug_counters(g);
    const double items = (double)std::max<unsigned long long>(1ULL, g[1]);
    fprintf(stderr, "[sffgpu exact kernel, per masked chunk] chunks %llu (with work %llu, with candidates %llu) flushes %.2f "
            "candidates %.1f | us: setup %.2f hierarchy %.2f narrow %.2f | per wave total %.1f us over %llu waves\n",
            g[0], g[1], g[2], g[3] / items, g[7] / items, g[4] / items / 100.0, g[5] / items / 100.0, g[6] / items / 100.0,
            (double)g[8] / (double)std::max<unsigned long long>(1ULL, g[9]) / 100.0, g[9]);
    fprintf(stderr, "[sffgpu exact kernel, narrow phase per chunk with candidates] us: staging %.2f culls %.2f exact steps %.2f (the rest: pair formation) | "
            "touching (sample, candidate) pairs %.2f\n", g[10] / 100.0 / (double)std::max<unsigned long long>(1ULL, g[2]),
            g[11] / 100.0 / (double)std::max<unsigned long long>(1ULL, g[2]), g[13] / 100.0 / (double)std::max<unsigned long long>(1ULL, g[2]),
            (double)g[14] / (double)std::max<unsigned long long>(1ULL, g[2]));
    unsigned long long q[16];
    sffk::debug_counters_query(q);
    const double qw = (double)std::max<unsigned long long>(1ULL, q[0]);
    fprintf(stderr, "[sffgpu query kernel, per sampled wave] us: grid scan %.2f classify %.2f cull %.2f (flushes %.2f) | live %.2f "
            "pairs/live %.1f survivors/live %.2f\n", q[1] / qw / 100.0, q[2] / qw / 100.0, q[3] / qw / 100.0, q[4] / qw / 100.0,
            q[7] / qw, (double)q[5] / (double)std::max<unsigned long long>(1ULL, q[7]),
            (double)q[6] / (double)std::max<unsigned long long>(1ULL, q[7]));
    fprintf(stderr, "[sffgpu block query kernel] us per sampled workgroup: samples %.2f | cells+lists %.2f | 2nd list %.2f | exact %.2f | classify %.2f | cull %.2f | flush %.2f\n",
            q[1] / qw / 100.0, q[2] / qw / 100.0, q[3] / qw / 100.0, q[4] / qw / 100.0, q[5] / qw / 100.0, q[6] / qw / 100.0, q[7] / qw / 100.0);
    fprintf(stderr, "[sffgpu block query kernel] shader clock over the sampled workgroups' lifetimes: %.0f MHz (lifetime %.2f us)\n",
            100.0 * (double)q[10] / (double)std::max<unsigned long long>(1ULL, q[11]), q[11] / qw / 100.0);
#endif
  }
}

}
```

### space_filling_forest_star_amd/csrc/knobs.cpp

```cpp
#include "knobs.h"

#include <algorithm>
#include <climits>
#include <cstdlib>
#include <cstring>

namespace sff {
namespace {

bool is_set(const char* name) { return getenv(name) != nullptr; }
bool flag(const char* name, bool dflt) {
  const char* e = getenv(name);
  return e ? atoi(e) != 0 : dflt;
}
int int_in(const char* name, int dflt, int lo = INT_MIN, int hi = INT_MAX) {
  const char* e = getenv(name);
  return e ? std::min(hi, std::max(lo, atoi(e))) : dflt;
}
double double_min(const char* name, double dflt, double lo) {
  const char* e = getenv(name);
  return e ? std::max(lo, atof(e)) : dflt;
}
bool is(const char* name, const char* word) {
  const char* e = getenv(name);
  return e && !strcmp(e, word);
}

}

Knobs Knobs::from_env() {
  Knobs k;
  k.timer_stride = int_in("SFFGPU_TIMER_STRIDE", k.timer_stride, 1);
  k.profile = is_set("SFFGPU_PROFILE");
  k.no_cand = flag("SFFGPU_NO_CAND", k.no_cand);
  k.no_clearance = flag("SFFGPU_NO_CLEARANCE", k.no_clearance);
  k.clear_cells = double_min("SFFGPU_CLEAR_CELLS", k.clear_cells, 512.0);
  k.clear_hdiv = double_min("SFFGPU_CLEAR_HDIV", k.clear_hdiv, 0.5);
  k.no_trigrid = flag("SFFGPU_NO_TRIGRID", k.no_trigrid);
  k.tg_div = double_min("SFFGPU_TG_DIV", k.tg_div, 1.0);
  k.test_grid_bk = int_in("SFFGPU_TEST_GRID_BK", k.test_grid_bk, 1, 8);
  k.test_grid_bkmax = int_in("SFFGPU_TEST_GRID_BKMAX", k.test_grid_bkmax, 1, 64);
  k.test_grid_ovf = int_in("SFFGPU_TEST_GRID_OVF", k.test_grid_ovf);
  k.compact_grid = flag("SFFGPU_COMPACT_GRID", k.compact_grid);
  k.test_grid_pool = int_in("SFFGPU_TEST_GRID_POOL", k.test_grid_pool, 1, 1 << 26);

  k.query = is("SFFGPU_QUERY", "wide") ? QUERY_WIDE : is("SFFGPU_QUERY", "block") ? QUERY_BLOCK : QUERY_AUTO;
  k.share = is_set("SFFGPU_SHARE") ? (flag("SFFGPU_SHARE", false) ? 1 : 0) : -1;
  k.seg_blocks = int_in("SFFGPU_SEG_BLOCKS", k.seg_blocks, 1, 4096);
  k.cull_blocks = int_in("SFFGPU_CULL_BLOCKS", k.cull_blocks);
  k.seg_listcap = int_in("SFFGPU_SEG_LISTCAP", k.seg_listcap);
  k.star_knn = is("SFFGPU_STAR_KNN", "lone") ? STAR_KNN_LONE : STAR_KNN_WG;

  k.engine = is("SFFGPU_ENGINE", "host") ? ENGINE_HOST : is("SFFGPU_ENGINE", "device") ? ENGINE_DEVICE : ENGINE_AUTO;
  k.prio_device = flag("SFFGPU_PRIO_DEVICE", k.prio_device);
  k.prio_seq = flag("SFFGPU_PRIO_SEQ", k.prio_seq);
  k.prio_loop = flag("SFFGPU_PRIO_LOOP", k.prio_loop);
  k.goal_loop = flag("SFFGPU_GOAL_LOOP", k.goal_loop);
  k.prio_goal_loop = flag("SFFGPU_PRIO_GOAL_LOOP", k.prio_goal_loop);
  k.no_order = flag("SFFGPU_NO_ORDER", k.no_order);
  k.order_min_wave = int_in("SFFGPU_ORDER_MIN_WAVE", k.order_min_wave, 2);
  k.test_hitcap = int_in("SFFGPU_TEST_HITCAP", k.test_hitcap, 1, 64);
  k.test_nbcap = int_in("SFFGPU_TEST_NBCAP", k.test_nbcap, 1);
  k.test_star_passes = int_in("SFFGPU_TEST_STAR_PASSES", k.test_star_passes, 1);
  k.test_exchange_self = is_set("SFFGPU_TEST_EXCHANGE_SELF");
  k.star_tail = flag("SFFGPU_STAR_TAIL", k.star_tail);
  k.star_tail_wgs = int_in("SFFGPU_STAR_TAIL_WGS", k.star_tail_wgs, 1);
  k.test_star_stall = int_in("SFFGPU_TEST_STAR_STALL", k.test_star_stall, 0);
  k.test_star_items = int_in("SFFGPU_TEST_STAR_ITEMS", k.test_star_items);
  k.test_border_cap = int_in("SFFGPU_TEST_BORDER_CAP", k.test_border_cap);
  k.no_graph = is_set("SFFGPU_NO_GRAPH") ? (flag("SFFGPU_NO_GRAPH", false) ? 1 : 0) : -1;
  {
    const char* pre = getenv("LD_PRELOAD");
    k.profiler_preloaded = pre && strstr(pre, "rocprofiler");
  }
  k.no_wave_ahead = is_set("SFFGPU_NO_WAVE_AHEAD");
  k.no_fused_sample = flag("SFFGPU_NO_FUSED_SAMPLE", k.no_fused_sample);
  k.no_zc_status = flag("SFFGPU_NO_ZC_STATUS", k.no_zc_status);
  k.fallback_whole_wave = is_set("SFFGPU_FALLBACK_WHOLE_WAVE");
  k.kc_trace = int_in("SFFGPU_KC_TRACE", k.kc_trace);
  k.digest = is_set("SFFGPU_DIGEST");
  k.no_seq = flag("SFFGPU_NO_SEQ", k.no_seq);
  k.spec = flag("SFFGPU_SPEC", k.spec);
  k.spec_depth = int_in("SFFGPU_SPEC_DEPTH", k.spec_depth);
  k.spec_sets = int_in("SFFGPU_SPEC_SETS", k.spec_sets);
  k.spec_pipe = flag("SFFGPU_SPEC_PIPE", k.spec_pipe);
  k.test_spec_stall = int_in("SFFGPU_TEST_SPEC_STALL", k.test_spec_stall);
  k.no_dev_trig = flag("SFFGPU_NO_DEV_TRIG", k.no_dev_trig);
  if (const char* e = getenv("SFFGPU_SEQ_TRACE")) k.seq_trace = e;

  k.rrt_chain = flag("SFFGPU_RRT_CHAIN", k.rrt_chain);
  k.rrt_fork = flag("SFFGPU_RRT_FORK", k.rrt_fork);
  k.rrt_repair = flag("SFFGPU_RRT_REPAIR", k.rrt_repair);
  k.rrt_dry = flag("SFFGPU_RRT_DRY", k.rrt_dry);
  k.rrt_one_chain = flag("SFFGPU_RRT_ONE_CHAIN", k.rrt_one_chain);
  k.rrt_split = int_in("SFFGPU_RRT_SPLIT", k.rrt_split, 1);
  k.rrt_small = int_in("SFFGPU_RRT_SMALL", k.rrt_small, 1);
  k.rrt_grow = int_in("SFFGPU_RRT_GROW", k.rrt_grow, 100);
  k.rrt_no_grid = is_set("SFFGPU_RRT_NO_GRID");
  k.rrt_no_chain_conn = is_set("SFFGPU_RRT_NO_CHAIN_CONN");
  k.lazy_batch = flag("SFFGPU_LAZY_BATCH", k.lazy_batch);

  k.smooth_loop = flag("SFFGPU_SMOOTH_LOOP", k.smooth_loop);
  k.smooth_edges = int_in("SFFGPU_SMOOTH_EDGES", k.smooth_edges, 1);
  return k;
}

}
```

### space_filling_forest_star_amd/csrc/knobs.h

```cpp
#pragma once
#include <string>

namespace sff {

struct Knobs {
  enum Engine { ENGINE_AUTO, ENGINE_HOST, ENGINE_DEVICE };
  enum Query { QUERY_AUTO, QUERY_WIDE, QUERY_BLOCK };
  enum StarKnn { STAR_KNN_WG, STAR_KNN_LONE };

  int timer_stride = 32;
  bool profile = false;
  bool no_cand = false;
  bool no_clearance = false;
  double clear_cells = 134217728.0;
  double clear_hdiv = 2.0;
  bool no_trigrid = false;
  double tg_div = 3.0;
  int test_grid_bk = 8;
  int test_grid_bkmax = 64;
  int test_grid_ovf = -1;
  bool compact_grid = false;
  int test_grid_pool = 0;

  Query query = QUERY_AUTO;
  int share = -1;
  int seg_blocks = 0;
  int cull_blocks = 2048;
  int seg_listcap = -1;
  StarKnn star_knn = STAR_KNN_WG;

  Engine engine = ENGINE_AUTO;
  bool prio_device = true;
  bool prio_seq = false;
  bool prio_loop = false;
  bool goal_loop = false;
  bool prio_goal_loop = false;
  bool no_order = false;
  int order_min_wave = 4096;
  int test_hitcap = 64;
  int test_nbcap = 15;
  int test_star_passes = 0;
  bool test_exchange_self = false;
  bool star_tail = true;
  int star_tail_wgs = 0;
  int test_star_stall = 0;
  int test_star_items = -1;
  int test_border_cap = -1;
  int no_graph = -1;
  bool profiler_preloaded = false;
  bool no_wave_ahead = false;
  bool no_fused_sample = false;
  bool no_zc_status = false;
  bool fallback_whole_wave = false;
  int kc_trace = -1;
  bool digest = false;
  bool no_seq = false;
  bool spec = true;
  int spec_depth = 0;
  int spec_sets = 1;
  bool spec_pipe = true;
  int test_spec_stall = 0;
  bool no_dev_trig = false;
  std::string seq_trace;

  bool rrt_chain = true;
  bool rrt_fork = true;
  bool rrt_repair = true;
  bool rrt_dry = true;
  bool rrt_one_chain = true;
  int rrt_split = 2;
  int rrt_small = 48;
  int rrt_grow = 150;
  bool rrt_no_grid = false;
  bool rrt_no_chain_conn = false;
  bool lazy_batch = false;

  bool smooth_loop = false;
  int smooth_edges = 64;

  static Knobs from_env();
};

}
```

Baseline: 12.10 million.

## Recycle device engine buffers across forests and bound RNG word top-ups by wave size

When a Forest is destroyed, its device engine buffers, pinned buffers and events are handed to the context as a spare instead of being freed. The next forest adopts them, marking each buffer stale so a larger request reallocates without copying old contents, and forces the required memsets on first use. Engine-word top-ups are now sized from the actual node count per wave rather than the worst-case wave size, which cuts host RNG generation in early waves. A new check throws if a wave consumed words that were never produced, and start-up timing instrumentation is added. The cost is memory that stays held between forests, and stale data in recycled buffers is a correctness risk.

```diff
diff --git a/space_filling_forest_star_amd/csrc/engine.cpp b/space_filling_forest_star_amd/csrc/engine.cpp
--- a/space_filling_forest_star_amd/csrc/engine.cpp
+++ b/space_filling_forest_star_amd/csrc/engine.cpp
@@ -18,8 +18,28 @@
 }
 #define HIPCHK(x) hip_check((x), #x)
 
+AllocClock& alloc_clock() {
+  static thread_local AllocClock c;
+  return c;
+}
+namespace {
+struct AllocTimer {
+  std::chrono::steady_clock::time_point t0 = std::chrono::steady_clock::now();
+  ~AllocTimer() {
+    AllocClock& c = alloc_clock();
+    c.ms += std::chrono::duration<double, std::milli>(std::chrono::steady_clock::now() - t0).count();
+    ++c.n;
+  }
+};
+}
+
 void DevBuf::ensure(size_t bytes) {
-  if (bytes <= cap) return;
+  if (bytes <= cap) {
+    stale = false;
+    return;
+  }
+  AllocTimer timer;
+  if (stale) release();
   size_t want = std::max(bytes, cap * 2);
   want = (want + 255) & ~(size_t)255;
   void* np = nullptr;
@@ -35,9 +55,15 @@
   if (p) (void)hipFree(p);
   p = nullptr;
   cap = 0;
+  stale = false;
 }
 void PinBuf::ensure(size_t bytes) {
-  if (bytes <= cap) return;
+  if (bytes <= cap) {
+    stale = false;
+    return;
+  }
+  AllocTimer timer;
+  if (stale) release();
   size_t want = std::max(bytes, cap * 2);
   void* np = nullptr;
   HIPCHK(hipHostMalloc(&np, want, hipHostMallocDefault));
@@ -52,9 +78,10 @@
   if (p) (void)hipHostFree(p);
   p = nullptr;
   cap = 0;
+  stale = false;
 }
 void WordRing::init(uint64_t words) {
-  HIPCHK(hipEventCreateWithFlags(&ev_ring, hipEventDisableTiming));
+  if (!ev_ring) HIPCHK(hipEventCreateWithFlags(&ev_ring, hipEventDisableTiming));
   ring_words = words;
   ring.ensure((size_t)words * 8);
   h_ring.ensure((size_t)words * 8);
@@ -261,6 +288,7 @@
                     &seg_job[1].b, &seg_job[1].c, &seg_job[2].ids, &seg_job[2].a, &seg_job[2].b, &seg_job[2].c, &seg_job[3].ids, &seg_job[3].a,
                     &seg_job[3].b, &seg_job[3].c, &sm_dev};
   for (DevBuf* b : bufs) b->release();
+  spare_drop();
   env.reset();
   PinBuf* pins[] = {&h_a, &h_b, &h_c, &h_d, &h_e, &h_f, &h_g, &h_h, &p_in, &p_out, &rr_hq, &rr_hout, &seg_job[0].hids, &seg_job[0].hc, &seg_job[1].hids, &seg_job[1].hc, &seg_job[2].hids, &seg_job[2].hc,
                     &seg_job[3].hids, &seg_job[3].hc, &sm_pin};
@@ -799,6 +827,7 @@
   out->other_bytes = sum({&d_a, &d_b, &d_c, &d_d, &d_e, &d_f, &d_g, &d_h, &sm_dev, &r_in, &r_out, &r_q, &r_cnt, &r_sega, &r_segb,
                           &r_items, &r_items2, &r_sub, &r_center, &r_qrec, &r_out2, &rr_q1, &rr_q2, &rr_a, &rr_out, &rr_sq, &rr_np, &rr_alt, &rr_q2b, &rr_sqb});
   for (const SegJob& J : seg_job) out->other_bytes += sum({&J.ids, &J.a, &J.b, &J.c});
+  if (spare) out->other_bytes += (uint64_t)spare->device_bytes();
   out->total_bytes = out->env_bytes + out->store_bytes + out->grid_bytes + out->round_grid_bytes + out->other_bytes;
 }
 void Ctx::grid_insert_new() {
diff --git a/space_filling_forest_star_amd/csrc/engine.h b/space_filling_forest_star_amd/csrc/engine.h
--- a/space_filling_forest_star_amd/csrc/engine.h
+++ b/space_filling_forest_star_amd/csrc/engine.h
@@ -23,9 +23,16 @@
 };
 void hip_check(hipError_t e, const char* what);
 
+struct AllocClock {
+  double ms = 0;
+  int n = 0;
+};
+AllocClock& alloc_clock();
+
 struct DevBuf {
   void* p = nullptr;
   size_t cap = 0;
+  bool stale = false;
   void ensure(size_t bytes);
   void release();
   template <class T> T* as() const { return reinterpret_cast<T*>(p); }
@@ -33,6 +40,7 @@
 struct PinBuf {
   void* p = nullptr;
   size_t cap = 0;
+  bool stale = false;
   void ensure(size_t bytes);
   void release();
   template <class T> T* as() const { return reinterpret_cast<T*>(p); }
@@ -111,6 +119,8 @@
   ~EnvBlock();
 };
 
+struct DevSpare;
+
 struct Ctx {
   int device = 0;
   Knobs kn;
@@ -180,6 +190,8 @@
   DevBuf r_qrec;
   DevBuf r_out2;
   PinBuf p_in, p_out;
+  std::unique_ptr<DevSpare> spare;
+  void spare_drop();
 
   struct Timed { hipEvent_t a, b; int kind; bool round; };
   std::vector<Timed> pending;
@@ -341,6 +353,23 @@
   PinBuf h_seq;
   DevBuf seq_args;
   uint64_t seq_pick_slack = 0;
+  uint64_t slot_words = 0;
+  uint64_t produced_at[2] = {0, 0};
+  struct Start {
+    double alloc_ms = 0, upload_ms = 0, words_ms[2] = {0, 0}, capture_ms = 0, instantiate_ms = 0, wait0_ms = 0;
+    uint64_t words[2] = {0, 0};
+    int allocations = 0, adopted = 0, top_ups = 0;
+    bool wave0_waited = false, printed = false;
+  } start;
+  static const std::vector<DevBuf DevEngine::*>& dev_bufs();
+  static const std::vector<PinBuf DevEngine::*>& pin_bufs();
+};
+
+struct DevSpare {
+  DevEngine e;
+  DevBuf x_send, x_recv;
+  size_t device_bytes() const;
+  void release();
 };
 
 struct Forest {
@@ -357,6 +386,9 @@
   void dev_ring_append(const uint64_t* words, size_t n);
   void dev_ring_top_up(uint64_t cursor, uint64_t ahead);
   void dev_upload_state();
+  void dev_adopt_spare();
+  uint64_t dev_waves_words(int n_waves) const;
+  void dev_start_report();
   void dev_to_host();
   void dev_enqueue_begin();
   void dev_enqueue_round_eval(void* send_dev, bool sample = true);
diff --git a/space_filling_forest_star_amd/csrc/forest.cpp b/space_filling_forest_star_amd/csrc/forest.cpp
--- a/space_filling_forest_star_amd/csrc/forest.cpp
+++ b/space_filling_forest_star_amd/csrc/forest.cpp
@@ -279,31 +279,68 @@
   *out = s;
 }
 
+const std::vector<DevBuf DevEngine::*>& DevEngine::dev_bufs() {
+  using D = DevEngine;
+  static const std::vector<DevBuf D::*> all = {
+      &D::ctrl, &D::parent, &D::d_root, &D::d_closest, &D::iter, &D::nflag, &D::frontier, &D::closed,
+      &D::claim, &D::slot_node, &D::slot_fail, &D::act_slot, &D::b_n1, &D::b_n2, &D::b_ta, &D::b_tb,
+      &D::b_dist, &D::bt_key, &D::bt_val, &D::pair, &D::ulist,
+      &D::d_parent, &D::d_parent2, &D::d_force, &D::fault_pending, &D::frontier2, &D::rm_words, &D::rm_pref,
+      &D::slot_pos, &D::act_slot2, &D::trig, &D::s_ktab, &D::s_tree_cnt, &D::s_head, &D::s_mcnt, &D::s_mid, &D::s_md,
+      &D::s_next, &D::s_prop, &D::s_best, &D::s_psel, &D::s_dcl, &D::s_cnt, &D::s_accs, &D::s_hdr, &D::s_changed,
+      &D::s_ew, &D::s_ida, &D::s_idb, &D::s_sub, &D::s_segns, &D::s_fh, &D::s_sovf, &D::s_evs, &D::s_evn, &D::s_eve,
+      &D::s_evd, &D::s_acc, &D::s_backup, &D::s_items, &D::s_dbg, &D::s_hist, &D::w_acc, &D::acc_pref, &D::ustate32, &D::wg_pub, &D::commit_seq, &D::kc_trace,
+      &D::hp_base, &D::hp_size, &D::hp_v, &D::hp_key, &D::hp_pos, &D::hp_ref, &D::hp_gen, &D::hp_cnt, &D::slot_tree, &D::slot_heap, &D::slot_idx, &D::slot_word, &D::hp_plan,
+      &D::ord_hist, &D::ord_start, &D::ord_key, &D::ord_rank, &D::ord_pos, &D::ord_lst, &D::ord_cnt,
+      &D::w_ev, &D::ev_h, &D::ev_nb, &D::ev_raw, &D::spec_tab, &D::spec_area, &D::qclk_sh, &D::seq_args};
+  return all;
+}
+const std::vector<PinBuf DevEngine::*>& DevEngine::pin_bufs() {
+  static const std::vector<PinBuf DevEngine::*> all = {&DevEngine::h_ctrl, &DevEngine::h_seq, &DevEngine::h_trig};
+  return all;
+}
+
+size_t DevSpare::device_bytes() const {
+  size_t s = x_send.cap + x_recv.cap + e.wr.ring.cap;
+  for (auto m : DevEngine::dev_bufs()) s += (e.*m).cap;
+  return s;
+}
+void DevSpare::release() {
+  for (auto m : DevEngine::dev_bufs()) (e.*m).release();
+  for (auto m : DevEngine::pin_bufs()) (e.*m).release();
+  x_send.release();
+  x_recv.release();
+  e.wr.release();
+  if (e.wave_graph) (void)hipGraphExecDestroy(e.wave_graph);
+  if (e.ev_wave) (void)hipEventDestroy(e.ev_wave);
+  if (e.ev_wave2) (void)hipEventDestroy(e.ev_wave2);
+  e.wave_graph = nullptr;
+  e.ev_wave = e.ev_wave2 = nullptr;
+}
+void Ctx::spare_drop() {
+  if (!spare) return;
+  spare->release();
+  spare.reset();
+}
+
 Forest::~Forest() {
-  DevBuf* bufs[] = {&dev.ctrl, &dev.parent, &dev.d_root, &dev.d_closest, &dev.iter, &dev.nflag, &dev.frontier, &dev.closed,
-                    &dev.claim, &dev.slot_node, &dev.slot_fail, &dev.act_slot, &dev.b_n1, &dev.b_n2, &dev.b_ta, &dev.b_tb,
-                    &dev.b_dist, &dev.bt_key, &dev.bt_val, &dev.pair, &dev.ulist,
-                    &dev.d_parent, &dev.d_parent2, &dev.d_force, &dev.fault_pending, &dev.frontier2, &dev.rm_words, &dev.rm_pref,
-                    &dev.slot_pos, &dev.act_slot2, &dev.trig, &dev.s_ktab, &dev.s_tree_cnt, &dev.s_head, &dev.s_mcnt, &dev.s_mid, &dev.s_md,
-                    &dev.s_next, &dev.s_prop, &dev.s_best, &dev.s_psel, &dev.s_dcl, &dev.s_cnt, &dev.s_accs, &dev.s_hdr, &dev.s_changed,
-                    &dev.s_ew, &dev.s_ida, &dev.s_idb, &dev.s_sub, &dev.s_segns, &dev.s_fh, &dev.s_sovf, &dev.s_evs, &dev.s_evn, &dev.s_eve,
-                    &dev.s_evd, &dev.s_acc, &dev.s_backup, &dev.s_items, &dev.s_dbg, &dev.s_hist, &dev.w_acc, &dev.acc_pref, &dev.ustate32, &dev.wg_pub, &dev.commit_seq, &dev.kc_trace, &x_send, &x_recv,
-                    &dev.hp_base, &dev.hp_size, &dev.hp_v, &dev.hp_key, &dev.hp_pos, &dev.hp_ref, &dev.hp_gen, &dev.hp_cnt, &dev.slot_tree, &dev.slot_heap, &dev.slot_idx, &dev.slot_word, &dev.hp_plan,
-                    &dev.ord_hist, &dev.ord_start, &dev.ord_key, &dev.ord_rank, &dev.ord_pos, &dev.ord_lst, &dev.ord_cnt,
-                    &dev.w_ev, &dev.ev_h, &dev.ev_nb, &dev.ev_raw, &dev.spec_tab, &dev.spec_area, &dev.qclk_sh, &dev.seq_args};
   if (dev.inited) {
     (void)hipSetDevice(ctx->device);
     (void)hipStreamSynchronize(ctx->stream);
     (void)hipStreamSynchronize(ctx->copy_stream);
   }
-  for (DevBuf* b : bufs) b->release();
-  dev.h_ctrl.release();
-  dev.h_seq.release();
-  dev.wr.release();
-  dev.h_trig.release();
-  if (dev.wave_graph) (void)hipGraphExecDestroy(dev.wave_graph);
-  if (dev.ev_wave) (void)hipEventDestroy(dev.ev_wave);
-  if (dev.ev_wave2) (void)hipEventDestroy(dev.ev_wave2);
+  DevSpare s;
+  s.e = dev;
+  s.x_send = x_send;
+  s.x_recv = x_recv;
+  if (s.e.wave_graph) (void)hipGraphExecDestroy(s.e.wave_graph);
+  s.e.wave_graph = nullptr;
+  if (dev.inited && !kn.no_recycle) {
+    ctx->spare_drop();
+    ctx->spare.reset(new DevSpare(s));
+  } else {
+    s.release();
+  }
 }
 
 void Forest::begin_wave() {
diff --git a/space_filling_forest_star_amd/csrc/forest_batch.cpp b/space_filling_forest_star_amd/csrc/forest_batch.cpp
--- a/space_filling_forest_star_amd/csrc/forest_batch.cpp
+++ b/space_filling_forest_star_amd/csrc/forest_batch.cpp
@@ -53,6 +53,7 @@
   void take_in(int i, double* wait_ms) {
     Forest& f = *m[i];
     f.dev.status_copied[0] = true;
+    f.dev.produced_at[0] = f.dev.wr.produced;
     f.dev.host_stale = true;
     ++f.st.batch_launches;
     const int fault = f.dev_finish_wave(wait_ms, 0, true);
diff --git a/space_filling_forest_star_amd/csrc/forest_dev.cpp b/space_filling_forest_star_amd/csrc/forest_dev.cpp
--- a/space_filling_forest_star_amd/csrc/forest_dev.cpp
+++ b/space_filling_forest_star_amd/csrc/forest_dev.cpp
@@ -9,6 +9,7 @@
 
 #include "engine.h"
 #include "sff_geom.h"
+#include "wave_words.h"
 
 namespace sff {
 
@@ -323,6 +324,7 @@
   Ctx& c = *ctx;
   DevEngine& d = dev;
   const int cap = c.store_cap;
+  const bool first = d.node_cap == 0;
   d.node_cap = cap - cfg.wave - 16;
   d.temp_base = (cap - cfg.wave - 8) & ~3;
   if (d.node_cap < 64) throw HipError{"forest: node store too small for the device engine"};
@@ -335,14 +337,14 @@
   d.frontier2.ensure((size_t)cap * 4);
   const size_t old_rm = d.rm_words.cap;
   d.rm_words.ensure(((size_t)cap / 64 + 2) * 8);
-  if (d.rm_words.cap != old_rm)
+  if (first || d.rm_words.cap != old_rm)
     HIPCHK(hipMemsetAsync(d.rm_words.p, 0, d.rm_words.cap, c.stream));
   d.rm_pref.ensure(((size_t)cap / 64 + 2) * 4);
   d.closed.ensure((size_t)cap * 4);
   if (cfg.optimize) {
     const size_t old_head = d.s_head.cap;
     d.s_head.ensure((size_t)cap * 8);
-    if (d.s_head.cap != old_head) HIPCHK(hipMemsetAsync(d.s_head.p, 0, d.s_head.cap, c.stream));
+    if (first || d.s_head.cap != old_head) HIPCHK(hipMemsetAsync(d.s_head.p, 0, d.s_head.cap, c.stream));
   }
   if (cfg.record_parents && d.s_hist.p && 4 * cap + 4 * cfg.wave > d.hist_cap) {
     d.hist_cap = 4 * cap + 4 * cfg.wave;
@@ -350,7 +352,7 @@
   }
   const size_t old_claim = d.claim.cap;
   d.claim.ensure((size_t)cap * 4);
-  if (d.claim.cap != old_claim)
+  if (first || d.claim.cap != old_claim)
     HIPCHK(hipMemsetD32Async(reinterpret_cast<hipDeviceptr_t>(d.claim.p), 0x7fffffff, d.claim.cap / 4, c.stream));
 }
 
@@ -368,8 +370,8 @@
   const uint64_t want_tab = next_pow2((uint64_t)std::max(kn.test_border_cap >= 0 ? 64 : 1 << 16, 4 * d.border_cap));
   if (want_tab > d.bt_size) {
     d.bt_size = want_tab;
-    d.bt_key.release();
-    d.bt_val.release();
+    if (d.bt_key.cap < (size_t)want_tab * 8) d.bt_key.release();
+    if (d.bt_val.cap < (size_t)want_tab * 8) d.bt_val.release();
     d.bt_key.ensure((size_t)want_tab * 8);
     d.bt_val.ensure((size_t)want_tab * 8);
     HIPCHK(hipMemsetAsync(d.bt_key.p, 0, (size_t)want_tab * 8, c.stream));
@@ -413,10 +415,22 @@
 
 void Forest::dev_ring_top_up(uint64_t cursor, uint64_t ahead) {
   DevEngine& d = dev;
+  const int slot = d.start.top_ups < 2 ? d.start.top_ups : -1;
+  ++d.start.top_ups;
   if (d.wr.produced >= cursor + ahead) return;
   const uint64_t need = cursor + ahead - d.wr.produced;
   if (d.wr.produced + need - cursor > d.wr.ring_words) throw HipError{"forest: engine-word ring too small (internal error)"};
+  const auto t0 = Clock::now();
   dev_ring_append(nullptr, (size_t)need);
+  if (slot >= 0) { d.start.words[slot] = need; d.start.words_ms[slot] = ms_since(t0); }
+}
+
+uint64_t Forest::dev_waves_words(int n_waves) const {
+  const sffk::DevCtrl& k = dev.last;
+#ifdef SFFK_FIXED_TOP_UPS
+  return (uint64_t)n_waves * dev.max_wave_words;
+#endif
+  return wave_words_bound(k.n_nodes, cfg.wave, n_waves, dev.slot_words, k.in_wave ? std::max(1, k.n_slots) : 0);
 }
 
 void Forest::dev_upload_state() {
@@ -425,10 +439,15 @@
   HIPCHK(hipSetDevice(c.device));
   const int wave = cfg.wave;
   const int words_per = cfg.dim == 2 ? 1 : 6;
+  const auto t_upload = Clock::now();
+  const AllocClock alloc0 = alloc_clock();
+  const bool first_upload = !d.inited;
   if (!d.inited) {
-    HIPCHK(hipEventCreateWithFlags(&d.ev_wave, hipEventDisableTiming));
-    HIPCHK(hipEventCreateWithFlags(&d.ev_wave2, hipEventDisableTiming));
-    d.max_wave_words = (uint64_t)wave * ((use_priority() ? 5 : 1) + (uint64_t)std::max(1, cfg.threshold_misses) * words_per) + 64;
+    if (c.spare && !kn.no_recycle) dev_adopt_spare();
+    if (!d.ev_wave) HIPCHK(hipEventCreateWithFlags(&d.ev_wave, hipEventDisableTiming));
+    if (!d.ev_wave2) HIPCHK(hipEventCreateWithFlags(&d.ev_wave2, hipEventDisableTiming));
+    d.slot_words = (use_priority() ? 5 : 1) + (uint64_t)std::max(1, cfg.threshold_misses) * words_per;
+    d.max_wave_words = (uint64_t)wave * d.slot_words + 64;
     uint64_t ring_words = next_pow2(std::max<uint64_t>(4 * d.max_wave_words, (uint64_t)rng_ahead.size() + 2 * d.max_wave_words + 64));
     if (cfg.wave == 1) ring_words = std::max<uint64_t>(ring_words, 1 << 18);
     d.wr.init(ring_words);
@@ -441,6 +460,7 @@
     }
     d.ctrl.ensure(sizeof(sffk::DevCtrl));
     d.h_ctrl.ensure((size_t)SFFK_STATUS_RING * sizeof(sffk::DevCtrl));
+    memset(d.h_ctrl.p, 0xFF, (size_t)SFFK_STATUS_RING * sizeof(sffk::DevCtrl));
     d.slot_node.ensure((size_t)wave * 4);
     d.slot_pos.ensure((size_t)wave * 4);
     d.act_slot.ensure((size_t)wave * 4);
@@ -613,6 +633,51 @@
   d.host_nodes = n;
   d.host_stale = false;
   d.active = true;
+  if (first_upload) {
+    const AllocClock& ac = alloc_clock();
+    d.start.alloc_ms = ac.ms - alloc0.ms;
+    d.start.allocations = ac.n - alloc0.n;
+    d.start.upload_ms = ms_since(t_upload) - d.start.alloc_ms;
+  }
+}
+
+void Forest::dev_adopt_spare() {
+  Ctx& c = *ctx;
+  DevEngine& d = dev;
+  std::unique_ptr<DevSpare> s = std::move(c.spare);
+  s->e.kc_trace.release();
+  s->e.s_dbg.release();
+  int n = 0;
+  auto take = [&n](auto& mine, auto& theirs) {
+    if (mine.p || !theirs.p) return;
+    mine = theirs;
+    mine.stale = true;
+    theirs.p = nullptr;
+    theirs.cap = 0;
+    ++n;
+  };
+  for (auto m : DevEngine::dev_bufs()) take(d.*m, s->e.*m);
+  for (auto m : DevEngine::pin_bufs()) take(d.*m, s->e.*m);
+  take(x_send, s->x_send);
+  take(x_recv, s->x_recv);
+  take(d.wr.ring, s->e.wr.ring);
+  take(d.wr.h_ring, s->e.wr.h_ring);
+  auto take_event = [](hipEvent_t& mine, hipEvent_t& theirs) { if (!mine) { mine = theirs; theirs = nullptr; } };
+  take_event(d.wr.ev_ring, s->e.wr.ev_ring);
+  take_event(d.ev_wave, s->e.ev_wave);
+  take_event(d.ev_wave2, s->e.ev_wave2);
+  s->release();
+  d.start.adopted = n;
+  if (kn.test_poison_recycle) {
+    auto poison = [&](const DevBuf& b) { if (b.p) HIPCHK(hipMemsetAsync(b.p, 0xA5, b.cap, c.stream)); };
+    for (auto m : DevEngine::dev_bufs()) poison(d.*m);
+    poison(x_send);
+    poison(x_recv);
+    poison(d.wr.ring);
+    for (auto m : DevEngine::pin_bufs()) if ((d.*m).p) memset((d.*m).p, 0xA5, (d.*m).cap);
+    if (d.wr.h_ring.p) memset(d.wr.h_ring.p, 0xA5, d.wr.h_ring.cap);
+    HIPCHK(hipStreamSynchronize(c.stream));
+  }
 }
 
 void Forest::sync_host() {
@@ -1039,6 +1104,7 @@
   if (use_priority()) sffk::launch_prio_end(c.stream, dev_view(), c.store_view());
   sffk::launch_wave_end(c.stream, dev_view(), c.gridv.ovf_cnt, c.tgridv.ovf_cnt,
                         cfg.optimize ? d.s_acc.as<unsigned long long>() : nullptr);
+  d.produced_at[slot] = d.wr.produced;
   d.status_copied[slot] = kn.no_zc_status;
   if (!kn.no_zc_status) d.status_of[slot] = d.status_next++;
   else HIPCHK(hipMemcpyAsync(d.h_ctrl.as<sffk::DevCtrl>() + slot, d.ctrl.p, sizeof(sffk::DevCtrl), hipMemcpyDeviceToHost, c.stream));
@@ -1114,6 +1180,7 @@
       uint64_t before[T_KINDS];
       for (int k = 0; k < T_KINDS; ++k) before[k] = c.round_calls[k];
       d.force_timing = 0;
+      const auto t_cap = Clock::now();
       HIPCHK(hipStreamBeginCapture(c.stream, hipStreamCaptureModeRelaxed));
       hipGraph_t g = nullptr;
       try {
@@ -1126,8 +1193,13 @@
       }
       d.force_timing = -1;
       HIPCHK(hipStreamEndCapture(c.stream, &g));
+      const auto t_inst = Clock::now();
       HIPCHK(hipGraphInstantiate(&d.wave_graph, g, nullptr, nullptr, 0));
       (void)hipGraphDestroy(g);
+      if (!d.start.printed) {
+        d.start.capture_ms += std::chrono::duration<double, std::milli>(t_inst - t_cap).count();
+        d.start.instantiate_ms += ms_since(t_inst);
+      }
       for (int k = 0; k < T_KINDS; ++k) {
         d.graph_calls[k] = c.round_calls[k] - before[k];
         c.round_calls[k] = before[k];
@@ -1146,6 +1218,7 @@
     dev_enqueue_wave_kernels(sharded, words);
     d.force_timing = -1;
   }
+  d.produced_at[slot] = d.wr.produced;
   d.status_copied[slot] = kn.no_zc_status;
   if (!kn.no_zc_status) d.status_of[slot] = d.status_next++;
   else HIPCHK(hipMemcpyAsync(d.h_ctrl.as<sffk::DevCtrl>() + slot, d.ctrl.p, sizeof(sffk::DevCtrl), hipMemcpyDeviceToHost, c.stream));
@@ -1161,6 +1234,7 @@
     HIPCHK(hipEventSynchronize(slot ? d.ev_wave2 : d.ev_wave));
     if (stream_idle) c.sync();
     if (wait_ms) *wait_ms += ms_since(tw);
+    if (!d.start.wave0_waited) { d.start.wave0_waited = true; d.start.wait0_ms = ms_since(tw); }
   }
   if (!d.status_copied[slot]) {
     d.last = d.h_ctrl.as<sffk::DevCtrl>()[d.status_of[slot] & (SFFK_STATUS_RING - 1)];
@@ -1170,6 +1244,9 @@
   } else {
     d.last = d.h_ctrl.as<sffk::DevCtrl>()[slot];
   }
+  if (d.last.cursor > d.produced_at[slot])
+    throw HipError{"device engine: a wave read engine words that had not been generated (cursor " + std::to_string(d.last.cursor) +
+                   ", produced " + std::to_string(d.produced_at[slot]) + " when it was enqueued)"};
   if (!stream_idle) return d.last.fault;
   d.host_stale = true;
   const sffk::DevCtrl& s = d.last;
@@ -1237,7 +1314,7 @@
   if (!dev.active) dev_upload_state();
   const sffk::DevCtrl& k = dev.last;
   if (!k.in_wave && k.terminated) return false;
-  dev_ring_top_up(k.cursor, 2 * dev.max_wave_words);
+  dev_ring_top_up(k.cursor, dev_waves_words(2));
   dev_enqueue_begin();
   dev.host_stale = true;
   return true;
@@ -1438,6 +1515,7 @@
     }
     HIPCHK(hipMemcpyAsync(d.h_ctrl.as<sffk::DevCtrl>(), d.ctrl.p, sizeof(sffk::DevCtrl), hipMemcpyDeviceToHost, c.stream));
     d.status_copied[0] = true;
+    d.produced_at[0] = d.wr.produced;
     HIPCHK(hipEventRecord(d.ev_wave, c.stream));
     d.host_stale = true;
     const int fault = dev_finish_wave(&wait_ms, 0, true);
@@ -1497,6 +1575,17 @@
   }
 }
 
+void Forest::dev_start_report() {
+  DevEngine::Start& s = dev.start;
+  if (s.printed) return;
+  s.printed = true;
+  if (!kn.profile) return;
+  fprintf(stderr, "[sffgpu host event] forest start: allocations %.3f ms (%d new, %d adopted) | memsets + state upload + syncs %.3f ms | "
+          "words before wave 0: %llu in %.3f ms, before wave 1: %llu in %.3f ms | graph capture %.3f ms, instantiate %.3f ms (%llu captures) | "
+          "wait for wave 0 %.3f ms\n", s.alloc_ms, s.allocations, s.adopted, s.upload_ms, (unsigned long long)s.words[0], s.words_ms[0],
+          (unsigned long long)s.words[1], s.words_ms[1], s.capture_ms, s.instantiate_ms, (unsigned long long)dev.graph_captures, s.wait0_ms);
+}
+
 void Forest::run_device(int max_waves) {
   if (seq_eligible()) { run_device_seq(max_waves); return; }
   if (use_priority() && cfg.has_goal) {
@@ -1528,7 +1617,7 @@
         if (k.terminated) break;
         if (max_waves > 0 && (int)(k.waves - w0) >= max_waves) break;
       }
-      dev_ring_top_up(k.cursor, d.max_wave_words);
+      dev_ring_top_up(k.cursor, dev_waves_words(1));
       dev_enqueue_wave(slot);
       started = 1;
     } else {
@@ -1536,11 +1625,11 @@
     }
     const bool room = max_waves <= 0 || (int)(k.waves - w0) + (int)started + 1 <= max_waves;
     if (ahead_ok && room && !k.fault) {
-      dev_ring_top_up(k.cursor, 2 * d.max_wave_words);
+      dev_ring_top_up(k.cursor, dev_waves_words(2));
       dev_enqueue_wave(1 - slot);
       have_next = true;
     } else {
-      dev_ring_top_up(k.cursor, 2 * d.max_wave_words);
+      dev_ring_top_up(k.cursor, dev_waves_words(2));
     }
     int fault = dev_finish_wave(&wait_ms, slot, !have_next);
     const sffk::DevCtrl& s1 = d.last;
@@ -1578,6 +1667,7 @@
   }
   st.total_ms += ms_since(t0);
   st.host_ms += ms_since(t0) - wait_ms;
+  dev_start_report();
   if (kn.profile) {
     int32_t why[4] = {0, 0, 0, 0};
     HIPCHK(hipMemcpy(why, dev.fault_pending.p, 16, hipMemcpyDeviceToHost));
diff --git a/space_filling_forest_star_amd/csrc/knobs.cpp b/space_filling_forest_star_amd/csrc/knobs.cpp
--- a/space_filling_forest_star_amd/csrc/knobs.cpp
+++ b/space_filling_forest_star_amd/csrc/knobs.cpp
@@ -77,6 +77,8 @@
   k.no_fused_sample = flag("SFFGPU_NO_FUSED_SAMPLE", k.no_fused_sample);
   k.no_zc_status = flag("SFFGPU_NO_ZC_STATUS", k.no_zc_status);
   k.fallback_whole_wave = is_set("SFFGPU_FALLBACK_WHOLE_WAVE");
+  k.no_recycle = flag("SFFGPU_NO_RECYCLE", k.no_recycle);
+  k.test_poison_recycle = flag("SFFGPU_TEST_POISON_RECYCLE", k.test_poison_recycle);
   k.kc_trace = int_in("SFFGPU_KC_TRACE", k.kc_trace);
   k.digest = is_set("SFFGPU_DIGEST");
   k.no_seq = flag("SFFGPU_NO_SEQ", k.no_seq);
diff --git a/space_filling_forest_star_amd/csrc/knobs.h b/space_filling_forest_star_amd/csrc/knobs.h
--- a/space_filling_forest_star_amd/csrc/knobs.h
+++ b/space_filling_forest_star_amd/csrc/knobs.h
@@ -52,6 +52,8 @@
   bool no_fused_sample = false;
   bool no_zc_status = false;
   bool fallback_whole_wave = false;
+  bool no_recycle = false;
+  bool test_poison_recycle = false;
   int kc_trace = -1;
   bool digest = false;
   bool no_seq = false;
diff --git a/space_filling_forest_star_amd/csrc/wave_words.h b/space_filling_forest_star_amd/csrc/wave_words.h
--- /dev/null
+++ b/space_filling_forest_star_amd/csrc/wave_words.h
@@ -0,0 +1,19 @@
+#pragma once
+#include <stdint.h>
+
+#include <algorithm>
+
+namespace sff {
+
+inline uint64_t wave_words_bound(int64_t n_nodes, int wave, int n_waves, uint64_t per_slot, int first_slots = 0) {
+  uint64_t words = 0;
+  int64_t nn = std::max<int64_t>(n_nodes, 0);
+  for (int k = 0; k < n_waves; ++k) {
+    const int64_t s = (k == 0 && first_slots > 0) ? std::min<int64_t>(first_slots, wave) : std::min<int64_t>(wave, std::max<int64_t>(1, nn));
+    words += (uint64_t)s * per_slot + 64;
+    nn += s;
+  }
+  return words;
+}
+
+}
```

Result: no change. 12.15 million, median of 2 (+0.4%).
